# tiangexiang/OccNeRF

Measured on AMD Instinct MI355X. Metric: rays/sec at 512x512x128spp, random-init ckpt, higher is better.
Workload: dtype f32; 1 GPU; BASELINE configs[1]: free-view frame, 512x512 image, 128 samples/ray, non-rigid motion on, seeded random-init checkpoint; synthetic SMPL-like body and camera; 183784 rays hit the body bbox (ray_mask); H2D of the ray batch and the prior and D2H of [R,5] inside the step; the frame's rays sharded over the ranks; samples whose motion-weight sum is exactly 0 are dropped after the warp (bit-identical pi; rays_per_frame=183784, samples_per_ray=128, skip_empty_samples=True, dedup_repeated_samples=False, knn_center_cache=True, warp_bone_culling=True, world_size_formed=1

## Files before the change

### include/occnerf_hip.h

```cpp
#ifndef OCCNERF_HIP_H
#define OCCNERF_HIP_H

#include <stdint.h>

#ifdef __cplusplus
extern "C" {
#endif

#define OCCNERF_ABI_VERSION 5

int occnerf_abi_version(void);
const char *occnerf_last_error(void);

int occnerf_experiment_knob(const char *name, int value);


int occnerf_grid_encode_forward(const float *inputs, const float *embeddings,
                                const int32_t *offsets, float *outputs, uint32_t B, uint32_t D,
                                uint32_t C, uint32_t L, float S, uint32_t H, float *dy_dx,
                                uint32_t gridtype, int align_corners, uint32_t interp,
                                void *stream);

int occnerf_grid_encode_backward(const float *grad, const float *inputs, const float *embeddings,
                                 const int32_t *offsets, float *grad_embeddings, uint32_t B,
                                 uint32_t D, uint32_t C, uint32_t L, float S, uint32_t H,
                                 const float *dy_dx, float *grad_inputs, uint32_t gridtype,
                                 int align_corners, uint32_t interp, void *stream);

int occnerf_grid_encode_forward_h(const float *inputs, const float *embeddings, const int32_t *offsets,
                                  const int32_t *h_offsets, float *outputs, uint32_t B, uint32_t D, uint32_t C, uint32_t L,
                                  float S, uint32_t H, float *dy_dx, uint32_t gridtype, int align_corners,
                                  uint32_t interp, void *stream);

int occnerf_grid_grad_runs(const float *grad_rows, const float *inputs, int64_t B, uint32_t D, uint32_t L, uint32_t C,
                           float *grad, void *stream);

int occnerf_grid_encode_backward_h(const float *grad, const float *inputs, const float *embeddings,
                                   const int32_t *offsets, const int32_t *h_offsets, float *grad_embeddings,
                                   uint32_t B, uint32_t D, uint32_t C, uint32_t L, float S, uint32_t H,
                                   const float *dy_dx, float *grad_inputs, uint32_t gridtype, int align_corners,
                                   uint32_t interp, void *scratch, int64_t scratch_bytes, void *stream);

int occnerf_grid_encode_forward_f16(const float *inputs, const void *embeddings, const int32_t *offsets, void *outputs,
                                    uint32_t B, uint32_t D, uint32_t C, uint32_t L, float S, uint32_t H, void *dy_dx,
                                    uint32_t gridtype, int align_corners, uint32_t interp, void *stream);
int occnerf_grid_encode_backward_f16(const void *grad, const float *inputs, const void *embeddings, const int32_t *offsets,
                                     void *grad_embeddings, uint32_t B, uint32_t D, uint32_t C, uint32_t L, float S,
                                     uint32_t H, const void *dy_dx, void *grad_inputs, uint32_t gridtype, int align_corners,
                                     uint32_t interp, void *stream);

int occnerf_grid_encode_forward_f64(const float *inputs, const double *embeddings, const int32_t *offsets, double *outputs,
                                    uint32_t B, uint32_t D, uint32_t C, uint32_t L, float S, uint32_t H, double *dy_dx,
                                    uint32_t gridtype, int align_corners, uint32_t interp, void *stream);
int occnerf_grid_encode_backward_f64(const double *grad, const float *inputs, const double *embeddings, const int32_t *offsets,
                                     double *grad_embeddings, uint32_t B, uint32_t D, uint32_t C, uint32_t L, float S,
                                     uint32_t H, const double *dy_dx, double *grad_inputs, uint32_t gridtype, int align_corners,
                                     uint32_t interp, void *stream);

int occnerf_grad_total_variation(const float *inputs, const float *embeddings, float *grad,
                                 const int32_t *offsets, float weight, uint32_t B, uint32_t D,
                                 uint32_t C, uint32_t L, float S, uint32_t H, uint32_t gridtype,
                                 int align_corners, void *stream);


int occnerf_sample_warp(const float *rays, int64_t n, int32_t S, const float *t_vals,
                        const float *t_rand, const float *Rs, const float *Ts, const float *vol,
                        int32_t nb, int32_t G, const float *h_bbox_min, const float *h_bbox_scale,
                        float *z_vals, float *pts, float *x_skel, float *mask, void *stream);
int occnerf_bone_boxes(const float *vol, int32_t nb, int32_t G, int32_t *boxes, void *stream);
int occnerf_sample_warp_culled(const float *rays, int64_t n, int32_t S, const float *t_vals,
                               const float *Rs, const float *Ts, const float *vol, int32_t nb, int32_t G,
                               const int32_t *boxes, const float *h_bbox_min, const float *h_bbox_scale,
                               float *z_vals, float *x_skel, float *mask, void *stream);

int64_t occnerf_ray_order_temp_bytes(int64_t R);
int occnerf_ray_order(const float *dirs, int64_t R, int64_t stride, int64_t *order, void *temp, int64_t temp_bytes,
                      void *stream);

int occnerf_gen_rays(const double *h_Kinv, const double *h_R, const double *h_T, int32_t f32_camera,
                     int32_t H, int32_t W, const double *h_bbox_min, const double *h_bbox_max, float *rays8,
                     uint8_t *mask, void *stream);

int64_t occnerf_nonrigid_packed_floats(void);
int occnerf_nonrigid_pack(const float *const *h_W, const float *const *h_b, float *packed,
                          void *stream);
int occnerf_nonrigid(const float *xyz_in, int64_t N, const float *cond, const float *h_hann,
                     const float *W0, const float *b0, float *packed, float *xyz_out,
                     void *stream);
int occnerf_nonrigid_rows(float *xyz, int64_t N_max, const int32_t *rows, const int32_t *n_dev,
                          const float *cond, const float *h_hann, const float *W0, const float *b0,
                          float *packed, void *stream);
int occnerf_nonrigid_direct(const float *xyz_in, int64_t N, const float *cond, const float *h_hann,
                            const float *W0, const float *b0, float *packed, float *xyz_out,
                            void *stream);

int64_t occnerf_nonrigid_packed_bf16_bytes(void);
int occnerf_nonrigid_pack_bf16(const float *const *h_W, void *packed_bf16, void *stream);
int occnerf_nonrigid_bf16x3(const float *xyz_in, int64_t N, const float *cond, const float *h_hann,
                            const float *W0, const float *b0, float *packed, const void *packed_bf16,
                            float *xyz_out, void *stream);
int occnerf_nonrigid_bf16x3_rows(float *xyz, int64_t N_max, const int32_t *rows, const int32_t *n_dev,
                                 const float *cond, const float *h_hann, const float *W0, const float *b0,
                                 float *packed, const void *packed_bf16, void *stream);

int occnerf_msknn(const float *xyz, int64_t N, const float *points, const int32_t *index_map,
                  const int32_t *h_scale_begin, const int32_t *h_seed_from_coarser,
                  int32_t nscale, int32_t *knn_idxs, void *stream);

int occnerf_msknn_clustered(const float *xyz, const float *mask, int64_t n_rays, int32_t samples_per_ray,
                            const float *points, const float *centers,
                            const int32_t *cluster_ranges, const float *cluster_radius, int32_t ncl,
                            const float *group_centers, const int32_t *group_ranges, const float *group_radius, int32_t ngrp,
                            const int32_t *h_coarse_rows, const int32_t *h_seed_from_coarser,
                            int32_t nscale, const int32_t *query_rows, const int32_t *n_query_dev, int32_t *ray_start,
                            int32_t *knn_idxs, void *stream);
int occnerf_knn_center(const float *c, const float *points, const int32_t *index_map, const int32_t *h_scale_begin,
                       int32_t nscale, float *center_out, int32_t *idx_out, void *stream);
int occnerf_msknn_clustered_centered(const float *xyz, const float *mask, int64_t n_rays, int32_t samples_per_ray,
                                     const float *points, const float *centers,
                                     const int32_t *cluster_ranges, const float *cluster_radius, int32_t ncl,
                                     const float *group_centers, const int32_t *group_ranges, const float *group_radius, int32_t ngrp,
                                     const int32_t *h_coarse_rows, const int32_t *h_seed_from_coarser,
                                     int32_t nscale, const int32_t *query_rows, const int32_t *n_query_dev, int32_t *ray_start,
                                     const float *center, const int32_t *center_idx, int32_t *knn_idxs, void *stream);

int occnerf_knn_small(const float *q, int32_t nq, const float *s, int32_t ns, int32_t k,
                      int32_t *idx, void *stream);

int occnerf_unit_normals(const double *normals, int32_t P, double *unit, void *stream);

int occnerf_point_sdf(const float *point_cloud, const float *point_base, const double *normals,
                      const double *unit_normals, const int32_t *kidx, int32_t P,
                      double *knn_base, float *dist, void *stream);

int occnerf_point_sdf_backward(const float *point_cloud, const float *point_base, const double *normals,
                               const double *unit_normals, const int32_t *kidx, int32_t P, const double *d_knn_base,
                               const float *d_dist, float *d_point_dist, void *stream);
int32_t occnerf_point_table_stride(void);
int occnerf_point_table(const double *knn_base, const float *point_sdf, const float *learnable,
                        int32_t P, float bound, float two_bound, const float *embeddings,
                        const int32_t *offsets, const int32_t *h_offsets, uint32_t L, float S,
                        uint32_t H, float *table, void *stream);

int occnerf_point_pack(const float *point_base, const double *normals, const double *unit_normals,
                       const float *counter, const float *table, int32_t P, float *point_geo,
                       float *point_tail, void *stream);
int occnerf_sample_features(const float *xyz, int64_t N, const int32_t *knn_idxs, int32_t nscale,
                            const float *point_base, const double *normals,
                            const double *unit_normals, const float *counter,
                            const float *table, float bound, float two_bound,
                            const float *embeddings, const int32_t *offsets,
                            const int32_t *h_offsets, uint32_t L, float S, uint32_t H,
                            const int32_t *geo_idxs, const float *att_in, const int32_t *rows,
                            const int32_t *n_dev, const float *point_geo, const float *point_tail, int32_t P,
                            float *mlp_in, float *raw, float *enc_in, void *stream);
int occnerf_sample_features_centered(const float *xyz, int64_t N, const int32_t *knn_idxs, int32_t nscale,
                            const float *point_base, const double *normals,
                            const double *unit_normals, const float *counter,
                            const float *table, float bound, float two_bound,
                            const float *embeddings, const int32_t *offsets,
                            const int32_t *h_offsets, uint32_t L, float S, uint32_t H,
                            const int32_t *geo_idxs, const float *att_in, const int32_t *rows,
                            const int32_t *n_dev, const float *point_geo, const float *point_tail, int32_t P,
                            const float *center, const float *center_agg,
                                     float *mlp_in, float *raw, float *enc_in, void *stream);

int occnerf_agg_forward(const float *feats, int32_t F, const int32_t *knn, const float *atts, int64_t N, int32_t K,
                        float *agg, void *stream);
int32_t occnerf_agg_backward_slices(int64_t N);
int64_t occnerf_agg_backward_scratch_bytes(int64_t N, int32_t F);
int occnerf_agg_backward(const float *grad_agg, int32_t F, const int32_t *knn, const float *atts, int64_t N,
                         int32_t K, int32_t P, float *partial, void *scratch, int64_t scratch_bytes, void *stream);

int64_t occnerf_live_rows_temp_bytes(int64_t N);
int occnerf_live_rows(const float *mask, int64_t N, int32_t *rows, int32_t *count, void *temp,
                      int64_t temp_bytes, void *stream);
int occnerf_scatter_raw(const float *raw_c, const int32_t *rows, const int32_t *n_dev, int64_t N_max,
                        float *raw_full, void *stream);

int64_t occnerf_repeat_heads_temp_bytes(int64_t N_max);
int occnerf_repeat_heads(const void *keys, int64_t stride_dwords, int32_t key_dwords, const int32_t *rows,
                         const int32_t *n_dev, int64_t N_max, int32_t *scan, int32_t *heads, int32_t *head_count,
                         float *head_mask, void *temp, int64_t temp_bytes, void *stream);
int64_t occnerf_unique_heads_temp_bytes(int64_t cap);
int occnerf_unique_heads(const void *keys, int64_t stride_dwords, int32_t key_dwords, const int32_t *heads,
                         const int32_t *n_dev, int64_t cap, int32_t *heads_out, int32_t *count_out, int32_t *scan,
                         const int32_t *n_scan_dev, int64_t scan_cap, void *temp, int64_t temp_bytes, void *stream);
int occnerf_scatter_raw_heads(const float *raw_h, const float *raw_c, const int32_t *rows, const int32_t *n_dev,
                              const int32_t *scanA, const int32_t *scanB, int64_t N_max, float *raw_full, void *stream);
int occnerf_canonical_mlp_rows(const float *mlp_in, const int32_t *in_rows, int64_t N_max, const int32_t *n_dev,
                               const float *packed, float *raw, void *stream);

int64_t occnerf_canonical_mlp_packed_floats(void);
int occnerf_canonical_mlp_pack(const float *const *h_W, const float *const *h_b, float *packed,
                               void *stream);

int occnerf_canonical_mlp(const float *mlp_in, int64_t N, const float *packed, float *raw,
                          void *stream);
int occnerf_canonical_mlp_direct(const float *mlp_in, int64_t N, const float *packed, float *raw,
                                 void *stream);
int occnerf_canonical_mlp_counted(const float *mlp_in, int64_t N_max, const int32_t *n_dev,
                                  const float *packed, float *raw, void *stream);

int64_t occnerf_canonical_mlp_packed_bf16_bytes(void);
int occnerf_canonical_mlp_pack_bf16(const float *const *h_W, void *packed_bf16, void *stream);
int occnerf_canonical_mlp_bf16x3(const float *mlp_in, int64_t N, const float *packed,
                                 const void *packed_bf16, float *raw, int32_t variant,
                                 void *stream);
int occnerf_canonical_mlp_bf16x3_rows(const float *mlp_in, const int32_t *in_rows, int64_t N_max,
                                      const int32_t *n_dev, const float *packed, const void *packed_bf16,
                                      float *raw, int32_t variant, void *stream);

int occnerf_canonical_mlp_pack_f16(const float *const *h_W, void *packed_f16, void *stream);
int occnerf_canonical_mlp_f16x3(const float *mlp_in, const int32_t *in_rows, int64_t N_max, const int32_t *n_dev,
                                const float *packed, const void *packed_f16, float *raw, uint32_t *domain_flag,
                                void *stream);
int occnerf_nonrigid_pack_f16(const float *const *h_W, void *packed_f16, void *stream);
int occnerf_nonrigid_f16x3(const float *xyz_in, int64_t N_max, const int32_t *rows, const int32_t *n_dev,
                           const float *cond, const float *h_hann, const float *W0, const float *b0, float *packed,
                           const void *packed_f16, float *xyz_out, uint32_t *domain_flag, void *stream);

int occnerf_composite(const float *raw, const float *mask, const float *z_vals, const float *rays,
                      const float *h_bgcolor, int64_t n, int32_t S, float *rgb, float *acc,
                      float *depth, float *weights, int32_t *term, const int64_t *out_rows, void *stream);


int occnerf_linear_pack(const float *W, const float *b, int32_t out_dim, int32_t in_dim, const int32_t *row_map,
                        int32_t n_pad, const int32_t *col_map, int32_t k_pad, int32_t bf16, void *Wp, void *Wt,
                        float *bias_p, void *stream);
int occnerf_linear_forward(const void *x0, int64_t ld0, int32_t k0, const void *x1, int64_t ld1, int32_t k1,
                           const void *W, const float *bias, int32_t relu, const void *mask, int64_t ldm, void *y,
                           int64_t ldy, int32_t out_f32, int32_t n_store, float *aux, int32_t aux_col,
                           int64_t aux_stride, int64_t M, int32_t n_pad, int32_t bf16, void *stream);
int32_t occnerf_linear_wgrad_slices(int64_t M);
int occnerf_linear_wgrad(const void *dz, int64_t lddz, int32_t n_pad, const void *x, int64_t ldx, int32_t k_pad,
                         int64_t M, int32_t bf16, float *part, float *dbpart, void *stream);
int occnerf_linear_wgrad_reduce(const float *part, const float *dbpart, int32_t G, int32_t n_pad, int32_t k_pad,
                                const int32_t *row_map, const int32_t *col_map, float *dW, int32_t in_dim, float *db,
                                int32_t accumulate, void *stream);

int64_t occnerf_trunks_packed_bytes(void);
int occnerf_trunks_pack_bf16(const float *const *h_W, void *packed, void *stream);
int occnerf_trunks_forward_bf16(const float *agg, const float *var, const float *enc, int64_t M, const float *packed_f32,
                                const void *packed_bf16, void *X0, void *const *h_A, void *GEO, void *const *h_B, float *raw4,
                                void *stream);

int occnerf_composite_backward(const float *raw, const float *mask, const float *z_vals, const float *rays,
                               const float *h_bgcolor, int64_t n, int32_t S, const float *g_rgb, const float *g_acc,
                               const float *g_depth, float *d_raw, float *d_mask, void *stream);

int32_t occnerf_warp_backward_slices(int64_t n_samples);
int occnerf_warp_backward(const float *rays, int64_t n, int32_t S, const float *z_vals, const float *g_mask,
                          const float *Rs, const float *Ts, const float *vol, int32_t nb, int32_t G,
                          const float *h_bbox_min, const float *h_bbox_scale, float *d_vol_part, float *d_rt_part,
                          void *stream);

int occnerf_agg_weights(const float *counter, const int32_t *knn, int64_t N, int32_t K, float *atts, float *var,
                        void *stream);

int occnerf_pose_motion_bases_backward(const float *const *h_W, const float *const *h_b, const float *posevec,
                                       const float *dst_Rs, const float *dst_Ts, const float *cnl_gtfms,
                                       const float *dRs, const float *dTs, float *const *h_dW, float *const *h_db,
                                       void *stream);

int occnerf_pose_motion_bases(const float *const *h_W, const float *const *h_b, const float *posevec, int32_t refine,
                              const float *dst_Rs, const float *dst_Ts, const float *cnl_gtfms, float *Rs, float *Ts,
                              void *stream);
int occnerf_prior_softmax(const float *decoded, const float *prior, int32_t C, int64_t V, float *vol, void *stream);
int occnerf_pack_rays(const float *rays, const float *near, const float *far, const int64_t *order, int64_t R, float *rays8,
                      void *stream);

int occnerf_assemble_image(const float *rgb, const float *alpha, const int64_t *ray_index, int64_t R, int32_t height,
                           int32_t width, const float *h_bgcolor01, uint8_t *out_rgb, uint8_t *out_alpha, void *stream);

int occnerf_convt3d_col2im(const float *cols, const float *bias, int32_t Cout, int32_t D, int32_t H, int32_t W,
                           float *out, void *stream);
int occnerf_convt3d_im2col(const float *gy, int32_t Cout, int32_t D, int32_t H, int32_t W, float *dcols, void *stream);

int32_t occnerf_adam_table_row_bytes(void);
int occnerf_adam_step(const void *table, int32_t n_tensors, const int32_t *chunks, int32_t n_chunks,
                      int32_t chunk_elems, double beta1, double beta2, double eps, double max_grad_norm, float *scratch,
                      void *stream);

int64_t occnerf_lpips_packed_floats(void);
int64_t occnerf_lpips_workspace_floats(int32_t N, int32_t H, int32_t W);
int occnerf_lpips_pack(const float *const *h_conv_w, const float *const *h_conv_b, const float *const *h_lin,
                       const float *shift, const float *scale, float *packed, void *stream);
int occnerf_lpips_forward(const float *packed, const float *in0, const float *in1, int32_t N, int32_t H, int32_t W,
                          int32_t in_nhwc, float *work, float *val, float *res, void *stream);
int occnerf_lpips_backward(const float *packed, float *work, int32_t N, int32_t H, int32_t W, int32_t in_nhwc,
                           const float *gres, float *d_in0, float *d_in1, void *stream);

int occnerf_patch_assemble(const float *rgb, const int32_t *row_of_pix, int64_t R, int32_t n_patches, int32_t size,
                           const float *h_bgcolor01, float *img, void *stream);
int occnerf_patch_assemble_backward(const float *d_img, const int32_t *pix_of_row, int64_t R, float *d_rgb, void *stream);

int32_t occnerf_patch_batch_max_patches(void);
int occnerf_patch_batch(const uint8_t *image, const uint8_t *alpha, const float *rays8, const uint8_t *box_mask, int32_t H,
                        int32_t W, int32_t n_patches, int32_t size, const double *h_u, double subject_ratio,
                        const float *h_bgcolor, int32_t *row_counts, float *rays, float *near, float *far, float *target_rgbs,
                        float *target_patches, uint8_t *patch_masks, int32_t *patch_div_indices, int32_t *xy_min,
                        int32_t *pix_of_row, int32_t *row_of_pix, int32_t *n_rows, void *stream);

#define OCCNERF_FRAME_METRICS_RECORD 14
int64_t occnerf_frame_metrics_workspace_bytes(int32_t N, int32_t H, int32_t W);
int occnerf_frame_metrics(const uint8_t *pred, const uint8_t *truth, const float *alpha, const uint8_t *body,
                          const float *gt_vis_alpha, const float *gt_alpha, int32_t N, int32_t H, int32_t W,
                          double data_range, double *record, double *ssim_map, void *workspace, void *stream);

#ifdef __cplusplus
}
#endif
#endif
```

### occnerf_amd/_lib.py

```python
import ctypes as C
import os

_HERE = os.path.dirname(os.path.abspath(__file__))
LIB_PATH = os.environ.get('OCCNERF_HIP_LIB') or os.path.join(_HERE, 'liboccnerf_hip.so')

ABI_VERSION = 5

_vp, _i32, _i64, _u32, _f32 = C.c_void_p, C.c_int32, C.c_int64, C.c_uint32, C.c_float

SIGNATURES = {
    'occnerf_abi_version': (C.c_int, []),
    'occnerf_last_error': (C.c_char_p, []),
    'occnerf_experiment_knob': (C.c_int, [C.c_char_p, C.c_int]),
    'occnerf_grid_encode_forward': (C.c_int, [_vp, _vp, _vp, _vp, _u32, _u32, _u32, _u32, _f32, _u32,
                                               _vp, _u32, C.c_int, _u32, _vp]),
    'occnerf_grid_encode_backward': (C.c_int, [_vp, _vp, _vp, _vp, _vp, _u32, _u32, _u32, _u32, _f32,
                                                _u32, _vp, _vp, _u32, C.c_int, _u32, _vp]),
    'occnerf_grid_grad_runs': (C.c_int, [_vp, _vp, _i64, _u32, _u32, _u32, _vp, _vp]),
    'occnerf_grid_encode_forward_h': (C.c_int, [_vp, _vp, _vp, _vp, _vp, _u32, _u32, _u32, _u32, _f32, _u32,
                                                 _vp, _u32, C.c_int, _u32, _vp]),
    'occnerf_grid_encode_backward_h': (C.c_int, [_vp, _vp, _vp, _vp, _vp, _vp, _u32, _u32, _u32, _u32, _f32,
                                                  _u32, _vp, _vp, _u32, C.c_int, _u32, _vp, _i64, _vp]),
    'occnerf_grid_encode_forward_f16': (C.c_int, [_vp, _vp, _vp, _vp, _u32, _u32, _u32, _u32, _f32, _u32,
                                                   _vp, _u32, C.c_int, _u32, _vp]),
    'occnerf_grid_encode_backward_f16': (C.c_int, [_vp, _vp, _vp, _vp, _vp, _u32, _u32, _u32, _u32, _f32,
                                                    _u32, _vp, _vp, _u32, C.c_int, _u32, _vp]),
    'occnerf_grid_encode_forward_f64': (C.c_int, [_vp, _vp, _vp, _vp, _u32, _u32, _u32, _u32, _f32, _u32,
                                                   _vp, _u32, C.c_int, _u32, _vp]),
    'occnerf_grid_encode_backward_f64': (C.c_int, [_vp, _vp, _vp, _vp, _vp, _u32, _u32, _u32, _u32, _f32,
                                                    _u32, _vp, _vp, _u32, C.c_int, _u32, _vp]),
    'occnerf_trunks_packed_bytes': (_i64, []),
    'occnerf_trunks_pack_bf16': (C.c_int, [_vp, _vp, _vp]),
    'occnerf_trunks_forward_bf16': (C.c_int, [_vp, _vp, _vp, _i64, _vp, _vp, _vp, _vp, _vp, _vp, _vp, _vp]),
    'occnerf_grad_total_variation': (C.c_int, [_vp, _vp, _vp, _vp, _f32, _u32, _u32, _u32, _u32, _f32,
                                                _u32, _u32, C.c_int, _vp]),
    'occnerf_sample_warp': (C.c_int, [_vp, _i64, _i32, _vp, _vp, _vp, _vp, _vp, _i32, _i32, _vp, _vp,
                                       _vp, _vp, _vp, _vp, _vp]),
    'occnerf_bone_boxes': (C.c_int, [_vp, _i32, _i32, _vp, _vp]),
    'occnerf_sample_warp_culled': (C.c_int, [_vp, _i64, _i32, _vp, _vp, _vp, _vp, _i32, _i32, _vp, _vp, _vp, _vp, _vp, _vp, _vp]),
    'occnerf_nonrigid_packed_floats': (_i64, []),
    'occnerf_nonrigid_pack': (C.c_int, [_vp, _vp, _vp, _vp]),
    'occnerf_nonrigid': (C.c_int, [_vp, _i64, _vp, _vp, _vp, _vp, _vp, _vp, _vp]),
    'occnerf_nonrigid_direct': (C.c_int, [_vp, _i64, _vp, _vp, _vp, _vp, _vp, _vp, _vp]),
    'occnerf_nonrigid_packed_bf16_bytes': (_i64, []),
    'occnerf_nonrigid_pack_bf16': (C.c_int, [_vp, _vp, _vp]),
    'occnerf_nonrigid_bf16x3': (C.c_int, [_vp, _i64, _vp, _vp, _vp, _vp, _vp, _vp, _vp, _vp]),
    'occnerf_nonrigid_bf16x3_rows': (C.c_int, [_vp, _i64, _vp, _vp, _vp, _vp, _vp, _vp, _vp, _vp, _vp]),
    'occnerf_msknn': (C.c_int, [_vp, _i64, _vp, _vp, _vp, _vp, _i32, _vp, _vp]),
    'occnerf_msknn_clustered': (C.c_int, [_vp, _vp, _i64, _i32, _vp, _vp, _vp, _vp, _i32, _vp, _vp, _vp, _i32, _vp, _vp, _i32,
                                           _vp, _vp, _vp, _vp, _vp]),
    'occnerf_msknn_clustered_centered': (C.c_int, [_vp, _vp, _i64, _i32, _vp, _vp, _vp, _vp, _i32, _vp, _vp, _vp, _i32, _vp, _vp, _i32,
                                           _vp, _vp, _vp, _vp, _vp, _vp, _vp]),
    'occnerf_knn_center': (C.c_int, [_vp, _vp, _vp, _vp, _i32, _vp, _vp, _vp]),
    'occnerf_knn_small': (C.c_int, [_vp, _i32, _vp, _i32, _i32, _vp, _vp]),
    'occnerf_unit_normals': (C.c_int, [_vp, _i32, _vp, _vp]),
    'occnerf_point_sdf': (C.c_int, [_vp, _vp, _vp, _vp, _vp, _i32, _vp, _vp, _vp]),
    'occnerf_ray_order_temp_bytes': (_i64, [_i64]),
    'occnerf_ray_order': (C.c_int, [_vp, _i64, _i64, _vp, _vp, _i64, _vp]),
    'occnerf_point_sdf_backward': (C.c_int, [_vp, _vp, _vp, _vp, _vp, _i32, _vp, _vp, _vp, _vp]),
    'occnerf_gen_rays': (C.c_int, [_vp, _vp, _vp, _i32, _i32, _i32, _vp, _vp, _vp, _vp, _vp]),
    'occnerf_agg_forward': (C.c_int, [_vp, _i32, _vp, _vp, _i64, _i32, _vp, _vp]),
    'occnerf_agg_backward_slices': (_i32, [_i64]),
    'occnerf_agg_backward_scratch_bytes': (_i64, [_i64, _i32]),
    'occnerf_agg_backward': (C.c_int, [_vp, _i32, _vp, _vp, _i64, _i32, _i32, _vp, _vp, _i64, _vp]),
    'occnerf_live_rows_temp_bytes': (_i64, [_i64]),
    'occnerf_live_rows': (C.c_int, [_vp, _i64, _vp, _vp, _vp, _i64, _vp]),
    'occnerf_scatter_raw': (C.c_int, [_vp, _vp, _vp, _i64, _vp, _vp]),
    'occnerf_repeat_heads_temp_bytes': (_i64, [_i64]),
    'occnerf_repeat_heads': (C.c_int, [_vp, _i64, _i32, _vp, _vp, _i64, _vp, _vp, _vp, _vp, _vp, _i64, _vp]),
    'occnerf_unique_heads_temp_bytes': (_i64, [_i64]),
    'occnerf_unique_heads': (C.c_int, [_vp, _i64, _i32, _vp, _vp, _i64, _vp, _vp, _vp, _vp, _i64, _vp, _i64, _vp]),
    'occnerf_scatter_raw_heads': (C.c_int, [_vp, _vp, _vp, _vp, _vp, _vp, _i64, _vp, _vp]),
    'occnerf_canonical_mlp_rows': (C.c_int, [_vp, _vp, _i64, _vp, _vp, _vp, _vp]),
    'occnerf_canonical_mlp_counted': (C.c_int, [_vp, _i64, _vp, _vp, _vp, _vp]),
    'occnerf_nonrigid_rows': (C.c_int, [_vp, _i64, _vp, _vp, _vp, _vp, _vp, _vp, _vp, _vp]),
    'occnerf_point_table_stride': (_i32, []),
    'occnerf_point_table': (C.c_int, [_vp, _vp, _vp, _i32, _f32, _f32, _vp, _vp, _vp, _u32, _f32, _u32, _vp,
                                       _vp]),
    'occnerf_point_pack': (C.c_int, [_vp, _vp, _vp, _vp, _vp, _i32, _vp, _vp, _vp]),
    'occnerf_sample_features': (C.c_int, [_vp, _i64, _vp, _i32, _vp, _vp, _vp, _vp, _vp, _f32, _f32, _vp,
                                           _vp, _vp, _u32, _f32, _u32, _vp, _vp, _vp, _vp, _vp, _vp, _i32, _vp, _vp,
                                           _vp, _vp]),
    'occnerf_sample_features_centered': (C.c_int, [_vp, _i64, _vp, _i32, _vp, _vp, _vp, _vp, _vp, _f32, _f32, _vp,
                                                    _vp, _vp, _u32, _f32, _u32, _vp, _vp, _vp, _vp, _vp, _vp, _i32, _vp, _vp,
                                                    _vp, _vp, _vp, _vp]),
    'occnerf_canonical_mlp_packed_floats': (_i64, []),
    'occnerf_canonical_mlp_pack': (C.c_int, [_vp, _vp, _vp, _vp]),
    'occnerf_canonical_mlp': (C.c_int, [_vp, _i64, _vp, _vp, _vp]),
    'occnerf_canonical_mlp_direct': (C.c_int, [_vp, _i64, _vp, _vp, _vp]),
    'occnerf_canonical_mlp_packed_bf16_bytes': (_i64, []),
    'occnerf_canonical_mlp_pack_bf16': (C.c_int, [_vp, _vp, _vp]),
    'occnerf_canonical_mlp_bf16x3': (C.c_int, [_vp, _i64, _vp, _vp, _vp, _i32, _vp]),
    'occnerf_canonical_mlp_pack_f16': (C.c_int, [_vp, _vp, _vp]),
    'occnerf_canonical_mlp_f16x3': (C.c_int, [_vp, _vp, _i64, _vp, _vp, _vp, _vp, _vp, _vp]),
    'occnerf_nonrigid_pack_f16': (C.c_int, [_vp, _vp, _vp]),
    'occnerf_nonrigid_f16x3': (C.c_int, [_vp, _i64, _vp, _vp, _vp, _vp, _vp, _vp, _vp, _vp, _vp, _vp, _vp]),
    'occnerf_canonical_mlp_bf16x3_rows': (C.c_int, [_vp, _vp, _i64, _vp, _vp, _vp, _vp, _i32, _vp]),
    'occnerf_composite': (C.c_int, [_vp, _vp, _vp, _vp, _vp, _i64, _i32, _vp, _vp, _vp, _vp, _vp, _vp, _vp]),
    'occnerf_linear_pack': (C.c_int, [_vp, _vp, _i32, _i32, _vp, _i32, _vp, _i32, _i32, _vp, _vp, _vp, _vp]),
    'occnerf_linear_forward': (C.c_int, [_vp, _i64, _i32, _vp, _i64, _i32, _vp, _vp, _i32, _vp, _i64, _vp, _i64, _i32,
                                          _i32, _vp, _i32, _i64, _i64, _i32, _i32, _vp]),
    'occnerf_linear_wgrad_slices': (_i32, [_i64]),
    'occnerf_linear_wgrad': (C.c_int, [_vp, _i64, _i32, _vp, _i64, _i32, _i64, _i32, _vp, _vp, _vp]),
    'occnerf_linear_wgrad_reduce': (C.c_int, [_vp, _vp, _i32, _i32, _i32, _vp, _vp, _vp, _i32, _vp, _i32, _vp]),
    'occnerf_composite_backward': (C.c_int, [_vp, _vp, _vp, _vp, _vp, _i64, _i32, _vp, _vp, _vp, _vp, _vp, _vp]),
    'occnerf_warp_backward_slices': (_i32, [_i64]),
    'occnerf_warp_backward': (C.c_int, [_vp, _i64, _i32, _vp, _vp, _vp, _vp, _vp, _i32, _i32, _vp, _vp, _vp, _vp, _vp]),
    'occnerf_agg_weights': (C.c_int, [_vp, _vp, _i64, _i32, _vp, _vp, _vp]),
    'occnerf_pose_motion_bases': (C.c_int, [_vp, _vp, _vp, _i32, _vp, _vp, _vp, _vp, _vp, _vp]),
    'occnerf_pose_motion_bases_backward': (C.c_int, [_vp, _vp, _vp, _vp, _vp, _vp, _vp, _vp, _vp, _vp, _vp]),
    'occnerf_prior_softmax': (C.c_int, [_vp, _vp, _i32, _i64, _vp, _vp]),
    'occnerf_pack_rays': (C.c_int, [_vp, _vp, _vp, _vp, _i64, _vp, _vp]),
    'occnerf_assemble_image': (C.c_int, [_vp, _vp, _vp, _i64, _i32, _i32, _vp, _vp, _vp, _vp]),
    'occnerf_convt3d_col2im': (C.c_int, [_vp, _vp, _i32, _i32, _i32, _i32, _vp, _vp]),
    'occnerf_convt3d_im2col': (C.c_int, [_vp, _i32, _i32, _i32, _i32, _vp, _vp]),
    'occnerf_adam_table_row_bytes': (_i32, []),
    'occnerf_adam_step': (C.c_int, [_vp, _i32, _vp, _i32, _i32] + [C.c_double] * 4 + [_vp, _vp]),
    'occnerf_lpips_packed_floats': (_i64, []),
    'occnerf_lpips_workspace_floats': (_i64, [_i32, _i32, _i32]),
    'occnerf_lpips_pack': (C.c_int, [_vp, _vp, _vp, _vp, _vp, _vp, _vp]),
    'occnerf_lpips_forward': (C.c_int, [_vp, _vp, _vp, _i32, _i32, _i32, _i32, _vp, _vp, _vp, _vp]),
    'occnerf_lpips_backward': (C.c_int, [_vp, _vp, _i32, _i32, _i32, _i32, _vp, _vp, _vp, _vp]),
    'occnerf_patch_assemble': (C.c_int, [_vp, _vp, _i64, _i32, _i32, _vp, _vp, _vp]),
    'occnerf_patch_assemble_backward': (C.c_int, [_vp, _vp, _i64, _vp, _vp]),
    'occnerf_patch_batch_max_patches': (_i32, []),
    'occnerf_patch_batch': (C.c_int, [_vp, _vp, _vp, _vp, _i32, _i32, _i32, _i32, _vp, C.c_double, _vp] + [_vp] * 12 + [_vp]),
    'occnerf_frame_metrics_workspace_bytes': (_i64, [_i32, _i32, _i32]),
    'occnerf_frame_metrics': (C.c_int, [_vp, _vp, _vp, _vp, _vp, _vp, _i32, _i32, _i32, C.c_double, _vp, _vp, _vp, _vp]),
}

_lib = None


def lib():
    global _lib
    if _lib is None:
        if not os.path.exists(LIB_PATH):
            raise ImportError(
                f'{LIB_PATH} not found: the gfx950 kernels are not built. Run '
                '`python -c "import __graft_entry__ as g; g.build()"` (or `make -C '
                'occnerf_amd/csrc`). There is no CPU fallback for this path.')
        import torch
        handle = C.CDLL(LIB_PATH)
        for name, (res, args) in SIGNATURES.items():
            fn = getattr(handle, name)
            fn.restype, fn.argtypes = res, args
        if handle.occnerf_abi_version() != ABI_VERSION:
            raise ImportError(f'liboccnerf_hip.so: ABI version {handle.occnerf_abi_version()}, this binding was written '
                              f'for {ABI_VERSION} (include/occnerf_hip.h OCCNERF_ABI_VERSION): rebuild the library')
        _lib = handle
    return _lib


def check(rc, what):
    if rc != 0:
        msg = lib().occnerf_last_error().decode(errors='replace')
        raise RuntimeError(f'{what} failed ({rc}): {msg}')
```

### occnerf_amd/config.py

```python
import argparse
import ast
import copy
import os

import yaml


class CfgNode(dict):
    def __getattr__(self, k):
        try:
            return self[k]
        except KeyError:
            raise AttributeError(k)

    def __setattr__(self, k, v):
        self[k] = v

    def get(self, k, default=None):
        return dict.get(self, k, default)

    @staticmethod
    def wrap(d):
        if isinstance(d, dict) and not isinstance(d, CfgNode):
            return CfgNode({k: CfgNode.wrap(v) for k, v in d.items()})
        return d

    def merge(self, other):
        for k, v in other.items():
            if isinstance(v, dict) and isinstance(self.get(k), dict):
                self[k].merge(v)
            else:
                self[k] = CfgNode.wrap(copy.deepcopy(v))
        return self

    def merge_from_file(self, path):
        with open(path) as f:
            return self.merge(yaml.safe_load(f) or {})

    def merge_from_list(self, opts):
        assert len(opts) % 2 == 0, 'opts must be KEY VALUE pairs'
        for key, val in zip(opts[0::2], opts[1::2]):
            node = self
            parts = key.split('.')
            for p in parts[:-1]:
                node = node[p]
            try:
                val = ast.literal_eval(val)
            except (ValueError, SyntaxError):
                pass
            node[parts[-1]] = val
        return self

    def clone(self):
        return CfgNode.wrap(copy.deepcopy(dict(self)))


_DEFAULTS = {
    'category': 'occnerf', 'task': 'zju_mocap', 'subject': 'p387', 'experiment': 'occnerf',
    'resume': False, 'eval_iter': 10000000, 'render_folder_name': '',
    'ignore_non_rigid_motions': False, 'render_skip': 1, 'render_frames': 100, 'num_workers': 4,
    'network_module': 'core.nets.occnerf.network',
    'embedder': {'module': 'core.nets.occnerf.embedders.fourier'},
    'non_rigid_embedder': {'module': 'core.nets.occnerf.embedders.hannw_fourier'},
    'canonical_mlp': {'module': 'core.nets.occnerf.canonical_mlps.occnerf_mlp', 'mlp_depth': 4,
                      'mlp_width': 256, 'multires': 10, 'i_embed': 0},
    'mweight_volume': {'module': 'core.nets.occnerf.mweight_vol_decoders.deconv_vol_decoder',
                       'embedding_size': 256, 'volume_size': 32, 'dst_voxel_size': 0.0625},
    'non_rigid_motion_mlp': {'module': 'core.nets.occnerf.non_rigid_motion_mlps.mlp_offset',
                             'condition_code_size': 69, 'mlp_width': 128, 'mlp_depth': 6,
                             'skips': [4], 'multires': 6, 'i_embed': 0, 'kick_in_iter': 100000,
                             'full_band_iter': 200000},
    'pose_decoder': {'module': 'core.nets.occnerf.pose_decoders.mlp_delta_body_pose',
                     'embedding_size': 69, 'mlp_width': 256, 'mlp_depth': 4,
                     'kick_in_iter': 2000000},
    'sex': 'neutral', 'total_bones': 24, 'bbox_offset': 0.3, 'load_net': 'latest',
    'N_samples': 128, 'perturb': 1.0, 'netchunk_per_gpu': 300000, 'chunk': 32768, 'n_gpus': 1,
    'bgcolor': [0.0, 0.0, 0.0], 'resize_img_scale': 0.5, 'show_alpha': False, 'show_truth': False,
    'patch': {'sample_subject_ratio': 0.8, 'N_patches': 6, 'size': 32},
    'freeview': {'frame_idx': 0}, 'tpose': {}, 'movement': {},
    'train': {'dataset_path': None, 'images_prescaled': False, 'seed': 0, 'prefetch': True},
    'occlude': False, 'occlusion': {'range': 405, 'mid': 451, 'width': 86},
    'eval': {'lpips': False, 'lpips_model_path': None, 'lpips_vgg16_path': None},
    'smpl_model': 'auto',
    'max_samples_per_pass': 1 << 28,
    'mlp_precision': 'fp32',
    'f16x3_domain_check': True,
    'train_fused_trunks': True,
    'skip_empty_samples': True,
    'device_rays': True,
    'ray_patch_order': True,
    'knn_culling': True,
    'knn_center_cache': True,
    'warp_bone_culling': True,
}

_cfg = None


def default_cfg():
    return CfgNode.wrap(copy.deepcopy(_DEFAULTS))


def get_cfg():
    global _cfg
    if _cfg is None:
        _cfg = default_cfg()
        _finish(_cfg)
    return _cfg


def set_cfg(cfg):
    global _cfg
    _cfg = cfg
    return cfg


def _finish(cfg):
    import torch
    cfg.logdir = os.path.join('experiments', cfg.category, cfg.task, cfg.subject, cfg.experiment)
    n = torch.cuda.device_count()
    cfg.n_gpus = n
    cfg.primary_gpus = [0] if n > 0 else ['cpu']
    cfg.secondary_gpus = ([g for g in range(n) if g != 0] or cfg.primary_gpus) if n > 1 \
        else cfg.primary_gpus


def make_cfg(argv=None):
    parser = argparse.ArgumentParser()
    parser.add_argument('--cfg', required=True, type=str)
    parser.add_argument('--eval', default='full', type=str)
    parser.add_argument('--type', default='skip', type=str)
    parser.add_argument('opts', default=None, nargs=argparse.REMAINDER)
    args = parser.parse_args(argv)
    cfg = default_cfg()
    here = os.path.dirname(os.path.dirname(os.path.abspath(__file__)))
    default_yaml = os.path.join(here, 'configs', 'default.yaml')
    if os.path.exists(default_yaml):
        cfg.merge_from_file(default_yaml)
    cfg.merge_from_file(args.cfg)
    cfg.merge_from_list(args.opts or [])
    _finish(cfg)
    set_cfg(cfg)
    return cfg, args
```

### occnerf_amd/csrc/features.hip

```cpp
#include "common.h"

#include <cstdlib>

namespace occ {

constexpr int kKnn = 10;
constexpr int kTableCols = 36;
constexpr int kTableStride = 64;

__device__ __forceinline__ double cos3_unit(const float (&a)[3], const double *__restrict__ un) {
    float na = norm3(a[0], a[1], a[2]);
    na = na < 1e-8f ? 1e-8f : na;
    const double t0 = __dmul_rn((double)__fdiv_rn(a[0], na), un[0]);
    const double t1 = __dmul_rn((double)__fdiv_rn(a[1], na), un[1]);
    const double t2 = __dmul_rn((double)__fdiv_rn(a[2], na), un[2]);
    return __dadd_rn(__dadd_rn(t0, t1), t2);
}

__global__ void unit_normals_kernel(const double *__restrict__ normals, int P,
                                    double *__restrict__ unit) {
    const int i = blockIdx.x * blockDim.x + threadIdx.x;
    if (i >= P) return;
    const double b0 = normals[i * 3], b1 = normals[i * 3 + 1], b2 = normals[i * 3 + 2];
    double nb = __dsqrt_rn(__dadd_rn(__dadd_rn(__dmul_rn(b0, b0), __dmul_rn(b1, b1)), __dmul_rn(b2, b2)));
// ... 68 lines not shown
        for (int k = 0; k < 3; k++) datt += d_knn_base[i * 3 + k] * (nbr[j][k] - num[k] / den);
        datt /= den;
        const double dc = c[j] < 0.0 ? -datt : (c[j] > 0.0 ? datt : 0.0);
        for (int k = 0; k < 3; k++) {
            const double u = dir[j][k] / nd[j];
            g += gd * u + dc * (unit[n * 3 + k] - c[j] * u) / nd[j];
        }
    }
    d_point_dist[i] = (float)g;
}

__global__ void point_table_kernel(const double *__restrict__ knn_base,
                                   const float *__restrict__ point_sdf,
                                   const float *__restrict__ learnable, int P, float bound,
                                   float two_bound, const float2 *__restrict__ embeddings,
                                   const int32_t *__restrict__ offsets, int L, GridLevels lv,
                                   GridModes4 gm, float *__restrict__ table) {
    const int i = blockIdx.x * blockDim.x + threadIdx.x;
    if (i >= P) return;
    float x[4];
#pragma unroll
    for (int c = 0; c < 3; c++)
        x[c] = (float)__ddiv_rn(__dadd_rn(knn_base[i * 3 + c], (double)bound), (double)two_bound);
    float s = __fdiv_rn(__fadd_rn(point_sdf[i], 0.2f), 0.8f);
    x[3] = s < 0.0f ? 0.0f : (s > 1.0f ? 1.0f : s);
    bool oob = false;
#pragma unroll
    for (int d = 0; d < 4; d++) oob |= (x[d] < 0.f || x[d] > 1.f);
    float *row = table + (size_t)i * kTableStride;
    for (int l = 0; l < L; l++) {
        float2 v = make_float2(0.f, 0.f);
        if (!oob) {
            const uint32_t o0 = (uint32_t)offsets[l];
            v = encode_level_d4c2(x, embeddings + o0, (uint32_t)offsets[l + 1] - o0, lv.scale[l],
                                  lv.resolution[l], gm.mode[l]);
        }
        row[l * 2] = v.x;
        row[l * 2 + 1] = v.y;
    }
    for (int l = L; l < 16; l++) row[l * 2] = row[l * 2 + 1] = 0.f;
#pragma unroll
    for (int c = 0; c < 3; c++) row[32 + c] = learnable[i * 3 + c];
    row[35] = 0.0f;
}

static GridModes4 modes_from_host_offsets(uint32_t L, const GridLevels &lv, const int32_t *h_offsets) {
    uint32_t sizes[kMaxLevels] = {0};
    if (h_offsets)
        for (uint32_t l = 0; l < L; l++) sizes[l] = (uint32_t)(h_offsets[l + 1] - h_offsets[l]);
    GridModes4 gm = make_grid_modes_d4(h_offsets ? L : 0, lv, sizes);
    return gm;
}

struct FeatParams {
    float bound, two_bound;
    int nscale, L;
    int P;
};

struct LevelRec4 {
    uint32_t entry0, size;
    float scale;
    uint32_t res_mode;
};
struct LevelRecs {
    LevelRec4 r[kMaxLevels];
};
struct LevelRec8 {
    uint32_t entry0, mask;
    float scale;
    uint32_t dense;
    uint32_t mul1, mul2, mul3, pad;
};
struct LevelRecs8 {
    LevelRec8 r[kMaxLevels];
};
__device__ __forceinline__ void level_taps_select(const float (&x)[4], const float2 *grid, const LevelRec8 lr,
                                                  LevelTaps4 &tp) {
    const uint32_t mul[4] = {1u, lr.mul1, lr.mul2, lr.mul3};
    uint32_t t[4][2];
#pragma unroll
    for (int d = 0; d < 4; d++) {
        float pos = __fmaf_rn(x[d], lr.scale, 0.5f);
        const float fl = floorf(pos);
        const uint32_t pg = (uint32_t)fl;
        pos -= fl;
        tp.fr[d] = pos;
        t[d][0] = pg * mul[d];
        t[d][1] = t[d][0] + mul[d];
    }
    uint32_t a01[4], x01[4], a23[4], x23[4];
#pragma unroll
    for (int i = 0; i < 4; i++) {
        a01[i] = t[0][i & 1] + t[1][i >> 1];
        x01[i] = t[0][i & 1] ^ t[1][i >> 1];
        a23[i] = t[2][i & 1] + t[3][i >> 1];
        x23[i] = t[2][i & 1] ^ t[3][i >> 1];
    }
#pragma unroll
    for (int idx = 0; idx < 16; idx++) {
        const uint32_t ia = a01[idx & 3] + a23[idx >> 2];
        const uint32_t ix = (x01[idx & 3] ^ x23[idx >> 2]) & lr.mask;
        const uint32_t index = lr.dense ? ia : ix;
#ifdef OCC_FEAT_EXP_RESIDENT_HASH
        tp.v[idx] = ld32(grid, (lr.entry0 + (index & 63u)) * 8u);
#else
        tp.v[idx] = ld32(grid, (lr.entry0 + index) * 8u);
#endif
    }
}

__global__ __launch_bounds__(256) void sample_features_kernel(
    const float *__restrict__ xyz, int64_t N, const int32_t *__restrict__ knn_idxs,
    const float *__restrict__ point_base, const double *__restrict__ normals,
    const double *__restrict__ unit, const float *__restrict__ counter,
    const float4 *__restrict__ table, const float2 *__restrict__ embeddings,
    const int32_t *__restrict__ offsets, GridLevels lv, GridModes4 gm, FeatParams prm,
    const int32_t *__restrict__ geo_idxs, const float *__restrict__ att_in,
    float *__restrict__ mlp_in, float *__restrict__ raw, float *__restrict__ enc_in_out) {
    const int nk = prm.nscale * kKnn;
    for (int64_t i = (int64_t)blockIdx.x * blockDim.x + threadIdx.x; i < N;
         i += (int64_t)gridDim.x * blockDim.x) {
        const int32_t *id = knn_idxs + i * nk;
        const float p[3] = {xyz[i * 3], xyz[i * 3 + 1], xyz[i * 3 + 2]};

        int neg = 0;
        float dsum = 0.0f;
        double num[3] = {0.0, 0.0, 0.0}, den = 0.0;
#pragma unroll
        for (int j = 0; j < kKnn; j++) {
            const int n = geo_idxs ? geo_idxs[i * kKnn + j] : id[j];
            float dir[3], nbr[3];
#pragma unroll
            for (int c = 0; c < 3; c++) {
                nbr[c] = point_base[n * 3 + c];
                dir[c] = __fsub_rn(p[c], nbr[c]);
            }
            double dot = 0.0;
#pragma unroll
            for (int c = 0; c < 3; c++) dot = __dadd_rn(dot, __dmul_rn((double)dir[c], normals[(size_t)n * 3 + c]));
            neg += dot < 0.0;
            dsum = __fadd_rn(dsum, norm3(dir[0], dir[1], dir[2]));
            if (j < 3) {
                const double att = fabs(cos3_unit(dir, unit + (size_t)n * 3));
#pragma unroll
                for (int c = 0; c < 3; c++) {
                    const float pn = __fdiv_rn(__fadd_rn(nbr[c], prm.bound), prm.two_bound);
                    num[c] = __dadd_rn(num[c], __dmul_rn(att, (double)pn));
                }
                den = __dadd_rn(den, att);
            }
        }
        float dist = __fdiv_rn(dsum, (float)kKnn);
        if (2 * neg > kKnn) dist = -dist;
        float nd = __fdiv_rn(__fadd_rn(dist, 0.2f), 0.5f);
        nd = nd < 0.0f ? 0.0f : (nd > 1.0f ? 1.0f : nd);
        float x[4];
#pragma unroll
        for (int c = 0; c < 3; c++) x[c] = (float)__ddiv_rn(num[c], den);
        x[3] = nd;
        if (enc_in_out) {
#pragma unroll
            for (int c = 0; c < 4; c++) enc_in_out[i * 4 + c] = x[c];
        }
        raw[i * 5 + 4] = dist;

        float *out = mlp_in + i * 68;

        bool oob = false;
#pragma unroll
        for (int d = 0; d < 4; d++) oob |= (x[d] < 0.f || x[d] > 1.f);
        for (int l = 0; l < prm.L; l++) {
            float2 v = make_float2(0.f, 0.f);
            if (!oob) {
                const uint32_t o0 = (uint32_t)offsets[l];
                v = encode_level_d4c2(x, embeddings + o0, (uint32_t)offsets[l + 1] - o0,
                                      lv.scale[l], lv.resolution[l], gm.mode[l]);
            }
            *reinterpret_cast<float2 *>(out + 36 + l * 2) = v;
        }

        float att[4 * kKnn];
        float amin = INFINITY;
#pragma unroll
        for (int j = 0; j < 4 * kKnn; j++) {
            att[j] = j < nk ? (att_in ? att_in[i * nk + j] : counter[id[j]]) : INFINITY;
            amin = fminf(amin, att[j]);
        }
        float amax = -INFINITY;
#pragma unroll
        for (int j = 0; j < 4 * kKnn; j++) {
            if (j < nk) {
                att[j] = __fadd_rn(att[j], __fsub_rn(1.0f, amin));
                amax = fmaxf(amax, att[j]);
            }
        }
        float mean = 0.0f;
#pragma unroll
        for (int j = 0; j < 4 * kKnn; j++) {
            if (j < nk) {
                att[j] = __fdiv_rn(att[j], amax);
                mean = __fadd_rn(mean, att[j]);
            }
        }
        mean = __fdiv_rn(mean, (float)nk);
        float var = 0.0f, smax = -INFINITY;
#pragma unroll
        for (int j = 0; j < 4 * kKnn; j++) {
            if (j < nk) {
                const float dlt = __fsub_rn(att[j], mean);
                var = __fadd_rn(var, __fmul_rn(dlt, dlt));
                smax = fmaxf(smax, att[j]);
            }
        }
        var = __fdiv_rn(var, (float)(nk - 1));
        float ssum = 0.0f;
#pragma unroll
        for (int j = 0; j < 4 * kKnn; j++) {
            if (j < nk) {
                att[j] = expf(__fsub_rn(att[j], smax));
                ssum = __fadd_rn(ssum, att[j]);
            }
        }
        float agg[kTableCols];
#pragma unroll
        for (int f = 0; f < kTableCols; f++) agg[f] = 0.0f;
#pragma unroll
        for (int j = 0; j < 4 * kKnn; j++) {
            if (j < nk) {
                const float a = __fdiv_rn(att[j], ssum);
                const float4 *row = table + (size_t)id[j] * (kTableStride / 4);
#pragma unroll
                for (int v = 0; v < kTableCols / 4; v++) {
                    const float4 t = row[v];
                    agg[v * 4 + 0] = __fadd_rn(agg[v * 4 + 0], __fmul_rn(a, t.x));
                    agg[v * 4 + 1] = __fadd_rn(agg[v * 4 + 1], __fmul_rn(a, t.y));
                    agg[v * 4 + 2] = __fadd_rn(agg[v * 4 + 2], __fmul_rn(a, t.z));
                    agg[v * 4 + 3] = __fadd_rn(agg[v * 4 + 3], __fmul_rn(a, t.w));
                }
            }
        }
        agg[35] = var;
#pragma unroll
        for (int v = 0; v < kTableCols / 4; v++)
            *reinterpret_cast<float4 *>(out + v * 4) =
                make_float4(agg[v * 4], agg[v * 4 + 1], agg[v * 4 + 2], agg[v * 4 + 3]);
    }
}


__global__ void point_pack_kernel(const float *__restrict__ point_base, const double *__restrict__ normals,
                                  const double *__restrict__ unit, const float *__restrict__ counter,
                                  const float *__restrict__ table, int P, float *__restrict__ geo,
                                  float4 *__restrict__ tailc) {
    const int i = blockIdx.x * blockDim.x + threadIdx.x;
    if (i >= P) return;
    float *r = geo + (size_t)i * 16;
    r[0] = point_base[i * 3], r[1] = point_base[i * 3 + 1], r[2] = point_base[i * 3 + 2], r[3] = 0.0f;
    double *d = reinterpret_cast<double *>(r + 4);
    d[0] = normals[i * 3], d[1] = normals[i * 3 + 1], d[2] = normals[i * 3 + 2];
    d[3] = unit[i * 3], d[4] = unit[i * 3 + 1], d[5] = unit[i * 3 + 2];
    const float *t = table + (size_t)i * kTableStride + 32;
    tailc[i] = make_float4(t[0], t[1], t[2], counter[i]);
}

__device__ __forceinline__ float grp_sum8(float v) {
    v += __shfl_xor(v, 1, 8);
    v += __shfl_xor(v, 2, 8);
    v += __shfl_xor(v, 4, 8);
    return v;
}
__device__ __forceinline__ float grp_min8(float v) {
    v = fminf(v, __shfl_xor(v, 1, 8));
    v = fminf(v, __shfl_xor(v, 2, 8));
    return fminf(v, __shfl_xor(v, 4, 8));
}
__device__ __forceinline__ float grp_max8(float v) {
    v = fmaxf(v, __shfl_xor(v, 1, 8));
    v = fmaxf(v, __shfl_xor(v, 2, 8));
    return fmaxf(v, __shfl_xor(v, 4, 8));
}

template <int Q>
__device__ __forceinline__ float quad_bcast(float v) {
    return __builtin_bit_cast(float, __builtin_amdgcn_mov_dpp(__builtin_bit_cast(int, v), Q * 0x55, 0xf, 0xf, true));
}
template <int Q>
__device__ __forceinline__ double quad_bcast_f64(float lo, float hi) {
    return __hiloint2double(__builtin_amdgcn_mov_dpp(__builtin_bit_cast(int, hi), Q * 0x55, 0xf, 0xf, true),
                            __builtin_amdgcn_mov_dpp(__builtin_bit_cast(int, lo), Q * 0x55, 0xf, 0xf, true));
}

constexpr int kLdsTailPoints = 9216;

template <bool GENERIC ,
          bool LDS_TAIL >
__global__ __launch_bounds__(LDS_TAIL ? 768 : 256, 3) void sample_features8_kernel(
    const float *__restrict__ xyz, int64_t N_max, const int32_t *__restrict__ knn_idxs,
    const float4 *__restrict__ geo , const float4 *__restrict__ tailc ,
    const float4 *__restrict__ table, const float2 *__restrict__ embeddings,
    LevelRecs levels, LevelRecs8 levels8, FeatParams prm, const int32_t *__restrict__ rows ,
    const int32_t *__restrict__ n_dev , float *__restrict__ mlp_in, float *__restrict__ raw, float *__restrict__ enc_in_out,
    const float *__restrict__ center ,
    const float *__restrict__ center_agg ) {
    constexpr int NK = 4 * kKnn;
    float ccx = 0.f, ccy = 0.f, ccz = 0.f, cr2 = 0.f;
    if (center) ccx = center[0], ccy = center[1], ccz = center[2], cr2 = center[3];
    __shared__ float4 s_tail[LDS_TAIL ? kLdsTailPoints : 1];
    __shared__ float4 s_out[LDS_TAIL ? 768 : 256];
    static_assert(sizeof(float4) * (size_t)kLdsTailPoints + sizeof(float4) * 768 <= 160 * 1024,
                  "sample_features8_kernel<LDS_TAIL>: (tail, count) image + per-lane encoding slots exceed gfx950's 160 KiB of LDS");
    if constexpr (LDS_TAIL) {
        for (int i = threadIdx.x; i < prm.P; i += blockDim.x) s_tail[i] = tailc[i];
        __syncthreads();
    }
    const int g = threadIdx.x & 7;
    const int lane64 = threadIdx.x & 63;
    const int tr = ((lane64 & 7) << 3) | (lane64 >> 3);
    const int64_t N = n_dev ? (int64_t)*n_dev : N_max;
    if (N <= 0) return;
    const int64_t group0 = ((int64_t)blockIdx.x * blockDim.x + threadIdx.x) >> 3;
    const int64_t ngroups = ((int64_t)gridDim.x * blockDim.x) >> 3;
    const int64_t iters = (N + ngroups - 1) / ngroups;

    struct StageA {
        float p[3];
        int idg, id89;
        int id5[5];
    };
    auto out_row = [&](int64_t it) {
        const int64_t i_raw = group0 + it * ngroups;
        return i_raw < N ? i_raw : N - 1;
    };
    auto load_a = [&](int64_t i, StageA &a) {
        const int32_t *id = knn_idxs + i * NK;
        struct __attribute__((packed, aligned(4))) F3 { float v[3]; };
        struct __attribute__((packed, aligned(4))) I4 { int v[4]; };
        const F3 pq = *reinterpret_cast<const F3 *>(xyz + i * 3);
        a.p[0] = pq.v[0], a.p[1] = pq.v[1], a.p[2] = pq.v[2];
        a.idg = id[g];
        a.id89 = id[8 + (g >> 2)];
        const I4 q = *reinterpret_cast<const I4 *>(id + g * 5);
        a.id5[0] = q.v[0], a.id5[1] = q.v[1], a.id5[2] = q.v[2], a.id5[3] = q.v[3];
        a.id5[4] = id[g * 5 + 4];
    };
    StageA cur, nxt;
    int32_t i1;
    {
        const int64_t o0 = out_row(0), o1 = out_row(1);
        load_a(rows ? (int64_t)rows[o0] : o0, cur);
        i1 = rows ? rows[o1] : (int32_t)o1;
    }
    for (int64_t it = 0; it < iters; it++) {
        const bool live = group0 + it * ngroups < N;
        const int64_t o = out_row(it);
        const int64_t o2 = out_row(it + 2);
        float *out = mlp_in + o * 68;

        bool cached_agg = false;
        if (cr2 > 0.0f) {
            const float dx = cur.p[0] - ccx, dy = cur.p[1] - ccy, dz = cur.p[2] - ccz;
            const bool inside = __builtin_fmaf(dz, dz, __builtin_fmaf(dy, dy, dx * dx)) < cr2;
            cached_agg = __builtin_amdgcn_ballot_w64(live && !inside) == 0;
        }
        float4 tl[5];
#pragma unroll
        for (int k = 0; k < 5; k++) tl[k] = make_float4(0.f, 0.f, 0.f, 0.f);
        if (!cached_agg) {
#pragma unroll
            for (int k = 0; k < 5; k++) tl[k] = LDS_TAIL ? s_tail[cur.id5[k]] : ld32(tailc, (uint32_t)cur.id5[k] * 16u);
        }

        float nrm[5];
        int negf[5];
        double t_att[2] = {0.0, 0.0}, t_num[2][3] = {{0.0, 0.0, 0.0}, {0.0, 0.0, 0.0}};
        {
            float4 pc[5];
#pragma unroll
            for (int k = 0; k < 5; k++) {
                const int nid = k < 4 ? __shfl(cur.idg, 2 * k + (g >> 2), 8) : cur.id89;
                pc[k] = ld32(geo, (uint32_t)nid * 64u + (uint32_t)(g & 3) * 16u);
            }
#pragma unroll
            for (int k = 0; k < 5; k++) {
                const float nbr[3] = {quad_bcast<0>(pc[k].x), quad_bcast<0>(pc[k].y), quad_bcast<0>(pc[k].z)};
                const double nx = quad_bcast_f64<1>(pc[k].x, pc[k].y), ny = quad_bcast_f64<1>(pc[k].z, pc[k].w);
                const double nz = quad_bcast_f64<2>(pc[k].x, pc[k].y);
                float dir[3];
#pragma unroll
                for (int c = 0; c < 3; c++) dir[c] = __fsub_rn(cur.p[c], nbr[c]);
                double dot = __dadd_rn(0.0, __dmul_rn((double)dir[0], nx));
                dot = __dadd_rn(dot, __dmul_rn((double)dir[1], ny));
                dot = __dadd_rn(dot, __dmul_rn((double)dir[2], nz));
                negf[k] = dot < 0.0;
                nrm[k] = norm3(dir[0], dir[1], dir[2]);
                if (k < 2) {
                    const double un[3] = {quad_bcast_f64<2>(pc[k].z, pc[k].w), quad_bcast_f64<3>(pc[k].x, pc[k].y),
                                          quad_bcast_f64<3>(pc[k].z, pc[k].w)};
                    t_att[k] = fabs(cos3_unit(dir, un));
#pragma unroll
                    for (int c = 0; c < 3; c++) {
                        const float pn = __fdiv_rn(__fadd_rn(nbr[c], prm.bound), prm.two_bound);
                        t_num[k][c] = __dmul_rn(t_att[k], (double)pn);
                    }
                }
            }
        }
        float dsum = 0.0f;
        int neg = 0;
#pragma unroll
        for (int j = 0; j < kKnn; j++) {
            dsum = __fadd_rn(dsum, __shfl(nrm[j >> 1], 4 * (j & 1), 8));
            neg += __shfl(negf[j >> 1], 4 * (j & 1), 8);
        }
        double num[3] = {0.0, 0.0, 0.0}, den = 0.0;
#pragma unroll
        for (int j = 0; j < 3; j++) {
#pragma unroll
            for (int c = 0; c < 3; c++) num[c] = __dadd_rn(num[c], __shfl(t_num[j >> 1][c], 4 * (j & 1), 8));
            den = __dadd_rn(den, __shfl(t_att[j >> 1], 4 * (j & 1), 8));
        }
        float dist = __fdiv_rn(dsum, (float)kKnn);
        if (2 * neg > kKnn) dist = -dist;
        float nd = __fdiv_rn(__fadd_rn(dist, 0.2f), 0.5f);
        nd = nd < 0.0f ? 0.0f : (nd > 1.0f ? 1.0f : nd);
        float x[4];
#pragma unroll
        for (int c = 0; c < 3; c++) x[c] = (float)__ddiv_rn(num[c], den);
        x[3] = nd;
        if (live && g == 0) {
            raw[o * 5 + 4] = dist;
            if (enc_in_out) *reinterpret_cast<float4 *>(enc_in_out + o * 4) = make_float4(x[0], x[1], x[2], x[3]);
        }

        float a5[5] = {0.f, 0.f, 0.f, 0.f, 0.f};
        float var = 0.0f;
        float tail[3] = {0.f, 0.f, 0.f};
        if (!cached_agg) {
            float lmin = INFINITY;
#pragma unroll
            for (int k = 0; k < 5; k++) {
                a5[k] = tl[k].w;
                lmin = fminf(lmin, a5[k]);
            }
            const float amin = grp_min8(lmin);
            float lmax = -INFINITY;
#pragma unroll
            for (int k = 0; k < 5; k++) {
                a5[k] = __fadd_rn(a5[k], __fsub_rn(1.0f, amin));
                lmax = fmaxf(lmax, a5[k]);
            }
            const float amax = grp_max8(lmax);
            float lsum = 0.0f;
#pragma unroll
            for (int k = 0; k < 5; k++) {
                a5[k] = __fdiv_rn(a5[k], amax);
                lsum += a5[k];
            }
            const float mean = __fdiv_rn(grp_sum8(lsum), (float)NK);
            float lvar = 0.0f, lsm = -INFINITY;
#pragma unroll
            for (int k = 0; k < 5; k++) {
                const float dl = a5[k] - mean;
                lvar += dl * dl;
                lsm = fmaxf(lsm, a5[k]);
            }
            var = __fdiv_rn(grp_sum8(lvar), (float)(NK - 1));
            const float smax = grp_max8(lsm);
            float le = 0.0f;
#pragma unroll
            for (int k = 0; k < 5; k++) {
                a5[k] = expf(__fsub_rn(a5[k], smax));
                le += a5[k];
            }
            const float ssum = grp_sum8(le);
#pragma unroll
            for (int k = 0; k < 5; k++) a5[k] = __fdiv_rn(a5[k], ssum);

#pragma unroll
            for (int k = 0; k < 5; k++) {
                tail[0] += a5[k] * tl[k].x;
                tail[1] += a5[k] * tl[k].y;
                tail[2] += a5[k] * tl[k].z;
            }
        }

        bool cached_enc = false;
        if (cached_agg) {
            const bool eq = __float_as_uint(x[0]) == __float_as_uint(center_agg[36]) && __float_as_uint(x[1]) == __float_as_uint(center_agg[37]) &&
                            __float_as_uint(x[2]) == __float_as_uint(center_agg[38]) && __float_as_uint(x[3]) == __float_as_uint(center_agg[39]);
            cached_enc = __builtin_amdgcn_ballot_w64(live && !eq) == 0;
        }
        float2 ev[2];
        int32_t i2;
        if (!cached_enc) {
            LevelTaps4 tp[2];
            bool oob = false;
            float xt[4];
#pragma unroll
            for (int d = 0; d < 4; d++) xt[d] = __shfl(x[d], tr);
#pragma unroll
            for (int d = 0; d < 4; d++) oob |= (xt[d] < 0.f || xt[d] > 1.f);
            __builtin_amdgcn_sched_barrier(0);
            if (oob) {
#pragma unroll
                for (int d = 0; d < 4; d++) xt[d] = 0.5f;
            }
#pragma unroll
            for (int a = 0; a < 2; a++) {
                if constexpr (GENERIC) {
                    const LevelRec4 lr = levels.r[2 * (lane64 >> 3) + a];
                    encode_level_d4c2_taps(xt, embeddings, lr.size, lr.scale, lr.res_mode & 0xFFFFFFu, lr.res_mode >> 24,
                                           lr.entry0, tp[a]);
                } else {
                    level_taps_select(xt, embeddings, levels8.r[2 * (lane64 >> 3) + a], tp[a]);
                }
            }
            load_a(i1, nxt);
            i2 = rows ? rows[o2] : (int32_t)o2;
            __builtin_amdgcn_sched_barrier(0);
            float2 evt[2];
#pragma unroll
            for (int a = 0; a < 2; a++) {
                evt[a] = encode_level_d4c2_reduce(tp[a]);
                if (oob) evt[a] = make_float2(0.f, 0.f);
            }
#pragma unroll
            for (int a = 0; a < 2; a++) ev[a] = make_float2(__shfl(evt[a].x, tr), __shfl(evt[a].y, tr));
        } else {
            load_a(i1, nxt);
            i2 = rows ? rows[o2] : (int32_t)o2;
            const float4 ce = *reinterpret_cast<const float4 *>(center_agg + 40 + 4 * g);
            ev[0] = make_float2(ce.x, ce.y), ev[1] = make_float2(ce.z, ce.w);
        }
        s_out[threadIdx.x] = make_float4(ev[0].x, ev[0].y, ev[1].x, ev[1].y);

        float agg[4] = {0.f, 0.f, 0.f, 0.f};
        if (!cached_agg) {
            const uint32_t piece = (uint32_t)g * 16u;
            auto issue_chunk = [&](int c, float4 (&t)[10]) {
#pragma unroll
                for (int h = 0; h < 2; h++) {
#pragma unroll
                    for (int k = 0; k < 5; k++)
#ifdef OCC_FEAT_EXP_RESIDENT_ROWS
                        t[h * 5 + k] = ld32(table, (uint32_t)(__shfl(cur.id5[k], 2 * c + h, 8) & 15) * (uint32_t)(kTableStride * 4) + piece);
#else
                        t[h * 5 + k] = ld32(table, (uint32_t)__shfl(cur.id5[k], 2 * c + h, 8) * (uint32_t)(kTableStride * 4) + piece);
#endif
                }
            };
            float4 b0[10], b1[10], b2[10];
            issue_chunk(0, b0);
            issue_chunk(1, b1);
    #pragma unroll 1
            for (int c = 0; c < 4; c++) {
                const int cn = c + 2 < 4 ? c + 2 : 3;
                issue_chunk(cn, b2);
#pragma unroll
                for (int h = 0; h < 2; h++) {
#pragma unroll
                    for (int k = 0; k < 5; k++) {
                        const float w = __shfl(a5[k], 2 * c + h, 8);
                        const float4 t = b0[h * 5 + k];
                        agg[0] = __fadd_rn(agg[0], __fmul_rn(w, t.x));
                        agg[1] = __fadd_rn(agg[1], __fmul_rn(w, t.y));
                        agg[2] = __fadd_rn(agg[2], __fmul_rn(w, t.z));
                        agg[3] = __fadd_rn(agg[3], __fmul_rn(w, t.w));
                    }
                }
#pragma unroll
                for (int k = 0; k < 10; k++) b0[k] = b1[k], b1[k] = b2[k];
            }
#pragma unroll
            for (int c = 0; c < 3; c++) tail[c] = grp_sum8(tail[c]);
        } else {
            const float4 ca = *reinterpret_cast<const float4 *>(center_agg + 4 * g);
            agg[0] = ca.x, agg[1] = ca.y, agg[2] = ca.z, agg[3] = ca.w;
            tail[0] = center_agg[32], tail[1] = center_agg[33], tail[2] = center_agg[34], var = center_agg[35];
        }
        if (live) {
            *reinterpret_cast<float4 *>(out + 4 * g) = make_float4(agg[0], agg[1], agg[2], agg[3]);
            if (g == 0) *reinterpret_cast<float4 *>(out + 32) = make_float4(tail[0], tail[1], tail[2], var);
            *reinterpret_cast<float4 *>(out + 36 + 4 * g) = s_out[threadIdx.x];
        }
        cur = nxt;
        i1 = i2;
    }
}


}

OCC_API int occnerf_unit_normals(const double *normals, int32_t P, double *unit, void *stream) {
    using namespace occ;
    OCC_REQUIRE(normals && unit, "unit_normals: null argument");
    if (P <= 0) return 0;
    hipLaunchKernelGGL(unit_normals_kernel, dim3((P + 255) / 256), dim3(256), 0, as_stream(stream), normals, P, unit);
    return check_launch("unit_normals");
}

OCC_API int occnerf_point_sdf(const float *point_cloud, const float *point_base,
                              const double *normals, const double *unit_normals,
                              const int32_t *kidx, int32_t P, double *knn_base, float *dist,
                              void *stream) {
    using namespace occ;
    OCC_REQUIRE(point_cloud && point_base && normals && unit_normals && kidx && knn_base && dist,
                "point_sdf: null argument");
    if (P <= 0) return 0;
    hipLaunchKernelGGL(point_sdf_kernel, dim3((P + 255) / 256), dim3(256), 0, as_stream(stream), point_cloud,
                       point_base, normals, unit_normals, kidx, P, knn_base, dist);
    return check_launch("point_sdf");
}

OCC_API int occnerf_point_sdf_backward(const float *point_cloud, const float *point_base, const double *normals,
                                       const double *unit_normals, const int32_t *kidx, int32_t P, const double *d_knn_base,
                                       const float *d_dist, float *d_point_dist, void *stream) {
    using namespace occ;
    OCC_REQUIRE(point_cloud && point_base && normals && unit_normals && kidx && d_knn_base && d_dist && d_point_dist,
                "point_sdf_backward: null argument");
    if (P <= 0) return 0;
    hipLaunchKernelGGL(point_sdf_backward_kernel, dim3((P + 255) / 256), dim3(256), 0, as_stream(stream), point_cloud, point_base,
                       normals, unit_normals, kidx, P, d_knn_base, d_dist, d_point_dist);
    return check_launch("point_sdf_backward");
}

OCC_API int32_t occnerf_point_table_stride(void) { return occ::kTableStride; }

OCC_API int occnerf_point_table(const double *knn_base, const float *point_sdf,
                                const float *learnable, int32_t P, float bound, float two_bound,
                                const float *embeddings, const int32_t *offsets,
                                const int32_t *h_offsets, uint32_t L, float S, uint32_t H, float *table,
                                void *stream) {
    using namespace occ;
    OCC_REQUIRE(knn_base && point_sdf && learnable && embeddings && offsets && table, "point_table: null argument");
    OCC_REQUIRE(L >= 1 && L <= 16, "point_table: L=%u unsupported", L);
    if (P <= 0) return 0;
    const GridLevels lv = make_grid_levels(L, S, H);
    const GridModes4 gm = modes_from_host_offsets(L, lv, h_offsets);
    hipLaunchKernelGGL(point_table_kernel, dim3((P + 255) / 256), dim3(256), 0, as_stream(stream), knn_base,
                       point_sdf, learnable, P, bound, two_bound, reinterpret_cast<const float2 *>(embeddings),
                       offsets, (int)L, lv, gm, table);
    return check_launch("point_table");
}

OCC_API int occnerf_point_pack(const float *point_base, const double *normals, const double *unit_normals,
                               const float *counter, const float *table, int32_t P, float *point_geo,
                               float *point_tail, void *stream) {
    using namespace occ;
    OCC_REQUIRE(point_base && normals && unit_normals && counter && table && point_geo && point_tail,
                "point_pack: null argument");
    if (P <= 0) return 0;
    hipLaunchKernelGGL(point_pack_kernel, dim3((P + 255) / 256), dim3(256), 0, as_stream(stream), point_base, normals,
                       unit_normals, counter, table, P, point_geo, reinterpret_cast<float4 *>(point_tail));
    return check_launch("point_pack");
}

OCC_API int occnerf_sample_features(const float *xyz, int64_t N, const int32_t *knn_idxs,
                                    int32_t nscale, const float *point_base, const double *normals,
                                    const double *unit_normals, const float *counter,
                                    const float *table, float bound, float two_bound,
                                    const float *embeddings, const int32_t *offsets,
                                    const int32_t *h_offsets, uint32_t L, float S, uint32_t H,
                                    const int32_t *geo_idxs,
                                    const float *att_in, const int32_t *rows, const int32_t *n_dev,
                                    const float *point_geo, const float *point_tail, int32_t P,
                                    float *mlp_in, float *raw, float *enc_in, void *stream) {
    return occnerf_sample_features_centered(xyz, N, knn_idxs, nscale, point_base, normals, unit_normals, counter, table, bound,
                                            two_bound, embeddings, offsets, h_offsets, L, S, H, geo_idxs, att_in, rows, n_dev,
                                            point_geo, point_tail, P, nullptr, nullptr, mlp_in, raw, enc_in, stream);
}

OCC_API int occnerf_sample_features_centered(const float *xyz, int64_t N, const int32_t *knn_idxs,
                                             int32_t nscale, const float *point_base, const double *normals,
                                             const double *unit_normals, const float *counter,
                                             const float *table, float bound, float two_bound,
                                             const float *embeddings, const int32_t *offsets,
                                             const int32_t *h_offsets, uint32_t L, float S, uint32_t H,
                                             const int32_t *geo_idxs,
                                             const float *att_in, const int32_t *rows, const int32_t *n_dev,
                                             const float *point_geo, const float *point_tail, int32_t P,
                                             const float *center, const float *center_agg,
                                             float *mlp_in, float *raw, float *enc_in, void *stream) {
    using namespace occ;
    OCC_REQUIRE(!center == !center_agg, "sample_features: center and center_agg come together");
    if (N <= 0) return 0;
    OCC_REQUIRE(xyz && knn_idxs && point_base && normals && unit_normals && (counter || att_in) && table &&
                    embeddings && offsets && mlp_in && raw, "sample_features: null argument");
    OCC_REQUIRE(nscale >= 1 && nscale <= 4, "sample_features: nscale=%d unsupported", nscale);
    OCC_REQUIRE(L == 16, "sample_features: built for the 16-level encoder of occnerf_mlp.py:45 (L=%u)", L);
    if (N <= 0) return 0;
    const GridLevels lv = make_grid_levels(L, S, H);
    const GridModes4 gm = modes_from_host_offsets(L, lv, h_offsets);
    FeatParams prm{bound, two_bound, nscale, (int)L, (int)P};
    OCC_REQUIRE(!n_dev || rows, "sample_features: a device-side count needs the row list");
    OCC_REQUIRE(!point_geo == !point_tail, "sample_features: point_geo and point_tail come together (occnerf_point_pack)");
    const bool lanes8 = nscale == 4 && !geo_idxs && !att_in && counter && h_offsets && point_geo;
    OCC_REQUIRE(!rows || lanes8,
                "sample_features: a row list is only supported on the renderer's path (4 scales, per-point inputs, "
                "packed point records)");
    if (lanes8) {
        LevelRecs levels;
        for (uint32_t l = 0; l < kMaxLevels; l++)
            levels.r[l] = LevelRec4{(uint32_t)h_offsets[l], (uint32_t)(h_offsets[l + 1] - h_offsets[l]), lv.scale[l],
                                    lv.resolution[l] | (gm.mode[l] << 24)};
        LevelRecs8 levels8;
        bool generic = false;
        for (uint32_t l = 0; l < kMaxLevels; l++) {
            const uint32_t size = (uint32_t)(h_offsets[l + 1] - h_offsets[l]), r1 = lv.resolution[l] + 1;
            const bool dense = gm.mode[l] == kGridDense;
            generic |= gm.mode[l] == kGridGeneric;
            levels8.r[l] = LevelRec8{(uint32_t)h_offsets[l], dense ? 0xFFFFFFFFu : size - 1, lv.scale[l], dense ? 1u : 0u,
                                     dense ? r1 : 2654435761u, dense ? r1 * r1 : 805459861u,
                                     dense ? r1 * r1 * r1 : 3674653429u, 0u};
        }
        OCC_REQUIRE(P > 0, "sample_features: P=%d rows of packed point records", P);
        const bool lds_tail = P <= kLdsTailPoints && N >= 96 * 64;
        const int threads = lds_tail ? 768 : 256;
        int64_t blocks8 = (N * 8 + threads - 1) / threads;
        const int64_t cap = lds_tail ? (int64_t)kNumCU : (int64_t)kNumCU * 32;
        if (blocks8 > cap) blocks8 = cap;
        auto kern = generic ? (lds_tail ? sample_features8_kernel<true, true> : sample_features8_kernel<true, false>)
                            : (lds_tail ? sample_features8_kernel<false, true> : sample_features8_kernel<false, false>);
        hipLaunchKernelGGL(kern, dim3((unsigned)blocks8), dim3(threads), 0, as_stream(stream), xyz,
                           N, knn_idxs, reinterpret_cast<const float4 *>(point_geo),
                           reinterpret_cast<const float4 *>(point_tail),
                           reinterpret_cast<const float4 *>(table), reinterpret_cast<const float2 *>(embeddings),
                           levels, levels8, prm, rows, n_dev, mlp_in, raw, enc_in, center, center_agg);
        return check_launch("sample_features");
    }
    OCC_REQUIRE(!center, "sample_features: the centre aggregate is only supported on the renderer's path");
    int64_t blocks = (N + 255) / 256;
    if (blocks > (int64_t)kNumCU * 16) blocks = (int64_t)kNumCU * 16;
    hipLaunchKernelGGL(sample_features_kernel, dim3((unsigned)blocks), dim3(256), 0, as_stream(stream), xyz, N,
                       knn_idxs, point_base, normals, unit_normals, counter,
                       reinterpret_cast<const float4 *>(table), reinterpret_cast<const float2 *>(embeddings),
                       offsets, lv, gm, prm, geo_idxs, att_in, mlp_in, raw, enc_in);
    return check_launch("sample_features");
}
```

### occnerf_amd/csrc/knn.hip

```cpp
#include "common.h"

#include <map>
#include <mutex>
#include <utility>

#include <cmath>
#include <vector>

namespace occ {

typedef float f32x2 __attribute__((ext_vector_type(2)));

constexpr int kK = 10;

struct KBest {
    float s[kK];
    int i[kK];
};

__device__ __forceinline__ void kbest_reset(KBest &b) {
#pragma unroll
    for (int p = 0; p < kK; p++) {
        b.s[p] = INFINITY;
        b.i[p] = 0;
// ... 22 lines not shown
        const float s = sqrtf(d2);
        if (s < b.s[kK - 1]) {
            kbest_insert(b, s, row);
            thr = fminf(thr, filter_bound(b.s[kK - 1]));
        }
    }
}

struct MsKnnScales {
    int begin[5];
    int end[5];
    int seed[4];
    int nscale;
};

constexpr int kQ = 4;

__global__ __launch_bounds__(256) void msknn_kernel(const float *__restrict__ xyz, int64_t N,
                                                    const float4 *__restrict__ points,
                                                    const int32_t *__restrict__ index_map,
                                                    MsKnnScales sc,
                                                    int32_t *__restrict__ knn_idxs) {
    const int64_t tile = (int64_t)blockDim.x * kQ;
    for (int64_t base = (int64_t)blockIdx.x * tile; base < N; base += (int64_t)gridDim.x * tile) {
        int64_t qi[kQ];
        f32x2 qx[2], qy[2], qz[2];
#pragma unroll
        for (int a = 0; a < kQ; a++) {
            qi[a] = base + threadIdx.x + (int64_t)a * blockDim.x;
            const int64_t src = qi[a] < N ? qi[a] : N - 1;
            qx[a >> 1][a & 1] = xyz[src * 3 + 0];
            qy[a >> 1][a & 1] = xyz[src * 3 + 1];
            qz[a >> 1][a & 1] = xyz[src * 3 + 2];
        }
        KBest best[kQ];
        float thr[kQ];
#pragma unroll
        for (int a = 0; a < kQ; a++) thr[a] = INFINITY;

        for (int l = sc.nscale - 1; l >= 0; l--) {
#pragma unroll
            for (int a = 0; a < kQ; a++) {
                const bool carry = (l < sc.nscale - 1) && sc.seed[l];
                thr[a] = carry ? filter_bound(best[a].s[kK - 1]) : INFINITY;
                kbest_reset(best[a]);
            }
            const int jb = sc.begin[l], je = sc.end[l];
            for (int j = jb; j < je; j += 4) {
                const float4 p0 = points[j], p1 = points[j + 1], p2 = points[j + 2],
                             p3 = points[j + 3];
#define OCC_PT(P, OFF)                                                                     \
    {                                                                                      \
        _Pragma("unroll") for (int h = 0; h < 2; h++) {                                    \
            const f32x2 dx = qx[h] - P.x, dy = qy[h] - P.y, dz = qz[h] - P.z;              \
            const f32x2 d2 = __builtin_elementwise_fma(                                    \
                dz, dz, __builtin_elementwise_fma(dy, dy, dx * dx));                       \
            consider(best[2 * h], thr[2 * h], d2[0], j + OFF - jb);                        \
            consider(best[2 * h + 1], thr[2 * h + 1], d2[1], j + OFF - jb);                \
        }                                                                                  \
    }
                OCC_PT(p0, 0)
                OCC_PT(p1, 1)
                OCC_PT(p2, 2)
                OCC_PT(p3, 3)
#undef OCC_PT
            }
#pragma unroll
            for (int a = 0; a < kQ; a++) {
                if (qi[a] < N) {
                    int32_t *out = knn_idxs + (qi[a] * sc.nscale + l) * kK;
#pragma unroll
                    for (int p = 0; p < kK; p++) out[p] = index_map[jb + best[a].i[p]];
                }
            }
        }
    }
}

struct KBest64 {
    double k[kK];
};

__device__ __forceinline__ double key64(float s, int row) { return __hiloint2double(__float_as_int(s), row); }
__device__ __forceinline__ float key_dist(double k) { return __int_as_float(__double2hiint(k)); }
__device__ __forceinline__ int key_row(double k) { return __double2loint(k); }

__device__ __forceinline__ void kbest64_reset(KBest64 &b) {
#pragma unroll
    for (int p = 0; p < kK; p++) b.k[p] = key64(INFINITY, 0x7fffffff);
}

__device__ __forceinline__ void kbest64_insert(KBest64 &b, double t) {
#pragma unroll
    for (int p = 0; p < kK; p++) {
        double hi;
        asm("v_max_f64 %0, %1, %2" : "=v"(hi) : "v"(b.k[p]), "v"(t));
        asm("v_min_f64 %0, %0, %1" : "+v"(b.k[p]) : "v"(t));
        t = hi;
    }
}

__device__ __forceinline__ void consider_lex(KBest64 &b, float &thr, float &sb, float d2, int row) {
    if (d2 < thr) {
        kbest64_insert(b, key64(sqrtf(d2), row));
        sb = fminf(sb, key_dist(b.k[kK - 1]));
        thr = filter_bound(sb);
    }
}

__global__ __launch_bounds__(256) void knn_center_kernel(const float *__restrict__ c, const float4 *__restrict__ points,
                                                         const int32_t *__restrict__ index_map, MsKnnScales sc,
                                                         float *__restrict__ center_out ,
                                                         int32_t *__restrict__ idx_out ) {
    __shared__ unsigned long long s_key[4][11];
    const int lane = threadIdx.x & 63, l = threadIdx.x >> 6;
    const float cx = c[0], cy = c[1], cz = c[2];
    if (l < sc.nscale) {
        const int jb = sc.begin[l], je = sc.end[l];
        unsigned long long best[11];
#pragma unroll
        for (int p = 0; p < 11; p++) best[p] = ~0ull;
        for (int j = jb + lane; j < je; j += 64) {
            const float4 P = points[j];
            const float dx = cx - P.x, dy = cy - P.y, dz = cz - P.z;
            const float d = sqrtf(__builtin_fmaf(dz, dz, __builtin_fmaf(dy, dy, dx * dx)));
            unsigned long long t = ((unsigned long long)__float_as_uint(d) << 32) | (unsigned)(j - jb);
            if (!(d < INFINITY)) t = ~0ull;
#pragma unroll
            for (int p = 0; p < 11; p++) {
                const unsigned long long lo = t < best[p] ? t : best[p];
                t = t < best[p] ? best[p] : t;
                best[p] = lo;
            }
        }
        for (int round = 0; round < 11; round++) {
            unsigned long long m = best[0];
#pragma unroll
            for (int o = 32; o > 0; o >>= 1) {
                const unsigned long long other = ((unsigned long long)__shfl_xor((unsigned)(m >> 32), o) << 32) | __shfl_xor((unsigned)m, o);
                m = other < m ? other : m;
            }
            if (best[0] == m && m != ~0ull) {
#pragma unroll
                for (int p = 0; p < 10; p++) best[p] = best[p + 1];
                best[10] = ~0ull;
            }
            if (lane == 0) s_key[l][round] = m;
        }
    }
    __syncthreads();
    if (threadIdx.x < sc.nscale * 10) {
        const int ls = threadIdx.x / 10, j = threadIdx.x % 10;
        idx_out[ls * 10 + j] = index_map[sc.begin[ls] + (int)(unsigned)s_key[ls][j]];
    }
    if (threadIdx.x == 0) {
        float g = INFINITY, dmax = 0.0f;
        for (int ls = 0; ls < sc.nscale; ls++) {
            if (s_key[ls][10] == ~0ull) g = 0.0f;
            for (int j = 0; j < 10; j++)
                g = fminf(g, __uint_as_float((unsigned)(s_key[ls][j + 1] >> 32)) - __uint_as_float((unsigned)(s_key[ls][j] >> 32)));
            if (s_key[ls][10] != ~0ull) dmax = fmaxf(dmax, __uint_as_float((unsigned)(s_key[ls][10] >> 32)));
        }
        const float r = 0.9f * (0.5f * g - 2e-6f * (dmax + 1.0f));
        center_out[0] = cx, center_out[1] = cy, center_out[2] = cz;
        center_out[3] = (r > 0.0f && r < INFINITY) ? r * r : 0.0f;
    }
}

struct ClusteredScales {
    int nscale, ncl, ngrp;
    int coarse_begin, coarse_end;
    int seed[4];
};

struct OneQuery {
    float x, y, z;
    bool live;
};

#define OCC_PT1(P)                                                                          \
    {                                                                                       \
        const float dx = q.x - P.x, dy = q.y - P.y, dz = q.z - P.z;                         \
        const float d2 = __builtin_fmaf(dz, dz, __builtin_fmaf(dy, dy, dx * dx));           \
        consider_lex(best, thr, sb, d2, __float_as_int(P.w));                               \
    }
#define OCC_SCAN1(JB, JE)                                                                   \
    {                                                                                       \
        const int je_ = (JE);                                                               \
        int j = (JB);                                                                       \
        float4 n0 = points[j], n1 = points[j + 1], n2 = points[j + 2], n3 = points[j + 3];  \
        for (; j < je_; j += 4) {                                                           \
            const float4 p0 = n0, p1 = n1, p2 = n2, p3 = n3;                                \
            const int jn = j + 4 < je_ ? j + 4 : j;                                         \
            n0 = points[jn], n1 = points[jn + 1], n2 = points[jn + 2], n3 = points[jn + 3]; \
            OCC_PT1(p0) OCC_PT1(p1) OCC_PT1(p2) OCC_PT1(p3)                                 \
        }                                                                                   \
    }
#define OCC_EMIT1(L)                                                                        \
    if (q.live) {                                                                           \
        struct __attribute__((packed, aligned(4))) I4 { int v[4]; };                        \
        struct __attribute__((packed, aligned(4))) I2 { int v[2]; };                        \
        int32_t *out = knn_idxs + (qi * sc.nscale + (L)) * kK;                              \
        int r_[kK];                                                                         \
        _Pragma("unroll") for (int p = 0; p < kK; p++) r_[p] = key_row(best.k[p]) & 0xFFFF; \
        *reinterpret_cast<I4 *>(out) = I4{{r_[0], r_[1], r_[2], r_[3]}};                    \
        *reinterpret_cast<I4 *>(out + 4) = I4{{r_[4], r_[5], r_[6], r_[7]}};                \
        *reinterpret_cast<I2 *>(out + 8) = I2{{r_[8], r_[9]}};                              \
    }

__device__ __forceinline__ void search_one_query(const OneQuery q, const int64_t qi, const int lane,
                                                 const float4 *__restrict__ points, const float4 *__restrict__ centers,
                                                 const int2 *__restrict__ ranges, const float *__restrict__ radius,
                                                 const float4 *__restrict__ gcenters, const int2 *__restrict__ granges,
                                                 const float *__restrict__ gradius, const ClusteredScales &sc,
                                                 int32_t *__restrict__ knn_idxs) {
    KBest64 best;
    float thr = q.live ? INFINITY : -1.0f, sb = INFINITY;
    kbest64_reset(best);
    OCC_SCAN1(sc.coarse_begin, sc.coarse_end)
    OCC_EMIT1(sc.nscale - 1)
    const unsigned long long lv = __builtin_amdgcn_ballot_w64(q.live);
    const int first = lv ? __builtin_ctzll(lv) : 0;
    const float rx = __shfl(q.x, first), ry = __shfl(q.y, first), rz = __shfl(q.z, first);
    for (int l = sc.nscale - 2; l >= 0; l--) {
        sb = sc.seed[l] ? key_dist(best.k[kK - 1]) : INFINITY;
        thr = q.live ? filter_bound(sb) : -1.0f;
        kbest64_reset(best);
        const int2 *rg = ranges + (size_t)l * sc.ncl;
        const float *rd = radius + (size_t)l * sc.ncl;
        int k_first;
        {
            float bd = INFINITY;
            int bk = 0;
            for (int k = lane; k < sc.ncl; k += kWave) {
                const float4 c = centers[k];
                const float dx = rx - c.x, dy = ry - c.y, dz = rz - c.z;
                const float d = dx * dx + dy * dy + dz * dz;
                const bool has = rg[k].x < rg[k].y;
                if (has && d < bd) {
                    bd = d;
                    bk = k;
                }
            }
#pragma unroll
            for (int o = 32; o > 0; o >>= 1) {
                const float od = __shfl_xor(bd, o);
                const int ok = __shfl_xor(bk, o);
                if (od < bd || (od == bd && ok < bk)) {
                    bd = od;
                    bk = ok;
                }
            }
            k_first = __builtin_amdgcn_readfirstlane(bk);
        }
        {
            const int2 range = rg[k_first];
            OCC_SCAN1(range.x, range.y)
        }
        auto in_reach = [&](const float4 c, const float r) -> bool {
            const float dx = q.x - c.x, dy = q.y - c.y, dz = q.z - c.z;
            const float d2 = __builtin_fmaf(dz, dz, __builtin_fmaf(dy, dy, dx * dx));
            const float lim = (sb + r) * 1.00001f;
            return __builtin_amdgcn_ballot_w64(q.live && !(d2 > lim * lim)) != 0;
        };
        const int ngrp = sc.ngrp > 0 ? sc.ngrp : 1;
        for (int gi = 0; gi < ngrp; gi++) {
            int k_lo = 0, k_hi = sc.ncl;
            if (sc.ngrp > 0) {
                const float gr = gradius[(size_t)l * sc.ngrp + gi];
                if (gr < 0.0f) continue;
                if (!in_reach(gcenters[gi], gr)) continue;
                const int2 gk = granges[gi];
                k_lo = gk.x, k_hi = gk.y;
            }
            for (int k = k_lo; k < k_hi; k++) {
                if (k == k_first) continue;
                const int2 range = rg[k];
                if (range.x >= range.y) continue;
                if (!in_reach(centers[k], rd[k])) continue;
                OCC_SCAN1(range.x, range.y)
            }
        }
        OCC_EMIT1(l)
    }
}
#undef OCC_PT1
#undef OCC_SCAN1
#undef OCC_EMIT1

constexpr float kSplitExtent2 = 0.04f;

template <bool SPLIT >
__global__ __launch_bounds__(256) void msknn_clustered_kernel(
    const float *__restrict__ xyz, const float *__restrict__ mask , int64_t n_rays, int S,
    const float4 *__restrict__ points, const float4 *__restrict__ centers,
    const int2 *__restrict__ ranges , const float *__restrict__ radius ,
    const float4 *__restrict__ gcenters , const int2 *__restrict__ granges ,
    const float *__restrict__ gradius ,
    ClusteredScales sc, int32_t *__restrict__ knn_idxs, unsigned *__restrict__ ticket,
    const int32_t *__restrict__ qrows ,
    const int32_t *__restrict__ ray_start ,
    const float *__restrict__ center ,
    const int32_t *__restrict__ center_idx ,
    const float split_extent2 ) {
    const int lane = threadIdx.x & 63;
    float ccx = 0.f, ccy = 0.f, ccz = 0.f, cr2 = 0.f;
    if (center) ccx = center[0], ccy = center[1], ccz = center[2], cr2 = center[3];
    const int tiles_per_chunk = (S + 3) / 4;
    const int64_t n_tiles = ((n_rays + 63) / 64) * tiles_per_chunk;
    for (;;) {
        unsigned t32 = 0;
        if (lane == 0) t32 = atomicAdd(ticket, 1u);
        const int64_t job = (int64_t)(unsigned)__builtin_amdgcn_readfirstlane((int)t32);
        const int64_t tile = SPLIT ? job >> 2 : job;
        const int part = SPLIT ? (int)(job & 3) : 0;
        if (tile >= n_tiles) break;
        const int64_t n_blocks = (n_rays + 63) / 64;
        const int64_t blk = qrows ? tile % n_blocks : tile / tiles_per_chunk;
        const int64_t ray = blk * 64 + lane;
        const int s0 = (int)(qrows ? tile / n_blocks : tile % tiles_per_chunk) * 4;
        int64_t qi[kQ];
        bool live[kQ];
        f32x2 qx[2], qy[2], qz[2];
        int32_t hs = 0, hn = 0;
        if (qrows) {
            const int64_t r = ray < n_rays ? ray : n_rays - 1;
            hs = ray_start[r];
            hn = ray < n_rays ? ray_start[r + 1] - hs : 0;
        }
#pragma unroll
        for (int a = 0; a < kQ; a++) {
            live[a] = ray < n_rays && (s0 + a) < S;
            const int64_t r = ray < n_rays ? ray : n_rays - 1;
            const int sm = (s0 + a) < S ? (s0 + a) : S - 1;
            qi[a] = r * S + sm;
            if (qrows) {
                live[a] = (s0 + a) < hn;
                qi[a] = live[a] ? (int64_t)qrows[hs + s0 + a] : r * S;
            }
            if (mask && mask[qi[a]] == 0.0f) live[a] = false;
            qx[a >> 1][a & 1] = xyz[qi[a] * 3 + 0];
            qy[a >> 1][a & 1] = xyz[qi[a] * 3 + 1];
            qz[a >> 1][a & 1] = xyz[qi[a] * 3 + 2];
        }
        if (cr2 > 0.0f) {
#pragma unroll
            for (int a = 0; a < kQ; a++) {
                const float dx = qx[a >> 1][a & 1] - ccx, dy = qy[a >> 1][a & 1] - ccy, dz = qz[a >> 1][a & 1] - ccz;
                const float d2 = __builtin_fmaf(dz, dz, __builtin_fmaf(dy, dy, dx * dx));
                if (live[a] && d2 < cr2) {
                    live[a] = false;
                    struct __attribute__((packed, aligned(4))) I4 { int v[4]; };
                    struct __attribute__((packed, aligned(4))) I2 { int v[2]; };
                    for (int l = 0; part == 0 && l < sc.nscale; l++) {
                        int32_t *out = knn_idxs + (qi[a] * sc.nscale + l) * kK;
                        const int32_t *ci = center_idx + l * kK;
                        *reinterpret_cast<I4 *>(out) = I4{{ci[0], ci[1], ci[2], ci[3]}};
                        *reinterpret_cast<I4 *>(out + 4) = I4{{ci[4], ci[5], ci[6], ci[7]}};
                        *reinterpret_cast<I2 *>(out + 8) = I2{{ci[8], ci[9]}};
                    }
                }
            }
        }
        if (__builtin_amdgcn_ballot_w64(live[0] || live[1] || live[2] || live[3]) == 0) continue;
        if constexpr (SPLIT) {
            float lo[3] = {INFINITY, INFINITY, INFINITY}, hi[3] = {-INFINITY, -INFINITY, -INFINITY};
#pragma unroll
            for (int a = 0; a < kQ; a++) {
                if (live[a]) {
                    const float v[3] = {qx[a >> 1][a & 1], qy[a >> 1][a & 1], qz[a >> 1][a & 1]};
#pragma unroll
                    for (int d = 0; d < 3; d++) lo[d] = fminf(lo[d], v[d]), hi[d] = fmaxf(hi[d], v[d]);
                }
            }
#pragma unroll
            for (int o = 32; o > 0; o >>= 1) {
#pragma unroll
                for (int d = 0; d < 3; d++) {
                    lo[d] = fminf(lo[d], __shfl_xor(lo[d], o));
                    hi[d] = fmaxf(hi[d], __shfl_xor(hi[d], o));
                }
            }
            const float ex = hi[0] - lo[0], ey = hi[1] - lo[1], ez = hi[2] - lo[2];
            const float ext2 = __int_as_float(__builtin_amdgcn_readfirstlane(__float_as_int(ex * ex + ey * ey + ez * ez)));
            const bool spread = ext2 > split_extent2;
            if (!spread && part != 0) continue;
            if (spread) {
                OneQuery q1{0.f, 0.f, 0.f, false};
                int64_t q1i = 0;
#pragma unroll
                for (int a = 0; a < kQ; a++) {
                    if (a == part) {
                        q1 = OneQuery{qx[a >> 1][a & 1], qy[a >> 1][a & 1], qz[a >> 1][a & 1], live[a]};
                        q1i = qi[a];
                    }
                }
                if (__builtin_amdgcn_ballot_w64(q1.live) != 0)
                    search_one_query(q1, q1i, lane, points, centers, ranges, radius, gcenters, granges, gradius, sc, knn_idxs);
                continue;
            }
        }
        KBest64 best[kQ];
        float thr[kQ], sb[kQ];

     \
#define OCC_PT4(P)                                                                          \
    {                                                                                       \
        const f32x2 dx0 = qx[0] - P.x, dy0 = qy[0] - P.y, dz0 = qz[0] - P.z;                \
        const f32x2 dx1 = qx[1] - P.x, dy1 = qy[1] - P.y, dz1 = qz[1] - P.z;                \
        const f32x2 da = __builtin_elementwise_fma(dz0, dz0, __builtin_elementwise_fma(dy0, dy0, dx0 * dx0)); \
        const f32x2 db = __builtin_elementwise_fma(dz1, dz1, __builtin_elementwise_fma(dy1, dy1, dx1 * dx1)); \
        if ((da[0] < thr[0]) | (da[1] < thr[1]) | (db[0] < thr[2]) | (db[1] < thr[3])) {    \
            const int row = __float_as_int(P.w);                                            \
            consider_lex(best[0], thr[0], sb[0], da[0], row);                               \
            consider_lex(best[1], thr[1], sb[1], da[1], row);                               \
            consider_lex(best[2], thr[2], sb[2], db[0], row);                               \
            consider_lex(best[3], thr[3], sb[3], db[1], row);                               \
        }                                                                                   \
    }
        \
#define OCC_SCAN(JB, JE)                                                                    \
    {                                                                                       \
        const int je_ = (JE);                                                               \
        int j = (JB);                                                                       \
        float4 n0 = points[j], n1 = points[j + 1], n2 = points[j + 2], n3 = points[j + 3];  \
        for (; j < je_; j += 4) {                                                           \
            const float4 p0 = n0, p1 = n1, p2 = n2, p3 = n3;                                \
            const int jn = j + 4 < je_ ? j + 4 : j;                                         \
            n0 = points[jn], n1 = points[jn + 1], n2 = points[jn + 2], n3 = points[jn + 3]; \
            OCC_PT4(p0) OCC_PT4(p1) OCC_PT4(p2) OCC_PT4(p3)                                 \
        }                                                                                   \
    }
       \
#define OCC_EMIT(L)                                                                         \
    _Pragma("unroll") for (int a = 0; a < kQ; a++) {                                        \
        if (live[a]) {                                                                      \
            struct __attribute__((packed, aligned(4))) I4 { int v[4]; };                    \
            struct __attribute__((packed, aligned(4))) I2 { int v[2]; };                    \
            int32_t *out = knn_idxs + (qi[a] * sc.nscale + (L)) * kK;                       \
            int r_[kK];                                                                     \
            _Pragma("unroll") for (int p = 0; p < kK; p++) r_[p] = key_row(best[a].k[p]) & 0xFFFF; \
            *reinterpret_cast<I4 *>(out) = I4{{r_[0], r_[1], r_[2], r_[3]}};                \
            *reinterpret_cast<I4 *>(out + 4) = I4{{r_[4], r_[5], r_[6], r_[7]}};            \
            *reinterpret_cast<I2 *>(out + 8) = I2{{r_[8], r_[9]}};                          \
        }                                                                                   \
    }

#pragma unroll
        for (int a = 0; a < kQ; a++) {
            thr[a] = live[a] ? INFINITY : -1.0f;
            sb[a] = INFINITY;
            kbest64_reset(best[a]);
        }
        OCC_SCAN(sc.coarse_begin, sc.coarse_end)
        OCC_EMIT(sc.nscale - 1)

        for (int l = sc.nscale - 2; l >= 0; l--) {
#pragma unroll
            for (int a = 0; a < kQ; a++) {
                sb[a] = sc.seed[l] ? key_dist(best[a].k[kK - 1]) : INFINITY;
                thr[a] = live[a] ? filter_bound(sb[a]) : -1.0f;
                kbest64_reset(best[a]);
            }
            const int2 *rg = ranges + (size_t)l * sc.ncl;
            const float *rd = radius + (size_t)l * sc.ncl;
            int k_first;
            {
                const float rx = __int_as_float(__builtin_amdgcn_readfirstlane(__float_as_int(qx[0][0])));
                const float ry = __int_as_float(__builtin_amdgcn_readfirstlane(__float_as_int(qy[0][0])));
                const float rz = __int_as_float(__builtin_amdgcn_readfirstlane(__float_as_int(qz[0][0])));
                float bd = INFINITY;
                int bk = 0;
                for (int k = lane; k < sc.ncl; k += kWave) {
                    const float4 c = centers[k];
                    const float dx = rx - c.x, dy = ry - c.y, dz = rz - c.z;
                    const float d = dx * dx + dy * dy + dz * dz;
                    const bool has = rg[k].x < rg[k].y;
                    if (has && d < bd) {
                        bd = d;
                        bk = k;
                    }
                }
#pragma unroll
                for (int o = 32; o > 0; o >>= 1) {
                    const float od = __shfl_xor(bd, o);
                    const int ok = __shfl_xor(bk, o);
                    if (od < bd || (od == bd && ok < bk)) {
                        bd = od;
                        bk = ok;
                    }
                }
                k_first = __builtin_amdgcn_readfirstlane(bk);
            }
            {
                const int2 range = rg[k_first];
                OCC_SCAN(range.x, range.y)
            }
            auto in_reach = [&](const float4 c, const float r) -> bool {
                bool want = false;
#pragma unroll
                for (int h = 0; h < 2; h++) {
                    const f32x2 dx = qx[h] - c.x, dy = qy[h] - c.y, dz = qz[h] - c.z;
                    const f32x2 d2 = __builtin_elementwise_fma(dz, dz, __builtin_elementwise_fma(dy, dy, dx * dx));
#pragma unroll
                    for (int e = 0; e < 2; e++) {
                        const float lim = (sb[2 * h + e] + r) * 1.00001f;
                        want |= live[2 * h + e] && !(d2[e] > lim * lim);
                    }
                }
                return __builtin_amdgcn_ballot_w64(want) != 0;
            };
            const int ngrp = sc.ngrp > 0 ? sc.ngrp : 1;
            for (int gi = 0; gi < ngrp; gi++) {
                int k_lo = 0, k_hi = sc.ncl;
                if (sc.ngrp > 0) {
                    const float gr = gradius[(size_t)l * sc.ngrp + gi];
                    if (gr < 0.0f) continue;
                    if (!in_reach(gcenters[gi], gr)) continue;
                    const int2 gk = granges[gi];
                    k_lo = gk.x, k_hi = gk.y;
                }
                for (int k = k_lo; k < k_hi; k++) {
                    if (k == k_first) continue;
                    const int2 range = rg[k];
                    if (range.x >= range.y) continue;
                    if (!in_reach(centers[k], rd[k])) continue;
                    OCC_SCAN(range.x, range.y)
                }
            }
            OCC_EMIT(l)
        }
#undef OCC_PT4
#undef OCC_SCAN
#undef OCC_EMIT
    }
}

template <int K, int LQ>
__global__ __launch_bounds__(256) void knn_small_kernel(const float *__restrict__ q, int nq,
                                                        const float *__restrict__ s, int ns,
                                                        int32_t *__restrict__ idx) {
    const int g = threadIdx.x & (LQ - 1);
    const int i_raw = (blockIdx.x * blockDim.x + threadIdx.x) / LQ;
    const int i = i_raw < nq ? i_raw : nq - 1;
    const float qx = q[i * 3], qy = q[i * 3 + 1], qz = q[i * 3 + 2];
    double best[K];
#pragma unroll
    for (int p = 0; p < K; p++) best[p] = key64(INFINITY, 0x7fffffff);
    for (int j0 = g; j0 < ns; j0 += 4 * LQ) {
        float sx[4], sy[4], sz[4];
#pragma unroll
        for (int u = 0; u < 4; u++) {
            const int j = j0 + u * LQ < ns ? j0 + u * LQ : ns - 1;
            sx[u] = s[j * 3];
            sy[u] = s[j * 3 + 1];
            sz[u] = s[j * 3 + 2];
        }
#pragma unroll
        for (int u = 0; u < 4; u++) {
            const int j = j0 + u * LQ;
            if (j >= ns) break;
            const float dx = qx - sx[u], dy = qy - sy[u], dz = qz - sz[u];
            double t = key64(sqrtf(__fmaf_rn(dz, dz, __fmaf_rn(dy, dy, __fmul_rn(dx, dx)))), j);
            if (t < best[K - 1]) {
#pragma unroll
                for (int p = 0; p < K; p++) {
                    const double lo = fmin(best[p], t);
                    t = fmax(best[p], t);
                    best[p] = lo;
                }
            }
        }
    }
#pragma unroll
    for (int o = 1; o < LQ; o <<= 1) {
        double other[K];
#pragma unroll
        for (int p = 0; p < K; p++) other[p] = __shfl_xor(best[p], o, LQ);
#pragma unroll
        for (int e = 0; e < K; e++) {
            double t = other[e];
#pragma unroll
            for (int p = 0; p < K; p++) {
                const double lo = fmin(best[p], t);
                t = fmax(best[p], t);
                best[p] = lo;
            }
        }
    }
    if (g == 0 && i_raw < nq) {
#pragma unroll
        for (int p = 0; p < K; p++) idx[i * K + p] = key_row(best[p]);
    }
}

}

OCC_API int occnerf_msknn(const float *xyz, int64_t N, const float *points,
                          const int32_t *index_map, const int32_t *h_scale_begin,
                          const int32_t *h_seed_from_coarser, int32_t nscale, int32_t *knn_idxs,
                          void *stream) {
    using namespace occ;
    if (N <= 0) return 0;
    OCC_REQUIRE(xyz && points && index_map && h_scale_begin && knn_idxs, "msknn: null argument");
    OCC_REQUIRE(nscale >= 1 && nscale <= 4, "msknn: nscale=%d unsupported (1..4)", nscale);
    if (N <= 0) return 0;
    MsKnnScales sc;
    sc.nscale = nscale;
    for (int l = 0; l < nscale; l++) {
        sc.begin[l] = h_scale_begin[l];
        sc.end[l] = h_scale_begin[l + 1];
        OCC_REQUIRE(sc.begin[l] % 4 == 0, "msknn: scale %d must start at a multiple of 4 rows "
                    "(pad each scale with +inf rows)", l);
        OCC_REQUIRE(sc.end[l] - sc.begin[l] >= kK, "msknn: scale %d has fewer than %d points", l, kK);
        sc.seed[l] = h_seed_from_coarser ? h_seed_from_coarser[l] : 0;
    }
    const int64_t tile = 256 * kQ;
    int64_t blocks = (N + tile - 1) / tile;
    if (blocks > (int64_t)kNumCU * 8) blocks = (int64_t)kNumCU * 8;
    hipLaunchKernelGGL(msknn_kernel, dim3((unsigned)blocks), dim3(256), 0, as_stream(stream), xyz, N,
                       reinterpret_cast<const float4 *>(points), index_map, sc, knn_idxs);
    return check_launch("msknn");
}

namespace occ {
__global__ void ray_list_ranges_kernel(const int32_t *__restrict__ qrows, const int32_t *__restrict__ n_dev, int64_t n_rays,
                                       int S, int32_t *__restrict__ ray_start) {
    const int64_t r = (int64_t)blockIdx.x * blockDim.x + threadIdx.x;
    if (r > n_rays) return;
    const int32_t n = *n_dev;
    const int64_t key = r * S;
    int32_t lo = 0, hi = n;
    while (lo < hi) {
        const int32_t mid = (lo + hi) >> 1;
        if ((int64_t)qrows[mid] < key) lo = mid + 1;
        else hi = mid;
    }
    ray_start[r] = lo;
}
}

OCC_API int occnerf_knn_center(const float *c, const float *points, const int32_t *index_map,
                               const int32_t *h_scale_begin, int32_t nscale, float *center_out, int32_t *idx_out, void *stream) {
    using namespace occ;
    OCC_REQUIRE(c && points && index_map && h_scale_begin && center_out && idx_out, "knn_center: null argument");
    OCC_REQUIRE(nscale >= 1 && nscale <= 4, "knn_center: nscale=%d unsupported (1..4)", nscale);
    MsKnnScales sc;
    sc.nscale = nscale;
    for (int l = 0; l < nscale; l++) {
        sc.begin[l] = h_scale_begin[l];
        sc.end[l] = h_scale_begin[l + 1];
        sc.seed[l] = 0;
        OCC_REQUIRE(sc.end[l] - sc.begin[l] >= kK, "knn_center: scale %d has fewer than %d points", l, kK);
    }
    hipLaunchKernelGGL(knn_center_kernel, dim3(1), dim3(256), 0, as_stream(stream), c, reinterpret_cast<const float4 *>(points),
                       index_map, sc, center_out, idx_out);
    return check_launch("knn_center");
}

OCC_API int occnerf_msknn_clustered(const float *xyz, const float *mask, int64_t n_rays, int32_t samples_per_ray,
                                    const float *points,
                                    const float *centers, const int32_t *cluster_ranges,
                                    const float *cluster_radius, int32_t ncl, const float *group_centers,
                                    const int32_t *group_ranges, const float *group_radius, int32_t ngrp,
                                    const int32_t *h_coarse_rows,
                                    const int32_t *h_seed_from_coarser, int32_t nscale,
                                    const int32_t *query_rows, const int32_t *n_query_dev, int32_t *ray_start,
                                    int32_t *knn_idxs, void *stream) {
    return occnerf_msknn_clustered_centered(xyz, mask, n_rays, samples_per_ray, points, centers, cluster_ranges, cluster_radius, ncl,
                                            group_centers, group_ranges, group_radius, ngrp, h_coarse_rows, h_seed_from_coarser,
                                            nscale, query_rows, n_query_dev, ray_start, nullptr, nullptr, knn_idxs, stream);
}

OCC_API int occnerf_msknn_clustered_centered(const float *xyz, const float *mask, int64_t n_rays, int32_t samples_per_ray,
                                             const float *points,
                                             const float *centers, const int32_t *cluster_ranges,
                                             const float *cluster_radius, int32_t ncl, const float *group_centers,
                                             const int32_t *group_ranges, const float *group_radius, int32_t ngrp,
                                             const int32_t *h_coarse_rows,
                                             const int32_t *h_seed_from_coarser, int32_t nscale,
                                             const int32_t *query_rows, const int32_t *n_query_dev, int32_t *ray_start,
                                             const float *center, const int32_t *center_idx,
                                             int32_t *knn_idxs, void *stream) {
    using namespace occ;
    OCC_REQUIRE(!center == !center_idx, "msknn_clustered: center and center_idx come together (occnerf_knn_center)");
    if (n_rays <= 0 || samples_per_ray <= 0) return 0;
    OCC_REQUIRE((!query_rows && !n_query_dev && !ray_start) || (query_rows && n_query_dev && ray_start),
                "msknn_clustered: query_rows, n_query_dev and the ray_start scratch come together");
    OCC_REQUIRE(!(query_rows && mask), "msknn_clustered: a query list replaces the mask");
    OCC_REQUIRE(xyz && points && centers && cluster_ranges && cluster_radius && h_coarse_rows && knn_idxs,
                "msknn_clustered: null argument");
    OCC_REQUIRE(nscale >= 2 && nscale <= 4, "msknn_clustered: nscale=%d unsupported (2..4)", nscale);
    OCC_REQUIRE(ncl >= 1, "msknn_clustered: ncl=%d", ncl);
    OCC_REQUIRE((ngrp == 0 && !group_centers && !group_ranges && !group_radius) ||
                    (ngrp > 0 && group_centers && group_ranges && group_radius),
                "msknn_clustered: group_centers, group_ranges, group_radius and ngrp come together");
    ClusteredScales sc;
    sc.nscale = nscale;
    sc.ncl = ncl;
    sc.ngrp = ngrp;
    sc.coarse_begin = h_coarse_rows[0];
    sc.coarse_end = h_coarse_rows[1];
    OCC_REQUIRE(sc.coarse_begin % 4 == 0 && (sc.coarse_end - sc.coarse_begin) % 4 == 0 &&
                    sc.coarse_end - sc.coarse_begin >= kK, "msknn_clustered: bad coarse row range");
    for (int l = 0; l < 4; l++) {
        sc.seed[l] = (l < nscale && h_seed_from_coarser) ? h_seed_from_coarser[l] : 0;
    }
    const int64_t tiles = ((n_rays + 63) / 64) * ((samples_per_ray + 3) / 4);
    OCC_REQUIRE(tiles < (1ll << 31), "msknn_clustered: too many tiles for one launch");
    const bool split = tiles <= (int64_t)kNumCU * 12 * 4;
    int64_t blocks = ((split ? 4 * tiles : tiles) + 3) / 4;
    if (blocks > (int64_t)kNumCU * 3) blocks = (int64_t)kNumCU * 3;
    constexpr int kTicketLines = 1024;
    static std::mutex mu;
    static std::map<int, unsigned *> pools;
    static std::map<std::pair<int, void *>, unsigned *> lines;
    int dev = 0;
    OCC_REQUIRE(hipGetDevice(&dev) == hipSuccess && dev >= 0, "msknn_clustered: device id");
    unsigned *ticket;
    {
        std::lock_guard<std::mutex> lock(mu);
        unsigned *&pool = pools[dev];
        if (!pool)
            OCC_REQUIRE(hipMalloc(&pool, kTicketLines * 64) == hipSuccess,
                        "msknn_clustered: hipMalloc of the ticket lines (the first call must not be inside a stream capture)");
        auto it = lines.find(std::make_pair(dev, stream));
        if (it == lines.end()) {
            int used = 0;
            for (auto &kv : lines) used += kv.first.first == dev;
            OCC_REQUIRE(used < kTicketLines, "msknn_clustered: more than %d streams on device %d", kTicketLines, dev);
            it = lines.emplace(std::make_pair(dev, stream), pool + 16 * used).first;
        }
        ticket = it->second;
    }
    OCC_REQUIRE(hipMemsetAsync(ticket, 0, sizeof(unsigned), as_stream(stream)) == hipSuccess, "msknn_clustered: memset");
    if (query_rows)
        hipLaunchKernelGGL(ray_list_ranges_kernel, dim3((unsigned)((n_rays + 256) / 256)), dim3(256), 0, as_stream(stream),
                           query_rows, n_query_dev, n_rays, samples_per_ray, ray_start);
    auto kern = split ? msknn_clustered_kernel<true> : msknn_clustered_kernel<false>;
    hipLaunchKernelGGL(kern, dim3((unsigned)blocks), dim3(256), 0, as_stream(stream), xyz, mask,
                       n_rays, samples_per_ray, reinterpret_cast<const float4 *>(points),
                       reinterpret_cast<const float4 *>(centers), reinterpret_cast<const int2 *>(cluster_ranges),
                       cluster_radius, reinterpret_cast<const float4 *>(group_centers),
                       reinterpret_cast<const int2 *>(group_ranges), group_radius, sc, knn_idxs, ticket, query_rows, ray_start,
                       center, center_idx, kSplitExtent2);
    return check_launch("msknn_clustered");
}

OCC_API int occnerf_knn_small(const float *q, int32_t nq, const float *s, int32_t ns, int32_t k,
                              int32_t *idx, void *stream) {
    using namespace occ;
    if (nq <= 0) return 0;
    OCC_REQUIRE(q && s && idx, "knn_small: null argument");
    OCC_REQUIRE(ns >= k, "knn_small: fewer support points (%d) than k (%d)", ns, k);
    if (nq <= 0) return 0;
    hipStream_t st = as_stream(stream);
    const bool wide = ns >= 1024 && nq <= (1 << 20);
    const dim3 block(64), grid(wide ? nq : (nq + 7) / 8);
#define OCC_KS(KK)                                                                                      \
    case KK:                                                                                            \
        if (wide) hipLaunchKernelGGL((knn_small_kernel<KK, 64>), grid, block, 0, st, q, nq, s, ns, idx); \
        else hipLaunchKernelGGL((knn_small_kernel<KK, 8>), grid, block, 0, st, q, nq, s, ns, idx);       \
        break;
    switch (k) {
        OCC_KS(1)
        OCC_KS(3)
        OCC_KS(10)
        OCC_KS(16)
        default: set_error("knn_small: k=%d not built (1, 3, 10, 16)", k); return 1;
    }
#undef OCC_KS
    return check_launch("knn_small");
}
```

### occnerf_amd/network.py

```python
import os

import numpy as np
import torch
import torch.nn as nn

from . import geometry, ops
from .canonical_mlp import CanonicalMLP
from .config import get_cfg
from .rayorder import ray_patch_order
from .modules import (BodyPoseRefiner, MotionBasisComputer, MotionWeightVolumeDecoder,
                      NonRigidMotionMLP, hann_window_weights)


class _Replica(nn.Module):

    def __init__(self, module):
        super().__init__()
        self.module = module

    def forward(self, *a, **k):
        return self.module(*a, **k)


def _load_smpl(cfg):
    choice = cfg.get('smpl_model', 'auto')
    model_dir = './third_parties/smpl/models' if choice in ('auto', 'synthetic') else choice
    pkl = os.path.join(model_dir, 'basicModel_neutral_lbs_10_207_0_v1.0.0.pkl')
    if choice != 'synthetic' and os.path.exists(pkl):
        from third_parties.smpl.smpl_numpy import SMPL
        return SMPL(sex='neutral', model_dir=model_dir)
    from .synth import SyntheticSMPL
    return SyntheticSMPL()


class Network(nn.Module):
    def __init__(self, avg_betas=None):
        super().__init__()
        cfg = get_cfg()
        self.cfg = cfg
        self.motion_basis_computer = MotionBasisComputer(total_bones=cfg.total_bones)
        self.mweight_vol_decoder = MotionWeightVolumeDecoder(
            embedding_size=cfg.mweight_volume.embedding_size,
            volume_size=cfg.mweight_volume.volume_size, total_bones=cfg.total_bones)
        nr = cfg.non_rigid_motion_mlp
        self.non_rigid_mlp = _Replica(NonRigidMotionMLP(
            pos_embed_size=nr.multires * 6, condition_code_size=nr.condition_code_size,
            mlp_width=nr.mlp_width, mlp_depth=nr.mlp_depth, skips=nr.skips))
        self.pose_decoder = BodyPoseRefiner(
            embedding_size=cfg.pose_decoder.embedding_size, mlp_width=cfg.pose_decoder.mlp_width,
            mlp_depth=cfg.pose_decoder.mlp_depth, total_bones=cfg.total_bones)
        self._ctx = None
        self._ray_orders = {}
        self._wconst = None
        self._packed = None

    def generate_neural_points(self, avg_betas):
        cfg = self.cfg
        self.smpl = _load_smpl(cfg)
        betas = np.zeros(10) if avg_betas is None else np.asarray(avg_betas)
        verts, joints = self.smpl(np.zeros(72,), betas)
        try:
            import trimesh
            normals = np.asarray(trimesh.Trimesh(vertices=verts, faces=self.smpl.faces, process=False,
                                                 maintain_order=True).vertex_normals)
        except ImportError:
            normals = geometry.vertex_normals(verts, self.smpl.faces)
        min_xyz = np.min(joints, axis=0) - cfg.bbox_offset
        max_xyz = np.max(joints, axis=0) + cfg.bbox_offset
        self.bound = np.max(np.abs(list(min_xyz) + list(max_xyz)))
        self.detailed_bound = torch.tensor(np.array([list(min_xyz), list(max_xyz)]))

        self.point_base = nn.Parameter(torch.tensor(verts).float(), requires_grad=False)
        self.point_dist = nn.Parameter(torch.zeros(verts.shape[0], 1).float(), requires_grad=True)
        self.point_dist.data.uniform_(-1e-4, 1e-4)
        self.point_counter = nn.Parameter(torch.ones(verts.shape[0]), requires_grad=False)
        self.point_norms = torch.tensor(normals)

        self.fps_index, ratio = [], 1.0
        for _ in range(3):
            ratio /= 4
            self.fps_index.append(torch.from_numpy(geometry.farthest_point_sampling(verts, ratio)))

        self.cnl_mlp = _Replica(CanonicalMLP(
            mlp_depth=cfg.canonical_mlp.mlp_depth, mlp_width=cfg.canonical_mlp.mlp_width,
            input_ch=63, skips=[], bound=self.bound, detailed_bound=self.detailed_bound))
        self._ctx = self._packed = self._wconst = None

    def deploy_mlps_to_secondary_gpus(self):
        return self

    @property
    def point_cloud(self):
        return self.point_base + self.point_dist

    def _f16x3_flag_word(self):
        w = self.__dict__.get('_f16x3_word')
        if w is None or w.device != self.point_base.device:
            w = self.__dict__['_f16x3_word'] = torch.zeros(1, device=self.point_base.device, dtype=torch.int32)
        return w

    def _f16x3_enqueue_check(self, flag, what):
        self._frames_rendered = getattr(self, '_frames_rendered', 0) + 1
        host = torch.empty(1, dtype=torch.int32, pin_memory=True)
        host.copy_(flag, non_blocking=True)
        flag.zero_()
        done = torch.cuda.Event()
        done.record(torch.cuda.current_stream(flag.device))
        self.__dict__.setdefault('_f16x3_pending', []).append((done, host, f'{what} {self._frames_rendered}'))

    def check_f16x3_domain(self, wait=True):
        pending = self.__dict__.get('_f16x3_pending')
        while pending:
            done, host, frame_no = pending[0]
            if not wait and not done.query():
                return
            done.synchronize()
            pending.pop(0)
            if int(host[0]) != 0:
                pending.clear()
                raise RuntimeError(f"occnerf_amd: {frame_no} of this Network left the domain of the f16x3 kernels (a hidden activation "
                                   'reached 4 094): its results are not fp32-grade -- use mlp_precision=\'fp32\' / '
                                   "train_nonrigid_f16x3=False (a render with cfg.f16x3_domain_check=True falls back by itself, at the "
                                   'price of one wait per frame)')

    def invalidate_cache(self):
        self._ctx = self._packed = self._wconst = None
        self._ray_orders = {}
        self.__dict__.pop('_per_step_graph', None)

    def load_state_dict(self, *a, **k):
        out = super().load_state_dict(*a, **k)
        self.invalidate_cache()
        return out

    def _apply(self, fn, *a, **k):
        out = super()._apply(fn, *a, **k)
        self.invalidate_cache()
        return out

    def _context(self):
        dev = self.point_base.device
        if self._ctx is not None and self._ctx['device'] == dev:
            return self._ctx
        base = self.point_base.detach()
        P = base.shape[0]
        sets = [torch.arange(P)] + [f.long() for f in self.fps_index]
        rows, imap, begin = [], [], [0]
        for idx in sets:
            pts = base[idx.to(dev)]
            pad = (-pts.shape[0]) % 4
            rows.append(torch.cat([pts, torch.full((pad, 3), float('inf'), device=dev)]))
            imap.append(torch.cat([idx, torch.zeros(pad, dtype=idx.dtype)]))
            begin.append(begin[-1] + pts.shape[0] + pad)
        pts4 = torch.cat(rows)
        pts4 = torch.cat([pts4, torch.zeros(pts4.shape[0], 1, device=dev)], dim=1).contiguous()
        as_sets = [set(s.tolist()) for s in sets]
        seed = [int(l + 1 < len(sets) and as_sets[l + 1] <= as_sets[l]) for l in range(len(sets))]
        normals = self.point_norms.to(dev).double().contiguous()
        cl = geometry.build_knn_clusters(base.cpu().numpy(), [s.numpy() for s in sets])
        clusters = {k: (torch.from_numpy(np.ascontiguousarray(v)).to(dev) if k in
                        ('points', 'index_map', 'centers', 'ranges', 'radius', 'group_centers', 'group_ranges', 'group_radius') else v)
                    for k, v in cl.items()}
        self._ctx = {
            'clusters': clusters,
            'device': dev, 'points': pts4, 'index_map': torch.cat(imap).int().to(dev),
            'scale_begin': begin, 'seed': seed, 'normals': normals,
            'unit': ops.unit_normals(normals),
            'bound32': float(np.float32(self.bound)),
            'two_bound32': float(np.float32(2 * np.float64(self.bound))),
        }
        return self._ctx

    def _packed_weights(self):
        cm, nr = self.cnl_mlp.module, self.non_rigid_mlp.module
        nr_lin = [m for m in nr.block_mlps if isinstance(m, nn.Linear)]
        cw, cb = cm.linear_params()
        prec = str(self.cfg.get('mlp_precision', 'fp32'))
        if prec not in ('fp32', 'bf16x3', 'f16x3'):
            raise RuntimeError(f"cfg.mlp_precision must be 'fp32', 'f16x3' or 'bf16x3', got {prec!r}")
        pack_c = {'bf16x3': ops.canonical_mlp_pack_bf16, 'f16x3': ops.canonical_mlp_pack_f16}.get(prec)
        pack_n = {'bf16x3': ops.nonrigid_pack_bf16, 'f16x3': ops.nonrigid_pack_f16}.get(prec)
        srcs = cw + cb + [m.weight for m in nr_lin] + [m.bias for m in nr_lin]
        key = (prec, str(self.cfg.get('f16x3_domain_check', True))) + tuple((t.data_ptr(), t._version) for t in srcs)
        if self._packed is not None and self._packed['key'] == key:
            return self._packed
        self._packed = {
            'key': key,
            'cnl': ops.canonical_mlp_pack(cw, cb),
            'cnl_bf16': pack_c(cw) if pack_c else None,
            'nr': ops.nonrigid_pack([m.weight.detach() for m in nr_lin],
                                    [m.bias.detach() for m in nr_lin]),
            'nr_bf16': pack_n([m.weight.detach() for m in nr_lin]) if pack_n else None,
            'nr_w0': nr_lin[0].weight.detach(), 'nr_b0': nr_lin[0].bias.detach(),
            'domain_flag': torch.zeros(1, device=cw[0].device, dtype=torch.int32)
            if (prec == 'f16x3' and self.cfg.get('f16x3_domain_check', True)) else None,
        }
        return self._packed

    def _weight_constants(self):
        dec_mod = self.mweight_vol_decoder
        enc = self.cnl_mlp.module.encoder
        srcs = list(dec_mod.parameters()) + [self.point_dist, self.point_base, enc.embeddings]
        key = tuple((t.data_ptr(), t._version) for t in srcs)
        if self._wconst is not None and self._wconst['key'] == key:
            return self._wconst
        with torch.no_grad():
            dec = dec_mod.decoder.forward_gemm(dec_mod.const_embedding[None])[0].contiguous()
            table = self._point_stage(self._context())
        self._wconst = {'key': key, 'dec': dec, 'table': table}
        return self._wconst

    def _point_pack(self, wc):
        srcs = [self.point_counter, self.point_base]
        key = (wc['table'].data_ptr(),) + tuple((t.data_ptr(), t._version) for t in srcs)
        if wc.get('pack_key') != key:
            ctx = self._context()
            wc['pack'] = ops.point_pack(self.point_base.detach(), ctx['normals'], ctx['unit'],
                                        self.point_counter.detach(), wc['table'])
            wc['pack_key'] = key
        return wc['pack']

    def _point_stage(self, ctx):
        enc = self.cnl_mlp.module.encoder
        pc = self.point_cloud.detach().float().contiguous()
        base = self.point_base.detach()
        kidx = ops.knn_small(pc, base, 3)
        knn_base, sdf = ops.point_sdf(pc, base, ctx['normals'], ctx['unit'], kidx)
        table = ops.point_table(knn_base, sdf, pc, ctx['bound32'], ctx['two_bound32'],
                                enc.embeddings.detach(), enc.offsets, enc.log2_per_level_scale,
                                enc.base_resolution)
        return table

    def _stage_features(self, rays8, z, xyz, mask, pk, cond, hann, table, pack, center=None):
        cfg, ctx = self.cfg, self._context()
        S = int(cfg.N_samples)
        enc = self.cnl_mlp.module.encoder
        rows, count = ops.live_rows(mask)
        self.last_live_count = count
        dedup = bool(cfg.get('dedup_repeated_samples', True))
        scan_a = scan_b = mrows = mcount = None
        frows, fcount, kmask = rows, count, mask
        if not cfg.ignore_non_rigid_motions:
            if pk['nr_bf16'] is not None:
                ops.nonrigid_bf16x3_rows(xyz, rows, count, cond, hann, pk['nr_w0'], pk['nr_b0'], pk['nr'], pk['nr_bf16'],
                                         domain_flag=pk['domain_flag'])
            else:
                ops.nonrigid_rows(xyz, rows, count, cond, hann, pk['nr_w0'], pk['nr_b0'], pk['nr'])
        if dedup:
            scan_a, frows, fcount, kmask = ops.repeat_heads(xyz, 3, count, rows=rows,
                                                            want_mask=not cfg.get('knn_query_list', True))
            if cfg.get('dedup_global_positions', False):
                frows, fcount = ops.unique_heads(xyz, 3, frows, fcount, scan=scan_a, scan_count=count)
        self.last_head_counts = (fcount, None)
        if cfg.get('knn_query_list', True):
            knn = ops.msknn_clustered(xyz, rays8.shape[0], S, ctx['clusters'], ctx['seed'], rows=frows, count=fcount, center=center)
        else:
            knn = ops.msknn_clustered(xyz, rays8.shape[0], S, ctx['clusters'], ctx['seed'], mask=kmask, center=center)
        if center is not None and len(center) > 3 and center[3] != self._center_stamp(table):
            raise RuntimeError('stale kNN centre: its cached feature row was computed from another table / counter / embedding '
                               'version than this frame\'s (ops.sample_features freshness contract)')
        mlp_in, raw_c, _ = ops.sample_features(
            xyz, knn, self.point_base.detach(), ctx['normals'], ctx['unit'],
            self.point_counter.detach(), table, ctx['bound32'], ctx['two_bound32'],
            enc.embeddings.detach(), enc.offsets, enc.log2_per_level_scale, enc.base_resolution,
            rows=frows, count=fcount, pack=pack, center=None if center is None else center[0],
            center_agg=None if center is None else center[2])
        del knn
        if dedup:
            scan_b, mrows, mcount, _ = ops.repeat_heads(mlp_in, 68, fcount)
            if cfg.get('dedup_global', True):
                mrows, mcount = ops.unique_heads(mlp_in, 68, mrows, mcount, scan=scan_b, scan_count=fcount)
            self.last_head_counts = (fcount, mcount)
        return {'dedup': dedup, 'rays8': rays8, 'z': z, 'mask': mask, 'rows': rows, 'count': count, 'mlp_in': mlp_in,
                'raw_c': raw_c, 'scan_a': scan_a, 'scan_b': scan_b, 'mrows': mrows, 'mcount': mcount, 'cnl': pk['cnl'],
                'cnl_bf16': pk['cnl_bf16'], 'domain_flag': pk['domain_flag'], 'N': xyz.shape[0]}

    @staticmethod
    def _stage_mlp_composite(st, bgcolor, out, out_rows):
        dev, N = st['mlp_in'].device, st['N']

        def mlp(raw_out, count, in_rows=None):
            if st['cnl_bf16'] is not None:
                ops.canonical_mlp_bf16x3(st['mlp_in'], st['cnl'], st['cnl_bf16'], raw_out, count=count, in_rows=in_rows,
                                         domain_flag=st['domain_flag'])
            else:
                ops.canonical_mlp(st['mlp_in'], st['cnl'], raw_out, count=count, in_rows=in_rows)
        if st['dedup']:
            raw_h = torch.empty(st['mlp_in'].shape[0], 5, device=dev)
            mlp(raw_h, st['mcount'], st['mrows'])
            raw = ops.scatter_raw_heads(raw_h, st['raw_c'], st['rows'], st['count'], st['scan_a'], st['scan_b'],
                                        torch.zeros(N, 5, device=dev))
        else:
            mlp(st['raw_c'], st['count'])
            raw = ops.scatter_raw(st['raw_c'], st['rows'], st['count'], torch.zeros(N, 5, device=dev))
        st['mlp_in'] = None
        return ops.composite(raw, st['mask'], st['z'], st['rays8'], bgcolor, out=out, out_rows=out_rows)[:3]

    def _nonrigid_f16_pack(self):
        pk = self._packed_weights()
        if pk.get('nr_f16_train') is None:
            nr_lin = [m for m in self.non_rigid_mlp.module.block_mlps if isinstance(m, nn.Linear)]
            pk['nr_f16_train'] = pk['nr_bf16'] if (pk['nr_bf16'] is not None and pk['nr_bf16'].dtype == torch.float16) else \
                ops.nonrigid_pack_f16([m.weight.detach() for m in nr_lin])
        return pk['nr_f16_train']

    def _knn_center_lists(self, cond, hann):
        ctx, pk = self._context(), self._packed_weights()
        c = torch.zeros(64, 3, device=self.point_base.device)
        if not self.cfg.ignore_non_rigid_motions:
            c = ops.nonrigid(c, cond, hann, pk['nr_w0'], pk['nr_b0'], pk['nr'], direct=True)
        return ops.knn_center(c[0].contiguous(), ctx['points'], ctx['index_map'], ctx['scale_begin'])

    def _knn_center(self, cond, hann, table, pack):
        ctx, pk = self._context(), self._packed_weights()
        c = torch.zeros(64, 3, device=self.point_base.device)
        if not self.cfg.ignore_non_rigid_motions:
            c = ops.nonrigid(c, cond, hann, pk['nr_w0'], pk['nr_b0'], pk['nr'], direct=True)
        center, idx = ops.knn_center(c[0].contiguous(), ctx['points'], ctx['index_map'], ctx['scale_begin'])
        enc = self.cnl_mlp.module.encoder
        row, _, enc_in = ops.sample_features(
            c[:8].contiguous(), idx[None].expand(8, -1, -1).contiguous(), self.point_base.detach(), ctx['normals'], ctx['unit'],
            self.point_counter.detach(), table, ctx['bound32'], ctx['two_bound32'], enc.embeddings.detach(), enc.offsets,
            enc.log2_per_level_scale, enc.base_resolution, pack=pack, want_enc_in=True)
        return center, idx, ops.center_row(row[0], enc_in[0]), self._center_stamp(table)

    def _center_stamp(self, table):
        return (table.data_ptr(), table._version, self.point_counter._version, self.cnl_mlp.module.encoder.embeddings._version)

    def _render_rays(self, rays8, Rs, Ts, vol, bbox_min, bbox_scale, bgcolor, cond, hann,
                     table, t_rand=None, out=None, out_rows=None, pack=None, boxes=None, center=None):
        cfg, ctx = self.cfg, self._context()
        S = int(cfg.N_samples)
        enc = self.cnl_mlp.module.encoder
        t_vals = torch.linspace(0., 1., steps=S, device=rays8.device)
        z, xyz, mask, _ = ops.sample_warp(rays8, S, t_vals, Rs, Ts, vol, bbox_min, bbox_scale,
                                          t_rand=t_rand, boxes=boxes)
        pk = self._packed_weights()
        N = xyz.shape[0]
        if cfg.get('skip_empty_samples', True) and cfg.get('knn_culling', True):
            st = self._stage_features(rays8, z, xyz, mask, pk, cond, hann, table, pack, center)
            return self._stage_mlp_composite(st, bgcolor, out, out_rows)

        if not cfg.ignore_non_rigid_motions:
            if pk['nr_bf16'] is not None:
                ops.nonrigid_bf16x3(xyz, cond, hann, pk['nr_w0'], pk['nr_b0'], pk['nr'], pk['nr_bf16'], out=xyz, domain_flag=pk['domain_flag'])
            else:
                ops.nonrigid(xyz, cond, hann, pk['nr_w0'], pk['nr_b0'], pk['nr'], out=xyz)
        if cfg.get('knn_culling', True):
            knn = ops.msknn_clustered(xyz, rays8.shape[0], S, ctx['clusters'], ctx['seed'], center=center)
        else:
            knn = ops.msknn(xyz, ctx['points'], ctx['index_map'], ctx['scale_begin'], ctx['seed'])
        mlp_in, raw, _ = ops.sample_features(
            xyz, knn, self.point_base.detach(), ctx['normals'], ctx['unit'],
            self.point_counter.detach(), table, ctx['bound32'], ctx['two_bound32'],
            enc.embeddings.detach(), enc.offsets, enc.log2_per_level_scale, enc.base_resolution, pack=pack)
        del knn
        if pk['cnl_bf16'] is not None:
            ops.canonical_mlp_bf16x3(mlp_in, pk['cnl'], pk['cnl_bf16'], raw, domain_flag=pk['domain_flag'])
        else:
            ops.canonical_mlp(mlp_in, pk['cnl'], raw)
        del mlp_in
        return ops.composite(raw, mask, z, rays8, bgcolor, out=out, out_rows=out_rows)[:3]

    @staticmethod
    def _ray_patch_order(rays_d):
        return ray_patch_order(rays_d)

    @staticmethod
    def _host3(v):
        return ops.host_float3(v)

    @torch.no_grad()
    def live_samples_per_ray(self, rays, dst_Rs, dst_Ts, cnl_gtfms, motion_weights_priors, dst_posevec=None,
                             near=None, far=None, iter_val=1e7, **kwargs):
        cfg, dev = self.cfg, self.point_base.device
        f32 = lambda t: t.detach().float().contiguous().to(dev)
        wc = self._weight_constants()
        refine = iter_val >= cfg.pose_decoder.get('kick_in_iter', 0)
        Rs, Ts = ops.pose_motion_bases(self.pose_decoder, f32(dst_posevec).reshape(-1), refine, f32(dst_Rs), f32(dst_Ts),
                                       f32(cnl_gtfms))
        vol = ops.prior_softmax(wc['dec'], f32(motion_weights_priors))
        rays8 = ops.pack_rays(f32(rays).reshape(2, -1, 3), f32(near).reshape(-1), f32(far).reshape(-1), None)
        S = int(cfg.N_samples)
        t_vals = torch.linspace(0., 1., steps=S, device=dev)
        boxes = ops.bone_boxes(vol, Rs.shape[0]) if cfg.get('warp_bone_culling', True) else None
        _, _, mask, _ = ops.sample_warp(rays8, S, t_vals, Rs, Ts, vol, self._host3(kwargs['cnl_bbox_min_xyz']),
                                        self._host3(kwargs['cnl_bbox_scale_xyz']), boxes=boxes)
        return (mask.view(-1, S) != 0).sum(dim=1)

    @torch.no_grad()
    def render_preamble(self, data, iter_val=1e7):
        f32 = lambda t: t.detach().float().contiguous().to(self.point_base.device)
        wc = self._weight_constants()
        refine = iter_val >= self.cfg.pose_decoder.get('kick_in_iter', 0)
        Rs, Ts = ops.pose_motion_bases(self.pose_decoder, f32(data['dst_posevec']).reshape(-1), refine, f32(data['dst_Rs']),
                                       f32(data['dst_Ts']), f32(data['cnl_gtfms']))
        return Rs, Ts, ops.prior_softmax(wc['dec'], f32(data['motion_weights_priors']))

    def forward(self, rays, dst_Rs, dst_Ts, cnl_gtfms, motion_weights_priors, dst_posevec=None,
                near=None, far=None, iter_val=1e7, **kwargs):
        cfg = self.cfg
        dev = self.point_base.device
        if dev.type != 'cuda':
            raise RuntimeError('occnerf_amd.Network renders on a GPU only; move the module with '
                               '.cuda() first (the reference has no CPU path either)')
        dst_Rs, dst_Ts = dst_Rs[None], dst_Ts[None]
        dst_posevec, cnl_gtfms = dst_posevec[None], cnl_gtfms[None]
        motion_weights_priors = motion_weights_priors[None]
        want_grad = torch.is_grad_enabled()
        fused = not want_grad and not self.training
        R = int(near.numel())
        shape = list(rays[1].shape[:-1])
        if R == 0:
            z = torch.zeros(0, device=dev)
            return {'rgb': z.reshape(shape + [3]), 'alpha': z.reshape(shape), 'depth': z.reshape(shape),
                    'comp_loss': torch.zeros(0 if self.training else 1, device=dev)}

        nr = cfg.non_rigid_motion_mlp
        hann = hann_window_weights(nr.multires, iter_val, nr.kick_in_iter, nr.full_band_iter)
        refine = iter_val >= cfg.pose_decoder.get('kick_in_iter', 0)
        bbox_min = self._host3(kwargs['cnl_bbox_min_xyz'])
        bbox_scale = self._host3(kwargs['cnl_bbox_scale_xyz'])
        bgcolor = self._host3(kwargs['bgcolor'])
        S = int(cfg.N_samples)
        rays_o, rays_d = rays

        def morton_order(dirs):
            if not cfg.get('ray_patch_order', True):
                return None
            key = kwargs.get('ray_order_key')
            hit = self._ray_orders.get(key) if key is not None else None
            if hit is not None and hit.numel() == R and hit.device == dirs.device:
                return hit
            order = self._ray_patch_order(dirs)
            if key is not None:
                if len(self._ray_orders) >= 8:
                    self._ray_orders.clear()
                self._ray_orders[key] = order
            return order

        if fused:
            self.check_f16x3_domain(wait=False)
            with torch.no_grad():
                wc = self._weight_constants()
                pack = self._point_pack(wc)
                f32 = lambda t: t.detach().float().contiguous()
                cond = f32(dst_posevec).reshape(-1) if iter_val >= nr.kick_in_iter else \
                    torch.zeros(dst_posevec.numel(), device=dev)
                center = None
                if cfg.get('knn_center_cache', True) and cfg.get('knn_culling', True):
                    center = self._knn_center(cond, hann.tolist(), wc['table'], pack)
                Rs, Ts = ops.pose_motion_bases(self.pose_decoder, f32(dst_posevec).reshape(-1), refine, f32(dst_Rs[0]),
                                               f32(dst_Ts[0]), f32(cnl_gtfms[0]))
                vol = ops.prior_softmax(wc['dec'], f32(motion_weights_priors[0]))
                boxes = ops.bone_boxes(vol, Rs.shape[0]) if cfg.get('warp_bone_culling', True) else None
                rays_f = f32(torch.stack([rays_o.reshape(-1, 3), rays_d.reshape(-1, 3)]) if not torch.is_tensor(rays) else
                             rays.reshape(2, -1, 3))
                order = morton_order(rays_f[1])
                rays8 = ops.pack_rays(rays_f, f32(near).reshape(-1), f32(far).reshape(-1), order)
                out = (torch.empty(R, 3, device=dev), torch.empty(R, device=dev), torch.empty(R, device=dev))
                cap = int(cfg.get('max_samples_per_pass', 1 << 28))
                if R * S > (1 << 26):
                    free = (torch.cuda.mem_get_info(dev)[0] + torch.cuda.memory_reserved(dev)
                            - torch.cuda.memory_allocated(dev))
                    cap = min(cap, max(1 << 22, int(free // 2 // 470)))
                rays_per_pass = max(1, cap // S)

                def passes():
                    for i in range(0, R, rays_per_pass):
                        n = min(rays_per_pass, R - i)
                        if order is not None:
                            self._render_rays(rays8[i:i + n], Rs, Ts, vol, bbox_min, bbox_scale, bgcolor, cond, hann.tolist(),
                                              wc['table'], out=out, out_rows=order[i:i + n], pack=pack, boxes=boxes, center=center)
                        else:
                            self._render_rays(rays8[i:i + n], Rs, Ts, vol, bbox_min, bbox_scale, bgcolor, cond, hann.tolist(),
                                              wc['table'], out=tuple(t[i:i + n] for t in out), pack=pack, boxes=boxes, center=center)
                passes()
                mode = cfg.get('f16x3_domain_check', True)
                flag = self._packed_weights().get('domain_flag') if (R > 0 and mode) else None
                if flag is not None and mode == 'deferred':
                    self._f16x3_enqueue_check(flag, 'frame')
                elif flag is not None and int(flag.item()) != 0:
                    flag.zero_()
                    self.f16x3_fallback_frames = getattr(self, 'f16x3_fallback_frames', 0) + 1
                    if self.f16x3_fallback_frames == 1:
                        import warnings
                        warnings.warn("occnerf_amd: a hidden activation left the domain of cfg.mlp_precision='f16x3' (>= 4 094); "
                                      'this frame -- and every later one that does -- is rendered again with the fp32 kernels')
                    prec0 = cfg.mlp_precision
                    cfg.mlp_precision = 'fp32'
                    try:
                        passes()
                    finally:
                        cfg.mlp_precision = prec0
                rgb, acc, depth = out
                comp_loss = torch.zeros(1, device=dev)
        else:
            from . import train_path
            self.check_f16x3_domain(wait=False)
            with torch.set_grad_enabled(want_grad):
                with torch.autocast('cuda', enabled=False):
                    dst_Rs, dst_Ts, cnl_gtfms = dst_Rs.float(), dst_Ts.float(), cnl_gtfms.float()
                    dst_posevec = dst_posevec.float()
                    cond = dst_posevec if iter_val >= nr.kick_in_iter else torch.zeros_like(dst_posevec)
                    static = None
                    if want_grad and cfg.get('train_graph', True):
                        from . import train_graph
                        static = train_graph.get(self)(refine, dst_posevec, dst_Rs, dst_Ts, cnl_gtfms, motion_weights_priors)
                    if static is not None:
                        Rs, Ts, vol, knn_base, point_sdf = static
                    else:
                        Rs, Ts = train_path.motion_bases(self, refine, dst_posevec, dst_Rs, dst_Ts, cnl_gtfms)
                        vol = self.mweight_vol_decoder(motion_weights_priors=motion_weights_priors.float())[0]
                        knn_base, point_sdf = train_path.point_sdf_block(self)
                rays8 = torch.cat([rays_o.reshape(-1, 3).float(), rays_d.reshape(-1, 3).float(),
                                   near.reshape(-1, 1).float(), far.reshape(-1, 1).float()], -1)
                order = morton_order(rays8[:, 3:6])
                rays8 = (rays8[order] if order is not None else rays8).contiguous()
                t_rand = kwargs.get('t_rand')
                if t_rand is not None and order is not None:
                    t_rand = t_rand[order]
                outs = []
                for i in range(0, rays8.shape[0], int(cfg.chunk)):
                    outs.append(train_path.render_rays_autograd(
                        self, rays8[i:i + cfg.chunk], Rs, Ts, vol, bbox_min, bbox_scale, bgcolor, cond.float(),
                        hann.tolist(), None if t_rand is None else t_rand[i:i + cfg.chunk], point_block=(knn_base, point_sdf)))
                rgb, acc, depth, comp_loss = (torch.cat(t, 0) if len(outs) > 1 else outs[0][j]
                                              for j, t in enumerate(zip(*outs)))
                if order is not None:
                    inv = torch.empty_like(order)
                    inv[order] = torch.arange(order.numel(), device=order.device)
                    rgb, acc, depth = rgb[inv], acc[inv], depth[inv]
                    if comp_loss.shape[0] == order.numel():
                        comp_loss = comp_loss[inv]
        return {'rgb': rgb.reshape(shape + [3]), 'alpha': acc.reshape(shape),
                'depth': depth.reshape(shape),
                'comp_loss': comp_loss.reshape(-1)}
```

### occnerf_amd/ops.py

```python
import ctypes as C

import numpy as np
import torch

from . import _lib

_f32p = C.POINTER(C.c_float)


def _chk(t, dtype, name):
    if not torch.is_tensor(t):
        raise RuntimeError(f'{name} must be a tensor')
    if not t.is_cuda:
        raise RuntimeError(f'{name} must be a CUDA(HIP) tensor; there is no CPU path')
    if not t.is_contiguous():
        raise RuntimeError(f'{name} must be a contiguous tensor')
    if t.dtype != dtype:
        raise RuntimeError(f'{name} must be {dtype}, got {t.dtype}')
    return t.data_ptr()


def _guard_dev(dev):
    if torch.device(dev).type != 'cuda':
        raise RuntimeError(f'tensors are on {dev}: this path runs on a GPU only, there is no CPU path')
# ... 108 lines not shown
        args = [_chk(grad, dt, 'grad'), _chk(inputs, torch.float32, 'inputs'), _chk(embeddings, dt, 'embeddings'),
                _chk(offsets, torch.int32, 'offsets')]
        if fp32:
            args.append(_host_offsets(offsets))
        args += [_chk(grad_embeddings, dt, 'grad_embeddings'), int(B), int(D), int(Cc), int(L), float(S), int(H),
                 _opt(dy_dx, dt, 'dy_dx'), _opt(grad_inputs, dt, 'grad_inputs'), int(gridtype), int(bool(align_corners)),
                 int(interp)]
        if fp32:
            args += [None if scratch is None else scratch.data_ptr(), 0 if scratch is None else scratch.numel() * 8]
        rc = getattr(_lib.lib(), 'occnerf_grid_encode_backward' + _ENCODER_ENTRY[dt])(*args, _stream(inputs))
    _lib.check(rc, 'grid_encode_backward')


def grad_total_variation(inputs, embeddings, grad, offsets, weight, B, D, Cc, L, S, H, gridtype=0,
                         align_corners=False):
    rc = _lib.lib().occnerf_grad_total_variation(None, None, None, None, float(weight), int(B), int(D),
                                                 int(Cc), int(L), float(S), int(H), int(gridtype),
                                                 int(bool(align_corners)), None)
    _lib.check(rc, 'grad_total_variation')


def _host_f64(vals, n):
    a = np.ascontiguousarray(np.asarray(vals, dtype=np.float64).ravel())
    assert a.size == n, (a.size, n)
    return a, a.ctypes.data_as(C.c_void_p)


def gen_rays(K, E, H, W, bbox_min, bbox_max, device, out=None):
    dev = torch.device(device)
    if dev.type != 'cuda':
        raise RuntimeError(f'gen_rays: needs a GPU device, got {dev}')
    f32 = int(np.asarray(K).dtype == np.float32 and np.asarray(E).dtype == np.float32)
    E = np.asarray(E, dtype=np.float64)
    k0, pk = _host_f64(np.linalg.inv(np.asarray(K)).astype(np.float64), 9)
    r0, pr = _host_f64(E[:3, :3], 9)
    t0, pt = _host_f64(E[:3, 3], 3)
    l0, pl = _host_f64(bbox_min, 3)
    h0, ph = _host_f64(bbox_max, 3)
    if out is None:
        rays8 = torch.empty(H * W, 8, device=dev, dtype=torch.float32)
        mask = torch.empty(H * W, device=dev, dtype=torch.uint8)
    else:
        rays8, mask = out
        _chk(rays8, torch.float32, 'rays8'), _chk(mask, torch.uint8, 'mask')
        if rays8.numel() != H * W * 8 or mask.numel() != H * W or rays8.device != mask.device:
            raise RuntimeError(f'gen_rays: out must be rays8[{H * W},8] and mask[{H * W}] on one device')
    with _guard_dev(rays8.device):
        rc = _lib.lib().occnerf_gen_rays(pk, pr, pt, f32, int(H), int(W), pl, ph, rays8.data_ptr(),
                                         mask.data_ptr(), _stream(rays8))
    _lib.check(rc, 'gen_rays')
    return rays8, mask


def bone_boxes(vol, nb):
    boxes = torch.empty(nb, 6, device=vol.device, dtype=torch.int32)
    with _guard(vol):
        rc = _lib.lib().occnerf_bone_boxes(_chk(vol, torch.float32, 'vol'), int(nb), int(vol.shape[-1]), boxes.data_ptr(), _stream(vol))
    _lib.check(rc, 'bone_boxes')
    return boxes


def sample_warp(rays8, S, t_vals, Rs, Ts, vol, bbox_min, bbox_scale, t_rand=None, want_pts=False, boxes=None):
    n = rays8.shape[0]
    dev = rays8.device
    if boxes is not None and t_rand is None and not want_pts:
        z = torch.empty(n, S, device=dev, dtype=torch.float32)
        xs = torch.empty(n * S, 3, device=dev, dtype=torch.float32)
        mk = torch.empty(n * S, device=dev, dtype=torch.float32)
        _kmin, pmin = _host_f32(bbox_min, 3)
        _ksc, psc = _host_f32(bbox_scale, 3)
        with _guard_dev(dev):
            rc = _lib.lib().occnerf_sample_warp_culled(
                _chk(rays8, torch.float32, 'rays'), n, int(S), _chk(t_vals, torch.float32, 't_vals'),
                _chk(Rs, torch.float32, 'Rs'), _chk(Ts, torch.float32, 'Ts'), _chk(vol, torch.float32, 'vol'), int(Rs.shape[0]),
                int(vol.shape[-1]), _chk(boxes, torch.int32, 'boxes'), pmin, psc, z.data_ptr(), xs.data_ptr(), mk.data_ptr(),
                _stream(rays8))
        _lib.check(rc, 'sample_warp_culled')
        return z, xs, mk, None
    z = torch.empty(n, S, device=dev, dtype=torch.float32)
    xs = torch.empty(n * S, 3, device=dev, dtype=torch.float32)
    mk = torch.empty(n * S, device=dev, dtype=torch.float32)
    pts = torch.empty(n * S, 3, device=dev, dtype=torch.float32) if want_pts else None
    _kmin, pmin = _host_f32(bbox_min, 3)
    _ksc, psc = _host_f32(bbox_scale, 3)
    with _guard_dev(dev):
        rc = _lib.lib().occnerf_sample_warp(
            _chk(rays8, torch.float32, 'rays'), n, int(S), _chk(t_vals, torch.float32, 't_vals'),
            _opt(t_rand, torch.float32, 't_rand'), _chk(Rs, torch.float32, 'Rs'),
            _chk(Ts, torch.float32, 'Ts'), _chk(vol, torch.float32, 'vol'), int(Rs.shape[0]),
            int(vol.shape[-1]), pmin, psc, z.data_ptr(), None if pts is None else pts.data_ptr(),
            xs.data_ptr(), mk.data_ptr(), _stream(rays8))
    _lib.check(rc, 'sample_warp')
    return z, xs, mk, pts


def nonrigid_pack(weights, biases):
    dev = weights[0].device
    n = _lib.lib().occnerf_nonrigid_packed_floats()
    packed = torch.zeros(n, device=dev, dtype=torch.float32)
    with _guard_dev(dev):
        rc = _lib.lib().occnerf_nonrigid_pack(_ptr_table(weights, 'W'), _ptr_table(biases, 'b'),
                                              packed.data_ptr(), _stream(packed))
    _lib.check(rc, 'nonrigid_pack')
    return packed


def nonrigid(xyz, cond, hann, W0, b0, packed, out=None, direct=False):
    out = torch.empty_like(xyz) if out is None else out
    _kh, ph = _host_f32(hann, 6)
    fn = _lib.lib().occnerf_nonrigid_direct if direct else _lib.lib().occnerf_nonrigid
    with _guard(xyz):
        rc = fn(
            _chk(xyz, torch.float32, 'xyz'), xyz.shape[0], _chk(cond, torch.float32, 'cond'), ph,
            _chk(W0, torch.float32, 'W0'), _chk(b0, torch.float32, 'b0'),
            _chk(packed, torch.float32, 'packed'), _chk(out, torch.float32, 'xyz_out'), _stream(xyz))
    _lib.check(rc, 'nonrigid')
    return out


def nonrigid_rows(xyz, rows, count, cond, hann, W0, b0, packed):
    _kh, ph = _host_f32(hann, 6)
    with _guard(xyz):
        rc = _lib.lib().occnerf_nonrigid_rows(
            _chk(xyz, torch.float32, 'xyz'), rows.shape[0], _chk(rows, torch.int32, 'rows'),
            _chk(count, torch.int32, 'count'), _chk(cond, torch.float32, 'cond'), ph,
            _chk(W0, torch.float32, 'W0'), _chk(b0, torch.float32, 'b0'), _chk(packed, torch.float32, 'packed'),
            _stream(xyz))
    _lib.check(rc, 'nonrigid_rows')
    return xyz


def live_rows(mask):
    N = mask.shape[0]
    dev = mask.device
    nbytes = int(_lib.lib().occnerf_live_rows_temp_bytes(N))
    if nbytes < 0:
        raise RuntimeError('live_rows: temp size query failed')
    temp = torch.empty(max(nbytes, 16), device=dev, dtype=torch.uint8)
    rows = torch.empty(N, device=dev, dtype=torch.int32)
    count = torch.empty(1, device=dev, dtype=torch.int32)
    with _guard(mask):
        rc = _lib.lib().occnerf_live_rows(_chk(mask, torch.float32, 'mask'), N, rows.data_ptr(), count.data_ptr(),
                                          temp.data_ptr(), nbytes, _stream(mask))
    _lib.check(rc, 'live_rows')
    return rows, count


def scatter_raw(raw_c, rows, count, raw_full):
    with _guard(raw_c):
        rc = _lib.lib().occnerf_scatter_raw(_chk(raw_c, torch.float32, 'raw_c'), _chk(rows, torch.int32, 'rows'),
                                            _chk(count, torch.int32, 'count'), rows.shape[0],
                                            _chk(raw_full, torch.float32, 'raw_full'), _stream(raw_c))
    _lib.check(rc, 'scatter_raw')
    return raw_full


def repeat_heads(keys, key_cols, count, rows=None, want_mask=False):
    dev = keys.device
    if keys.dim() != 2 or not keys.is_contiguous() or keys.element_size() != 4:
        raise RuntimeError('repeat_heads: keys must be a contiguous [M, C] tensor of 4-byte elements')
    cap = keys.shape[0] if rows is None else rows.shape[0]
    scan = torch.empty(cap, device=dev, dtype=torch.int32)
    heads = torch.empty(cap, device=dev, dtype=torch.int32)
    head_count = torch.empty(1, device=dev, dtype=torch.int32)
    head_mask = torch.zeros(keys.shape[0], device=dev, dtype=torch.float32) if want_mask else None
    if cap == 0:
        head_count.zero_()
        return scan, heads, head_count, head_mask
    nbytes = int(_lib.lib().occnerf_repeat_heads_temp_bytes(cap))
    if nbytes < 0:
        raise RuntimeError('repeat_heads: temp size query failed')
    temp = torch.empty(max(nbytes, 16), device=dev, dtype=torch.uint8)
    with _guard_dev(dev):
        rc = _lib.lib().occnerf_repeat_heads(
            keys.data_ptr(), keys.shape[1], int(key_cols), _opt(rows, torch.int32, 'rows'),
            _chk(count, torch.int32, 'count'), cap, scan.data_ptr(), heads.data_ptr(), head_count.data_ptr(),
            None if head_mask is None else head_mask.data_ptr(), temp.data_ptr(), nbytes, _stream(keys))
    _lib.check(rc, 'repeat_heads')
    return scan, heads, head_count, head_mask


def unique_heads(keys, key_cols, heads, count, scan=None, scan_count=None):
    dev = keys.device
    if keys.dim() != 2 or not keys.is_contiguous() or keys.element_size() != 4:
        raise RuntimeError('unique_heads: keys must be a contiguous [M, C] tensor of 4-byte elements')
    cap = keys.shape[0] if heads is None else heads.shape[0]
    heads_out = torch.empty(cap, device=dev, dtype=torch.int32)
    count_out = torch.empty(1, device=dev, dtype=torch.int32)
    if cap == 0:
        count_out.zero_()
        return heads_out, count_out
    nbytes = int(_lib.lib().occnerf_unique_heads_temp_bytes(cap))
    if nbytes <= 0:
        raise RuntimeError('unique_heads: temp size query failed')
    temp = torch.empty(nbytes, device=dev, dtype=torch.uint8)
    with _guard_dev(dev):
        rc = _lib.lib().occnerf_unique_heads(
            keys.data_ptr(), keys.shape[1], int(key_cols), _opt(heads, torch.int32, 'heads'),
            _chk(count, torch.int32, 'count'), cap, heads_out.data_ptr(), count_out.data_ptr(),
            _opt(scan, torch.int32, 'scan'), _opt(scan_count, torch.int32, 'scan_count'),
            0 if scan is None else scan.shape[0], temp.data_ptr(), nbytes, _stream(keys))
    _lib.check(rc, 'unique_heads')
    return heads_out, count_out


def scatter_raw_heads(raw_h, raw_c, rows, count, scan_a, scan_b, raw_full):
    with _guard(raw_c):
        rc = _lib.lib().occnerf_scatter_raw_heads(
            _chk(raw_h, torch.float32, 'raw_h'), _chk(raw_c, torch.float32, 'raw_c'), _chk(rows, torch.int32, 'rows'),
            _chk(count, torch.int32, 'count'), _opt(scan_a, torch.int32, 'scan_a'), _opt(scan_b, torch.int32, 'scan_b'),
            rows.shape[0], _chk(raw_full, torch.float32, 'raw_full'), _stream(raw_c))
    _lib.check(rc, 'scatter_raw_heads')
    return raw_full


def nonrigid_pack_bf16(weights):
    dev = weights[0].device
    n = _lib.lib().occnerf_nonrigid_packed_bf16_bytes()
    packed = torch.zeros(n // 2, device=dev, dtype=torch.bfloat16)
    with _guard_dev(dev):
        rc = _lib.lib().occnerf_nonrigid_pack_bf16(_ptr_table(weights[:6], 'W'), packed.data_ptr(), _stream(packed))
    _lib.check(rc, 'nonrigid_pack_bf16')
    return packed


def nonrigid_pack_f16(weights):
    dev = weights[0].device
    n = _lib.lib().occnerf_nonrigid_packed_bf16_bytes()
    packed = torch.zeros(n // 2, device=dev, dtype=torch.float16)
    with _guard_dev(dev):
        rc = _lib.lib().occnerf_nonrigid_pack_f16(_ptr_table(weights[:6], 'W'), packed.data_ptr(), _stream(packed))
    _lib.check(rc, 'nonrigid_pack_f16')
    return packed


def _nonrigid_f16x3(xyz, rows, count, cond, hann, W0, b0, packed, packed_f16, out, domain_flag=None):
    _kh, ph = _host_f32(hann, 6)
    n_max = xyz.shape[0] if rows is None else rows.shape[0]
    with _guard(xyz):
        rc = _lib.lib().occnerf_nonrigid_f16x3(
            _chk(xyz, torch.float32, 'xyz'), n_max, _opt(rows, torch.int32, 'rows'), _opt(count, torch.int32, 'count'),
            _chk(cond, torch.float32, 'cond'), ph, _chk(W0, torch.float32, 'W0'), _chk(b0, torch.float32, 'b0'),
            _chk(packed, torch.float32, 'packed'), _chk(packed_f16, torch.float16, 'packed_f16'),
            _chk(out, torch.float32, 'xyz_out'), _opt(domain_flag, torch.int32, 'domain_flag'), _stream(xyz))
    _lib.check(rc, 'nonrigid_f16x3')
    return out


def nonrigid_bf16x3(xyz, cond, hann, W0, b0, packed, packed_bf16, out=None, domain_flag=None):
    out = torch.empty_like(xyz) if out is None else out
    if packed_bf16.dtype == torch.float16:
        return _nonrigid_f16x3(xyz, None, None, cond, hann, W0, b0, packed, packed_bf16, out, domain_flag)
    _kh, ph = _host_f32(hann, 6)
    with _guard(xyz):
        rc = _lib.lib().occnerf_nonrigid_bf16x3(
            _chk(xyz, torch.float32, 'xyz'), xyz.shape[0], _chk(cond, torch.float32, 'cond'), ph,
            _chk(W0, torch.float32, 'W0'), _chk(b0, torch.float32, 'b0'), _chk(packed, torch.float32, 'packed'),
            _chk(packed_bf16, torch.bfloat16, 'packed_bf16'), _chk(out, torch.float32, 'xyz_out'), _stream(xyz))
    _lib.check(rc, 'nonrigid_bf16x3')
    return out


def nonrigid_bf16x3_rows(xyz, rows, count, cond, hann, W0, b0, packed, packed_bf16, domain_flag=None):
    if packed_bf16.dtype == torch.float16:
        return _nonrigid_f16x3(xyz, rows, count, cond, hann, W0, b0, packed, packed_bf16, xyz, domain_flag)
    _kh, ph = _host_f32(hann, 6)
    with _guard(xyz):
        rc = _lib.lib().occnerf_nonrigid_bf16x3_rows(
            _chk(xyz, torch.float32, 'xyz'), rows.shape[0], _chk(rows, torch.int32, 'rows'), _chk(count, torch.int32, 'count'),
            _chk(cond, torch.float32, 'cond'), ph, _chk(W0, torch.float32, 'W0'), _chk(b0, torch.float32, 'b0'),
            _chk(packed, torch.float32, 'packed'), _chk(packed_bf16, torch.bfloat16, 'packed_bf16'), _stream(xyz))
    _lib.check(rc, 'nonrigid_bf16x3_rows')
    return xyz


def msknn(xyz, points, index_map, scale_begin, seed_from_coarser):
    N = xyz.shape[0]
    nscale = len(scale_begin) - 1
    out = torch.empty(N, nscale, 10, device=xyz.device, dtype=torch.int32)
    _kb, pb = _host_i32(scale_begin)
    _ks, ps = _host_i32(seed_from_coarser)
    with _guard(xyz):
        rc = _lib.lib().occnerf_msknn(_chk(xyz, torch.float32, 'xyz'), N,
                                      _chk(points, torch.float32, 'points'),
                                      _chk(index_map, torch.int32, 'index_map'), pb, ps, nscale,
                                      out.data_ptr(), _stream(xyz))
    _lib.check(rc, 'msknn')
    return out


def knn_center(c, points, index_map, scale_begin):
    nscale = len(scale_begin) - 1
    center = torch.empty(4, device=c.device, dtype=torch.float32)
    idx = torch.empty(nscale, 10, device=c.device, dtype=torch.int32)
    _kb, pb = _host_i32(scale_begin)
    with _guard(c):
        rc = _lib.lib().occnerf_knn_center(_chk(c, torch.float32, 'c'), _chk(points, torch.float32, 'points'),
                                           _chk(index_map, torch.int32, 'index_map'), pb, nscale, center.data_ptr(), idx.data_ptr(),
                                           _stream(c))
    _lib.check(rc, 'knn_center')
    return center, idx


def msknn_clustered(xyz, n_rays, S, cl, seed_from_coarser, mask=None, rows=None, count=None, out=None, center=None):
    nscale = int(cl['ranges'].shape[0]) + 1
    if out is None:
        out = torch.empty(n_rays * S, nscale, 10, device=xyz.device, dtype=torch.int32)
    if (rows is None) != (count is None) or (rows is not None and mask is not None):
        raise RuntimeError('msknn_clustered: rows and count come together, instead of mask')
    ray_start = torch.empty(n_rays + 1, device=xyz.device, dtype=torch.int32) if rows is not None else None
    _kc, pc = _host_i32(cl['coarse_rows'])
    _ks, ps = _host_i32(seed_from_coarser)
    with _guard(xyz):
        rc = _lib.lib().occnerf_msknn_clustered_centered(
            _chk(xyz, torch.float32, 'xyz'), _opt(mask, torch.float32, 'mask'), int(n_rays), int(S),
            _chk(cl['points'], torch.float32, 'points'), _chk(cl['centers'], torch.float32, 'centers'), _chk(cl['ranges'], torch.int32, 'cluster_ranges'),
            _chk(cl['radius'], torch.float32, 'cluster_radius'), int(cl['ncl']),
            _opt(cl.get('group_centers'), torch.float32, 'group_centers'), _opt(cl.get('group_ranges'), torch.int32, 'group_ranges'),
            _opt(cl.get('group_radius'), torch.float32, 'group_radius'), int(cl.get('ngrp', 0)), pc, ps, nscale,
            _opt(rows, torch.int32, 'rows'), _opt(count, torch.int32, 'count'),
            None if ray_start is None else ray_start.data_ptr(),
            None if center is None else _chk(center[0], torch.float32, 'center'),
            None if center is None else _chk(center[1], torch.int32, 'center_idx'), out.data_ptr(), _stream(xyz))
    _lib.check(rc, 'msknn_clustered')
    return out


def knn_small(q, s, k):
    out = torch.empty(q.shape[0], k, device=q.device, dtype=torch.int32)
    with _guard(q):
        rc = _lib.lib().occnerf_knn_small(_chk(q, torch.float32, 'q'), q.shape[0],
                                          _chk(s, torch.float32, 's'), s.shape[0], int(k),
                                          out.data_ptr(), _stream(q))
    _lib.check(rc, 'knn_small')
    return out


def unit_normals(normals):
    out = torch.empty_like(normals)
    with _guard(normals):
        rc = _lib.lib().occnerf_unit_normals(_chk(normals, torch.float64, 'normals'), normals.shape[0],
                                             out.data_ptr(), _stream(normals))
    _lib.check(rc, 'unit_normals')
    return out


def point_sdf(point_cloud, point_base, normals, unit, kidx):
    P = point_cloud.shape[0]
    kb = torch.empty(P, 3, device=point_cloud.device, dtype=torch.float64)
    dist = torch.empty(P, device=point_cloud.device, dtype=torch.float32)
    with _guard(point_cloud):
        rc = _lib.lib().occnerf_point_sdf(
            _chk(point_cloud, torch.float32, 'point_cloud'), _chk(point_base, torch.float32, 'point_base'),
            _chk(normals, torch.float64, 'normals'), _chk(unit, torch.float64, 'unit_normals'),
            _chk(kidx, torch.int32, 'kidx'), P, kb.data_ptr(), dist.data_ptr(), _stream(point_cloud))
    _lib.check(rc, 'point_sdf')
    return kb, dist


def table_stride():
    return int(_lib.lib().occnerf_point_table_stride())


def point_table(knn_base, sdf, learnable, bound32, two_bound32, embeddings, offsets, S, H):
    P = knn_base.shape[0]
    table = torch.empty(P, table_stride(), device=knn_base.device, dtype=torch.float32)
    with _guard(knn_base):
        rc = _lib.lib().occnerf_point_table(
            _chk(knn_base, torch.float64, 'knn_base'), _chk(sdf, torch.float32, 'point_sdf'),
            _chk(learnable, torch.float32, 'learnable'), P, float(bound32), float(two_bound32),
            _chk(embeddings, torch.float32, 'embeddings'), _chk(offsets, torch.int32, 'offsets'),
            _host_offsets(offsets), int(offsets.shape[0] - 1), float(S), int(H), table.data_ptr(),
            _stream(knn_base))
    _lib.check(rc, 'point_table')
    return table


def point_pack(point_base, normals, unit, counter, table):
    P, dev = point_base.shape[0], point_base.device
    geo = torch.empty(P, 16, device=dev, dtype=torch.float32)
    tail = torch.empty(P, 4, device=dev, dtype=torch.float32)
    with _guard_dev(dev):
        rc = _lib.lib().occnerf_point_pack(
            _chk(point_base, torch.float32, 'point_base'), _chk(normals, torch.float64, 'normals'),
            _chk(unit, torch.float64, 'unit_normals'), _chk(counter, torch.float32, 'counter'),
            _chk(table, torch.float32, 'table'), P, geo.data_ptr(), tail.data_ptr(), _stream(point_base))
    _lib.check(rc, 'point_pack')
    return geo, tail


def center_row(mlp_in_row, enc_in_row):
    return torch.cat([mlp_in_row[:36], enc_in_row[:4], mlp_in_row[36:68]]).contiguous()


def sample_features(xyz, knn_idxs, point_base, normals, unit, counter, table, bound32, two_bound32,
                    embeddings, offsets, S, H, raw=None, want_enc_in=False, geo_idxs=None,
                    att_in=None, rows=None, count=None, pack=None, center=None, center_agg=None):
    N = xyz.shape[0] if rows is None else rows.shape[0]
    dev = xyz.device
    if (pack is None and N > 0 and knn_idxs.shape[1] == 4 and geo_idxs is None and att_in is None
            and counter is not None and table.dim() == 2 and table.shape[1] == table_stride()):
        pack = point_pack(point_base, normals, unit, counter, table)
    geo, tail = pack if pack is not None else (None, None)
    if table.dim() != 2 or table.shape[1] != table_stride():
        raise RuntimeError(f'sample_features: table must be [P,{table_stride()}] (ops.point_table), got {tuple(table.shape)}')
    mlp_in = torch.empty(N, 68, device=dev, dtype=torch.float32)
    raw = torch.empty(N, 5, device=dev, dtype=torch.float32) if raw is None else raw
    enc_in = torch.empty(N, 4, device=dev, dtype=torch.float32) if want_enc_in else None
    with _guard_dev(dev):
        rc = _lib.lib().occnerf_sample_features_centered(
            _chk(xyz, torch.float32, 'xyz'), N, _chk(knn_idxs, torch.int32, 'knn_idxs'),
            int(knn_idxs.shape[1]), _chk(point_base, torch.float32, 'point_base'),
            _chk(normals, torch.float64, 'normals'), _chk(unit, torch.float64, 'unit_normals'),
            _opt(counter, torch.float32, 'counter'), _chk(table, torch.float32, 'table'),
            float(bound32), float(two_bound32), _chk(embeddings, torch.float32, 'embeddings'),
            _chk(offsets, torch.int32, 'offsets'), _host_offsets(offsets), int(offsets.shape[0] - 1),
            float(S), int(H), _opt(geo_idxs, torch.int32, 'geo_idxs'), _opt(att_in, torch.float32, 'att_in'),
            _opt(rows, torch.int32, 'rows'), _opt(count, torch.int32, 'count'),
            _opt(geo, torch.float32, 'point_geo'), _opt(tail, torch.float32, 'point_tail'),
            0 if geo is None else int(geo.shape[0]),
            _opt(center, torch.float32, 'center'), _opt(center_agg, torch.float32, 'center_agg'),
            mlp_in.data_ptr(), _chk(raw, torch.float32, 'raw'),
            None if enc_in is None else enc_in.data_ptr(), _stream(xyz))
    _lib.check(rc, 'sample_features')
    return mlp_in, raw, enc_in


def canonical_mlp_pack(weights, biases):
    dev = weights[0].device
    n = _lib.lib().occnerf_canonical_mlp_packed_floats()
    packed = torch.zeros(n, device=dev, dtype=torch.float32)
    with _guard_dev(dev):
        rc = _lib.lib().occnerf_canonical_mlp_pack(_ptr_table(weights, 'W'), _ptr_table(biases, 'b'),
                                                   packed.data_ptr(), _stream(packed))
    _lib.check(rc, 'canonical_mlp_pack')
    return packed


def canonical_mlp(mlp_in, packed, raw, direct=False, count=None, in_rows=None):
    if in_rows is not None:
        with _guard(mlp_in):
            rc = _lib.lib().occnerf_canonical_mlp_rows(
                _chk(mlp_in, torch.float32, 'mlp_in'), _chk(in_rows, torch.int32, 'in_rows'), in_rows.shape[0],
                _chk(count, torch.int32, 'count'), _chk(packed, torch.float32, 'packed'),
                _chk(raw, torch.float32, 'raw'), _stream(mlp_in))
        _lib.check(rc, 'canonical_mlp_rows')
        return raw
    if count is not None:
        with _guard(mlp_in):
            rc = _lib.lib().occnerf_canonical_mlp_counted(
                _chk(mlp_in, torch.float32, 'mlp_in'), mlp_in.shape[0], _chk(count, torch.int32, 'count'),
                _chk(packed, torch.float32, 'packed'), _chk(raw, torch.float32, 'raw'), _stream(mlp_in))
        _lib.check(rc, 'canonical_mlp_counted')
        return raw
    fn = _lib.lib().occnerf_canonical_mlp_direct if direct else _lib.lib().occnerf_canonical_mlp
    with _guard(mlp_in):
        rc = fn(_chk(mlp_in, torch.float32, 'mlp_in'), mlp_in.shape[0], _chk(packed, torch.float32, 'packed'),
                _chk(raw, torch.float32, 'raw'), _stream(mlp_in))
    _lib.check(rc, 'canonical_mlp')
    return raw


def trunks_pack_bf16(weights, out=None):
    dev = weights[0].device
    if out is None:
        out = torch.zeros(_lib.lib().occnerf_trunks_packed_bytes() // 2, device=dev, dtype=torch.bfloat16)
    with _guard_dev(dev):
        rc = _lib.lib().occnerf_trunks_pack_bf16(_ptr_table(weights[:9], 'W'), out.data_ptr(), _stream(out))
    _lib.check(rc, 'trunks_pack_bf16')
    return out


def trunks_forward_bf16(agg, var, enc, packed_f32, packed_bf16):
    M, dev, bf = agg.shape[0], agg.device, torch.bfloat16
    X0 = torch.empty(M, 96, device=dev, dtype=bf)
    A = [torch.empty(M, 256, device=dev, dtype=bf) for _ in range(4)]
    GEO = torch.empty(M, 96, device=dev, dtype=bf)
    B = [torch.empty(M, 256, device=dev, dtype=bf) for _ in range(4)]
    raw4 = torch.empty(M, 4, device=dev, dtype=torch.float32)
    pa = (C.c_void_p * 4)(*[t.data_ptr() for t in A])
    pb = (C.c_void_p * 4)(*[t.data_ptr() for t in B])
    with _guard(agg):
        rc = _lib.lib().occnerf_trunks_forward_bf16(
            _chk(agg, torch.float32, 'agg'), _chk(var, torch.float32, 'var'), _chk(enc, torch.float32, 'enc'), M,
            _chk(packed_f32, torch.float32, 'packed_f32'), _chk(packed_bf16, torch.bfloat16, 'packed_bf16'), X0.data_ptr(), pa,
            GEO.data_ptr(), pb, raw4.data_ptr(), _stream(agg))
    _lib.check(rc, 'trunks_forward_bf16')
    return X0, A, GEO, B, raw4


def canonical_mlp_pack_bf16(weights):
    dev = weights[0].device
    n = _lib.lib().occnerf_canonical_mlp_packed_bf16_bytes()
    packed = torch.zeros(n // 2, device=dev, dtype=torch.bfloat16)
    with _guard_dev(dev):
        rc = _lib.lib().occnerf_canonical_mlp_pack_bf16(_ptr_table(weights, 'W'), packed.data_ptr(),
                                                        _stream(packed))
    _lib.check(rc, 'canonical_mlp_pack_bf16')
    return packed


def canonical_mlp_pack_f16(weights):
    dev = weights[0].device
    n = _lib.lib().occnerf_canonical_mlp_packed_bf16_bytes()
    packed = torch.zeros(n // 2, device=dev, dtype=torch.float16)
    with _guard_dev(dev):
        rc = _lib.lib().occnerf_canonical_mlp_pack_f16(_ptr_table(weights, 'W'), packed.data_ptr(), _stream(packed))
    _lib.check(rc, 'canonical_mlp_pack_f16')
    return packed


def canonical_mlp_bf16x3(mlp_in, packed, packed_bf16, raw, variant=0, count=None, in_rows=None, domain_flag=None):
    if packed_bf16.dtype == torch.float16:
        n_max = mlp_in.shape[0] if in_rows is None else in_rows.shape[0]
        with _guard(mlp_in):
            rc = _lib.lib().occnerf_canonical_mlp_f16x3(
                _chk(mlp_in, torch.float32, 'mlp_in'), _opt(in_rows, torch.int32, 'in_rows'), n_max,
                _opt(count, torch.int32, 'count'), _chk(packed, torch.float32, 'packed'),
                _chk(packed_bf16, torch.float16, 'packed_f16'), _chk(raw, torch.float32, 'raw'),
                _opt(domain_flag, torch.int32, 'domain_flag'), _stream(mlp_in))
        _lib.check(rc, 'canonical_mlp_f16x3')
        return raw
    with _guard(mlp_in):
        if count is None:
            assert in_rows is None
            rc = _lib.lib().occnerf_canonical_mlp_bf16x3(
                _chk(mlp_in, torch.float32, 'mlp_in'), mlp_in.shape[0], _chk(packed, torch.float32, 'packed'),
                _chk(packed_bf16, torch.bfloat16, 'packed_bf16'), _chk(raw, torch.float32, 'raw'),
                int(variant), _stream(mlp_in))
        else:
            n_max = mlp_in.shape[0] if in_rows is None else in_rows.shape[0]
            rc = _lib.lib().occnerf_canonical_mlp_bf16x3_rows(
                _chk(mlp_in, torch.float32, 'mlp_in'), _opt(in_rows, torch.int32, 'in_rows'), n_max,
                _chk(count, torch.int32, 'count'), _chk(packed, torch.float32, 'packed'),
                _chk(packed_bf16, torch.bfloat16, 'packed_bf16'), _chk(raw, torch.float32, 'raw'), int(variant),
                _stream(mlp_in))
    _lib.check(rc, 'canonical_mlp_bf16x3')
    return raw


def composite(raw, mask, z_vals, rays8, bgcolor, want_weights=False, want_term=False, out=None, out_rows=None):
    n, S = z_vals.shape
    dev = raw.device
    if out is None:
        if out_rows is not None:
            raise RuntimeError('composite: out_rows needs caller-allocated outputs')
        out = (torch.empty(n, 3, device=dev, dtype=torch.float32), torch.empty(n, device=dev, dtype=torch.float32),
               torch.empty(n, device=dev, dtype=torch.float32))
    rgb, acc, dep = out
    for t, nm in ((rgb, 'rgb'), (acc, 'acc'), (dep, 'depth')):
        _chk(t, torch.float32, nm)
    w = torch.empty(n, S, device=dev, dtype=torch.float32) if want_weights else None
    tp = torch.empty(n, device=dev, dtype=torch.int32) if want_term else None
    _kbg, pbg = _host_f32(bgcolor, 3)
    with _guard_dev(dev):
        rc = _lib.lib().occnerf_composite(
            _chk(raw, torch.float32, 'raw'), _chk(mask, torch.float32, 'mask'),
            _chk(z_vals, torch.float32, 'z_vals'), _chk(rays8, torch.float32, 'rays'), pbg, n, int(S),
            rgb.data_ptr(), acc.data_ptr(), dep.data_ptr(), None if w is None else w.data_ptr(),
            None if tp is None else tp.data_ptr(), _opt(out_rows, torch.int64, 'out_rows'), _stream(raw))
    _lib.check(rc, 'composite')
    return rgb, acc, dep, w, tp


def pose_motion_bases(pose_decoder, posevec, refine, dst_Rs, dst_Ts, cnl_gtfms):
    import torch.nn as nn
    dev = dst_Rs.device
    lin = [m for m in pose_decoder.block_mlps if isinstance(m, nn.Linear)]
    if len(lin) != 5 or lin[0].in_features != 69 or lin[0].out_features != 256 or lin[4].out_features != 69:
        raise RuntimeError('pose_motion_bases: the fused kernel is built for the 69 -> 256 x4 -> 69 refiner of occnerf.yaml')
    Rs = torch.empty(24, 3, 3, device=dev, dtype=torch.float32)
    Ts = torch.empty(24, 3, device=dev, dtype=torch.float32)
    with _guard_dev(dev):
        rc = _lib.lib().occnerf_pose_motion_bases(
            _ptr_table([m.weight.detach() for m in lin], 'W'), _ptr_table([m.bias.detach() for m in lin], 'b'),
            _chk(posevec, torch.float32, 'posevec'), int(bool(refine)), _chk(dst_Rs, torch.float32, 'dst_Rs'),
            _chk(dst_Ts, torch.float32, 'dst_Ts'), _chk(cnl_gtfms, torch.float32, 'cnl_gtfms'), Rs.data_ptr(),
            Ts.data_ptr(), _stream(dst_Rs))
    _lib.check(rc, 'pose_motion_bases')
    return Rs, Ts


def prior_softmax(decoded, prior):
    Cn = decoded.shape[0]
    V = decoded.numel() // Cn
    vol = torch.empty_like(decoded)
    with _guard(decoded):
        rc = _lib.lib().occnerf_prior_softmax(_chk(decoded, torch.float32, 'decoded'), _chk(prior, torch.float32, 'prior'),
                                              int(Cn), int(V), vol.data_ptr(), _stream(decoded))
    _lib.check(rc, 'prior_softmax')
    return vol


def ray_order(dirs):
    R = dirs.shape[0]
    order = torch.empty(R, device=dirs.device, dtype=torch.int64)
    if R == 0:
        return order
    if not dirs.is_cuda or dirs.dtype != torch.float32 or dirs.dim() != 2 or dirs.shape[1] != 3 or dirs.stride(1) != 1:
        raise RuntimeError('ray_order: dirs must be a float32 [R,3] GPU tensor with unit element stride')
    nbytes = int(_lib.lib().occnerf_ray_order_temp_bytes(R))
    if nbytes < 0:
        raise RuntimeError('ray_order: temp size query failed')
    temp = torch.empty(nbytes, device=dirs.device, dtype=torch.uint8)
    with _guard(dirs):
        rc = _lib.lib().occnerf_ray_order(dirs.data_ptr(), R, int(dirs.stride(0)), order.data_ptr(), temp.data_ptr(), nbytes,
                                          _stream(dirs))
    _lib.check(rc, 'ray_order')
    return order


def pack_rays(rays, near, far, order=None):
    R = rays.shape[1]
    rays8 = torch.empty(R, 8, device=rays.device, dtype=torch.float32)
    with _guard(rays):
        rc = _lib.lib().occnerf_pack_rays(_chk(rays, torch.float32, 'rays'), _chk(near, torch.float32, 'near'),
                                          _chk(far, torch.float32, 'far'), _opt(order, torch.int64, 'order'), R,
                                          rays8.data_ptr(), _stream(rays))
    _lib.check(rc, 'pack_rays')
    return rays8


def agg_forward(feats, knn, atts):
    N, K = knn.shape
    F = feats.shape[1]
    agg = torch.empty(N, F, device=feats.device, dtype=torch.float32)
    with _guard(feats):
        rc = _lib.lib().occnerf_agg_forward(_chk(feats, torch.float32, 'feats'), int(F), _chk(knn, torch.int32, 'knn'),
                                            _chk(atts, torch.float32, 'atts'), N, int(K), agg.data_ptr(), _stream(feats))
    _lib.check(rc, 'agg_forward')
    return agg


def agg_backward(grad_agg, knn, atts, P):
    N, K = knn.shape
    F = grad_agg.shape[1]
    W = int(_lib.lib().occnerf_agg_backward_slices(N))
    partial = torch.empty(W, P, F, device=grad_agg.device, dtype=torch.float32)
    nbytes = int(_lib.lib().occnerf_agg_backward_scratch_bytes(N, int(F)))
    scratch = torch.empty(max(nbytes, 16), device=grad_agg.device, dtype=torch.uint8)
    with _guard(grad_agg):
        rc = _lib.lib().occnerf_agg_backward(_chk(grad_agg, torch.float32, 'grad_agg'), int(F),
                                             _chk(knn, torch.int32, 'knn'), _chk(atts, torch.float32, 'atts'), N,
                                             int(K), int(P), partial.data_ptr(), scratch.data_ptr(), nbytes,
                                             _stream(grad_agg))
    _lib.check(rc, 'agg_backward')
    return partial.sum(0)


class _Aggregate(torch.autograd.Function):
    @staticmethod
    def forward(ctx, feats, knn, atts):
        feats = feats.contiguous()
        ctx.save_for_backward(knn, atts)
        ctx.P = feats.shape[0]
        return agg_forward(feats, knn, atts)

    @staticmethod
    def backward(ctx, grad_agg):
        knn, atts = ctx.saved_tensors
        return agg_backward(grad_agg.contiguous(), knn, atts, ctx.P), None, None


def aggregate(feats, knn, atts):
    return _Aggregate.apply(feats, knn.contiguous(), atts.contiguous())


def lpips_pack(conv_w, conv_b, lins, shift, scale):
    dev = conv_w[0].device
    packed = torch.empty(int(_lib.lib().occnerf_lpips_packed_floats()), device=dev, dtype=torch.float32)
    w = [t.detach().contiguous() for t in conv_w]
    b = [t.detach().contiguous() for t in conv_b]
    li = [t.detach().contiguous() for t in lins]
    sh, sc = shift.detach().contiguous(), scale.detach().contiguous()
    if len(w) != 13 or len(b) != 13 or len(li) != 5:
        raise RuntimeError('lpips_pack: needs 13 conv weights, 13 conv biases and 5 lin weights')
    with _guard_dev(dev):
        hw, hb, hl = _ptr_table(w, 'conv weight'), _ptr_table(b, 'conv bias'), _ptr_table(li, 'lin weight')
        rc = _lib.lib().occnerf_lpips_pack(hw, hb, hl, _chk(sh, torch.float32, 'shift'), _chk(sc, torch.float32, 'scale'),
                                           packed.data_ptr(), _stream(packed))
    _lib.check(rc, 'lpips_pack')
    return packed


def _lpips_layout(in0, in1):
    if in0.is_contiguous() and in1.is_contiguous():
        return in0, in1, 0
    p0, p1 = in0.permute(0, 2, 3, 1), in1.permute(0, 2, 3, 1)
    if p0.is_contiguous() and p1.is_contiguous():
        return in0, in1, 1
    return in0.contiguous(), in1.contiguous(), 0


def lpips_forward(packed, in0, in1, want_res=False):
    if in0.dim() != 4 or in0.shape != in1.shape or in0.shape[1] != 3:
        raise RuntimeError(f'lpips: in0 and in1 must both be [N,3,H,W], got {tuple(in0.shape)} and {tuple(in1.shape)}')
    N, _, H, W = in0.shape
    in0, in1, nhwc = _lpips_layout(in0, in1)
    with _guard(in0):
        nw = int(_lib.lib().occnerf_lpips_workspace_floats(N, H, W))
        if nw < 0:
            raise RuntimeError(f'lpips: H and W must be >= 16 so that relu5_3 is not empty (got {H} x {W}), N >= 1')
        work = torch.empty(nw, device=in0.device, dtype=torch.float32)
        val = torch.empty(N, device=in0.device, dtype=torch.float32)
        res = torch.empty(5, N, device=in0.device, dtype=torch.float32) if want_res else None
        a0 = _chk(in0.permute(0, 2, 3, 1) if nhwc else in0, torch.float32, 'in0')
        a1 = _chk(in1.permute(0, 2, 3, 1) if nhwc else in1, torch.float32, 'in1')
        rc = _lib.lib().occnerf_lpips_forward(_chk(packed, torch.float32, 'packed'), a0, a1, N, H, W, nhwc, work.data_ptr(),
                                              val.data_ptr(), None if res is None else res.data_ptr(), _stream(in0))
    _lib.check(rc, 'lpips_forward')
    return val, res, work, nhwc


def lpips_backward(packed, work, shape, nhwc, gres, need0, need1):
    N, _, H, W = shape

    def alloc():
        return torch.empty((N, H, W, 3) if nhwc else (N, 3, H, W), device=work.device, dtype=torch.float32)
    d0 = alloc() if need0 else None
    d1 = alloc() if need1 else None
    with _guard(work):
        rc = _lib.lib().occnerf_lpips_backward(_chk(packed, torch.float32, 'packed'), _chk(work, torch.float32, 'work'), N,
                                               H, W, nhwc, _chk(gres, torch.float32, 'gres'),
                                               None if d0 is None else d0.data_ptr(), None if d1 is None else d1.data_ptr(),
                                               _stream(work))
    _lib.check(rc, 'lpips_backward')
    fix = (lambda t: None if t is None else t.permute(0, 3, 1, 2)) if nhwc else (lambda t: t)
# ... 78 lines not shown
```

Before: 1.208 million rays/s.

## Share a single cached centre feature row across samples inside the kNN centre ball

Samples that fall inside the cached kNN centre radius no longer get their own kNN index rows written or their own 68-float feature row. The feature kernel instead reads the centre's neighbour indices directly and records, in a row_of map, that these samples use one shared row appended after the real rows. The canonical MLP is passed the row_of map so it can read that shared row. This cuts kNN output writes and mlp_in stores for centre samples, and it adds an indirection, an atomic counter and an extra prefetch stage in the feature kernel.

After: 1.219 million rays/s (median of 6 runs). No clear change (+0.9%).

```diff
diff --git a/include/occnerf_hip.h b/include/occnerf_hip.h
--- a/include/occnerf_hip.h
+++ b/include/occnerf_hip.h
@@ -123,6 +123,14 @@
                                      const int32_t *h_coarse_rows, const int32_t *h_seed_from_coarser,
                                      int32_t nscale, const int32_t *query_rows, const int32_t *n_query_dev, int32_t *ray_start,
                                      const float *center, const int32_t *center_idx, int32_t *knn_idxs, void *stream);
+int occnerf_msknn_clustered_shared(const float *xyz, const float *mask, int64_t n_rays, int32_t samples_per_ray,
+                                   const float *points, const float *centers,
+                                   const int32_t *cluster_ranges, const float *cluster_radius, int32_t ncl,
+                                   const float *group_centers, const int32_t *group_ranges, const float *group_radius, int32_t ngrp,
+                                   const int32_t *h_coarse_rows, const int32_t *h_seed_from_coarser,
+                                   int32_t nscale, const int32_t *query_rows, const int32_t *n_query_dev, int32_t *ray_start,
+                                   const float *center, const int32_t *center_idx, int32_t skip_center_rows, int32_t *knn_idxs,
+                                   void *stream);
 
 int occnerf_knn_small(const float *q, int32_t nq, const float *s, int32_t ns, int32_t k,
                       int32_t *idx, void *stream);
@@ -164,6 +172,17 @@
                             const int32_t *n_dev, const float *point_geo, const float *point_tail, int32_t P,
                             const float *center, const float *center_agg,
                                      float *mlp_in, float *raw, float *enc_in, void *stream);
+int occnerf_sample_features_shared(const float *xyz, int64_t N, const int32_t *knn_idxs, int32_t nscale,
+                                   const float *point_base, const double *normals,
+                                   const double *unit_normals, const float *counter,
+                                   const float *table, float bound, float two_bound,
+                                   const float *embeddings, const int32_t *offsets,
+                                   const int32_t *h_offsets, uint32_t L, float S, uint32_t H,
+                                   const int32_t *geo_idxs, const float *att_in, const int32_t *rows,
+                                   const int32_t *n_dev, const float *point_geo, const float *point_tail, int32_t P,
+                                   const float *center, const float *center_agg, const int32_t *center_idx,
+                                   int32_t *row_of, int32_t shared_row, int32_t *shared_count,
+                                   float *mlp_in, float *raw, float *enc_in, void *stream);
 
 int occnerf_agg_forward(const float *feats, int32_t F, const int32_t *knn, const float *atts, int64_t N, int32_t K,
                         float *agg, void *stream);
diff --git a/occnerf_amd/_lib.py b/occnerf_amd/_lib.py
--- a/occnerf_amd/_lib.py
+++ b/occnerf_amd/_lib.py
@@ -51,6 +51,8 @@
                                            _vp, _vp, _vp, _vp, _vp]),
     'occnerf_msknn_clustered_centered': (C.c_int, [_vp, _vp, _i64, _i32, _vp, _vp, _vp, _vp, _i32, _vp, _vp, _vp, _i32, _vp, _vp, _i32,
                                            _vp, _vp, _vp, _vp, _vp, _vp, _vp]),
+    'occnerf_msknn_clustered_shared': (C.c_int, [_vp, _vp, _i64, _i32, _vp, _vp, _vp, _vp, _i32, _vp, _vp, _vp, _i32, _vp, _vp, _i32,
+                                                  _vp, _vp, _vp, _vp, _vp, _i32, _vp, _vp]),
     'occnerf_knn_center': (C.c_int, [_vp, _vp, _vp, _vp, _i32, _vp, _vp, _vp]),
     'occnerf_knn_small': (C.c_int, [_vp, _i32, _vp, _i32, _i32, _vp, _vp]),
     'occnerf_unit_normals': (C.c_int, [_vp, _i32, _vp, _vp]),
@@ -84,6 +86,9 @@
     'occnerf_sample_features_centered': (C.c_int, [_vp, _i64, _vp, _i32, _vp, _vp, _vp, _vp, _vp, _f32, _f32, _vp,
                                                     _vp, _vp, _u32, _f32, _u32, _vp, _vp, _vp, _vp, _vp, _vp, _i32, _vp, _vp,
                                                     _vp, _vp, _vp, _vp]),
+    'occnerf_sample_features_shared': (C.c_int, [_vp, _i64, _vp, _i32, _vp, _vp, _vp, _vp, _vp, _f32, _f32, _vp,
+                                                  _vp, _vp, _u32, _f32, _u32, _vp, _vp, _vp, _vp, _vp, _vp, _i32, _vp, _vp,
+                                                  _vp, _vp, _i32, _vp, _vp, _vp, _vp, _vp]),
     'occnerf_canonical_mlp_packed_floats': (_i64, []),
     'occnerf_canonical_mlp_pack': (C.c_int, [_vp, _vp, _vp, _vp]),
     'occnerf_canonical_mlp': (C.c_int, [_vp, _i64, _vp, _vp, _vp]),
diff --git a/occnerf_amd/config.py b/occnerf_amd/config.py
--- a/occnerf_amd/config.py
+++ b/occnerf_amd/config.py
@@ -91,6 +91,7 @@
     'ray_patch_order': True,
     'knn_culling': True,
     'knn_center_cache': True,
+    'share_centre_rows': True,
     'warp_bone_culling': True,
 }
 
diff --git a/occnerf_amd/csrc/features.hip b/occnerf_amd/csrc/features.hip
--- a/occnerf_amd/csrc/features.hip
+++ b/occnerf_amd/csrc/features.hip
@@ -394,10 +394,16 @@
     LevelRecs levels, LevelRecs8 levels8, FeatParams prm, const int32_t *__restrict__ rows ,
     const int32_t *__restrict__ n_dev , float *__restrict__ mlp_in, float *__restrict__ raw, float *__restrict__ enc_in_out,
     const float *__restrict__ center ,
-    const float *__restrict__ center_agg ) {
+    const float *__restrict__ center_agg ,
+    const int32_t *__restrict__ center_idx ,
+    int32_t *__restrict__ row_of ,
+    const int32_t shared_row ,
+    int32_t *__restrict__ shared_count ) {
     constexpr int NK = 4 * kKnn;
     float ccx = 0.f, ccy = 0.f, ccz = 0.f, cr2 = 0.f;
     if (center) ccx = center[0], ccy = center[1], ccz = center[2], cr2 = center[3];
+    const bool ids_from_center = center_idx != nullptr && cr2 > 0.0f;
+    int n_shared = 0;
     __shared__ float4 s_tail[LDS_TAIL ? kLdsTailPoints : 1];
     __shared__ float4 s_out[LDS_TAIL ? 768 : 256];
     static_assert(sizeof(float4) * (size_t)kLdsTailPoints + sizeof(float4) * 768 <= 160 * 1024,
@@ -424,12 +430,16 @@
         const int64_t i_raw = group0 + it * ngroups;
         return i_raw < N ? i_raw : N - 1;
     };
-    auto load_a = [&](int64_t i, StageA &a) {
-        const int32_t *id = knn_idxs + i * NK;
+    auto load_p = [&](int64_t i, float (&p)[3]) {
         struct __attribute__((packed, aligned(4))) F3 { float v[3]; };
+        const F3 pq = *reinterpret_cast<const F3 *>(xyz + i * 3);
+        p[0] = pq.v[0], p[1] = pq.v[1], p[2] = pq.v[2];
+    };
+    auto load_ids = [&](int64_t i, StageA &a) {
+        const float dx = a.p[0] - ccx, dy = a.p[1] - ccy, dz = a.p[2] - ccz;
+        const float d2 = __builtin_fmaf(dz, dz, __builtin_fmaf(dy, dy, dx * dx));
+        const int32_t *id = (ids_from_center && d2 < cr2) ? center_idx : knn_idxs + i * NK;
         struct __attribute__((packed, aligned(4))) I4 { int v[4]; };
-        const F3 pq = *reinterpret_cast<const F3 *>(xyz + i * 3);
-        a.p[0] = pq.v[0], a.p[1] = pq.v[1], a.p[2] = pq.v[2];
         a.idg = id[g];
         a.id89 = id[8 + (g >> 2)];
         const I4 q = *reinterpret_cast<const I4 *>(id + g * 5);
@@ -437,16 +447,20 @@
         a.id5[4] = id[g * 5 + 4];
     };
     StageA cur, nxt;
-    int32_t i1;
+    int32_t i1, i2;
     {
-        const int64_t o0 = out_row(0), o1 = out_row(1);
-        load_a(rows ? (int64_t)rows[o0] : o0, cur);
+        const int64_t o0 = out_row(0), o1 = out_row(1), o2 = out_row(2);
+        const int64_t i0 = rows ? (int64_t)rows[o0] : o0;
+        load_p(i0, cur.p);
+        load_ids(i0, cur);
         i1 = rows ? rows[o1] : (int32_t)o1;
+        load_p(i1, nxt.p);
+        i2 = rows ? rows[o2] : (int32_t)o2;
     }
     for (int64_t it = 0; it < iters; it++) {
         const bool live = group0 + it * ngroups < N;
         const int64_t o = out_row(it);
-        const int64_t o2 = out_row(it + 2);
+        const int64_t o3 = out_row(it + 3);
         float *out = mlp_in + o * 68;
 
         bool cached_agg = false;
@@ -583,8 +597,10 @@
                             __float_as_uint(x[2]) == __float_as_uint(center_agg[38]) && __float_as_uint(x[3]) == __float_as_uint(center_agg[39]);
             cached_enc = __builtin_amdgcn_ballot_w64(live && !eq) == 0;
         }
-        float2 ev[2];
-        int32_t i2;
+        const bool share_row = row_of != nullptr && cached_enc;
+        float2 ev[2] = {make_float2(0.f, 0.f), make_float2(0.f, 0.f)};
+        float p2[3];
+        int32_t i3;
         if (!cached_enc) {
             LevelTaps4 tp[2];
             bool oob = false;
@@ -608,8 +624,9 @@
                     level_taps_select(xt, embeddings, levels8.r[2 * (lane64 >> 3) + a], tp[a]);
                 }
             }
-            load_a(i1, nxt);
-            i2 = rows ? rows[o2] : (int32_t)o2;
+            load_ids(i1, nxt);
+            load_p(i2, p2);
+            i3 = rows ? rows[o3] : (int32_t)o3;
             __builtin_amdgcn_sched_barrier(0);
             float2 evt[2];
 #pragma unroll
@@ -620,12 +637,15 @@
 #pragma unroll
             for (int a = 0; a < 2; a++) ev[a] = make_float2(__shfl(evt[a].x, tr), __shfl(evt[a].y, tr));
         } else {
-            load_a(i1, nxt);
-            i2 = rows ? rows[o2] : (int32_t)o2;
-            const float4 ce = *reinterpret_cast<const float4 *>(center_agg + 40 + 4 * g);
-            ev[0] = make_float2(ce.x, ce.y), ev[1] = make_float2(ce.z, ce.w);
-        }
-        s_out[threadIdx.x] = make_float4(ev[0].x, ev[0].y, ev[1].x, ev[1].y);
+            load_ids(i1, nxt);
+            load_p(i2, p2);
+            i3 = rows ? rows[o3] : (int32_t)o3;
+            if (!share_row) {
+                const float4 ce = *reinterpret_cast<const float4 *>(center_agg + 40 + 4 * g);
+                ev[0] = make_float2(ce.x, ce.y), ev[1] = make_float2(ce.z, ce.w);
+            }
+        }
+        if (!share_row) s_out[threadIdx.x] = make_float4(ev[0].x, ev[0].y, ev[1].x, ev[1].y);
 
         float agg[4] = {0.f, 0.f, 0.f, 0.f};
         if (!cached_agg) {
@@ -666,19 +686,27 @@
             }
 #pragma unroll
             for (int c = 0; c < 3; c++) tail[c] = grp_sum8(tail[c]);
-        } else {
+        } else if (!share_row) {
             const float4 ca = *reinterpret_cast<const float4 *>(center_agg + 4 * g);
             agg[0] = ca.x, agg[1] = ca.y, agg[2] = ca.z, agg[3] = ca.w;
             tail[0] = center_agg[32], tail[1] = center_agg[33], tail[2] = center_agg[34], var = center_agg[35];
         }
-        if (live) {
+        if (live && !share_row) {
             *reinterpret_cast<float4 *>(out + 4 * g) = make_float4(agg[0], agg[1], agg[2], agg[3]);
             if (g == 0) *reinterpret_cast<float4 *>(out + 32) = make_float4(tail[0], tail[1], tail[2], var);
             *reinterpret_cast<float4 *>(out + 36 + 4 * g) = s_out[threadIdx.x];
         }
+        if (row_of) {
+            if (live && g == 0) row_of[o] = share_row ? shared_row : (int32_t)o;
+            if (share_row) n_shared += __builtin_popcountll(__builtin_amdgcn_ballot_w64(live && g == 0));
+        }
         cur = nxt;
+#pragma unroll
+        for (int c = 0; c < 3; c++) nxt.p[c] = p2[c];
         i1 = i2;
-    }
+        i2 = i3;
+    }
+    if (shared_count && n_shared > 0 && lane64 == 0) atomicAdd(shared_count, n_shared);
 }
 
 
@@ -774,8 +802,30 @@
                                              const float *point_geo, const float *point_tail, int32_t P,
                                              const float *center, const float *center_agg,
                                              float *mlp_in, float *raw, float *enc_in, void *stream) {
+    return occnerf_sample_features_shared(xyz, N, knn_idxs, nscale, point_base, normals, unit_normals, counter, table, bound,
+                                          two_bound, embeddings, offsets, h_offsets, L, S, H, geo_idxs, att_in, rows, n_dev,
+                                          point_geo, point_tail, P, center, center_agg, nullptr, nullptr, 0, nullptr, mlp_in, raw,
+                                          enc_in, stream);
+}
+
+OCC_API int occnerf_sample_features_shared(const float *xyz, int64_t N, const int32_t *knn_idxs,
+                                           int32_t nscale, const float *point_base, const double *normals,
+                                           const double *unit_normals, const float *counter,
+                                           const float *table, float bound, float two_bound,
+                                           const float *embeddings, const int32_t *offsets,
+                                           const int32_t *h_offsets, uint32_t L, float S, uint32_t H,
+                                           const int32_t *geo_idxs,
+                                           const float *att_in, const int32_t *rows, const int32_t *n_dev,
+                                           const float *point_geo, const float *point_tail, int32_t P,
+                                           const float *center, const float *center_agg, const int32_t *center_idx,
+                                           int32_t *row_of, int32_t shared_row, int32_t *shared_count,
+                                           float *mlp_in, float *raw, float *enc_in, void *stream) {
     using namespace occ;
     OCC_REQUIRE(!center == !center_agg, "sample_features: center and center_agg come together");
+    OCC_REQUIRE(center || !center_idx, "sample_features: center_idx needs the centre");
+    OCC_REQUIRE(row_of || !shared_count, "sample_features: shared_count comes with row_of");
+    OCC_REQUIRE(!row_of || shared_row >= 0, "sample_features: shared_row=%d", shared_row);
+    OCC_REQUIRE(!row_of || N < (1ll << 31), "sample_features: row_of holds 32-bit rows");
     if (N <= 0) return 0;
     OCC_REQUIRE(xyz && knn_idxs && point_base && normals && unit_normals && (counter || att_in) && table &&
                     embeddings && offsets && mlp_in && raw, "sample_features: null argument");
@@ -818,7 +868,8 @@
                            N, knn_idxs, reinterpret_cast<const float4 *>(point_geo),
                            reinterpret_cast<const float4 *>(point_tail),
                            reinterpret_cast<const float4 *>(table), reinterpret_cast<const float2 *>(embeddings),
-                           levels, levels8, prm, rows, n_dev, mlp_in, raw, enc_in, center, center_agg);
+                           levels, levels8, prm, rows, n_dev, mlp_in, raw, enc_in, center, center_agg, center_idx, row_of,
+                           shared_row, shared_count);
         return check_launch("sample_features");
     }
     OCC_REQUIRE(!center, "sample_features: the centre aggregate is only supported on the renderer's path");
diff --git a/occnerf_amd/csrc/knn.hip b/occnerf_amd/csrc/knn.hip
--- a/occnerf_amd/csrc/knn.hip
+++ b/occnerf_amd/csrc/knn.hip
@@ -348,6 +348,7 @@
     const int32_t *__restrict__ ray_start ,
     const float *__restrict__ center ,
     const int32_t *__restrict__ center_idx ,
+    const bool skip_center_rows ,
     const float split_extent2 ) {
     const int lane = threadIdx.x & 63;
     float ccx = 0.f, ccy = 0.f, ccz = 0.f, cr2 = 0.f;
@@ -398,7 +399,7 @@
                     live[a] = false;
                     struct __attribute__((packed, aligned(4))) I4 { int v[4]; };
                     struct __attribute__((packed, aligned(4))) I2 { int v[2]; };
-                    for (int l = 0; part == 0 && l < sc.nscale; l++) {
+                    for (int l = 0; part == 0 && !skip_center_rows && l < sc.nscale; l++) {
                         int32_t *out = knn_idxs + (qi[a] * sc.nscale + l) * kK;
                         const int32_t *ci = center_idx + l * kK;
                         *reinterpret_cast<I4 *>(out) = I4{{ci[0], ci[1], ci[2], ci[3]}};
@@ -728,8 +729,24 @@
                                              const int32_t *query_rows, const int32_t *n_query_dev, int32_t *ray_start,
                                              const float *center, const int32_t *center_idx,
                                              int32_t *knn_idxs, void *stream) {
+    return occnerf_msknn_clustered_shared(xyz, mask, n_rays, samples_per_ray, points, centers, cluster_ranges, cluster_radius, ncl,
+                                          group_centers, group_ranges, group_radius, ngrp, h_coarse_rows, h_seed_from_coarser,
+                                          nscale, query_rows, n_query_dev, ray_start, center, center_idx, 0, knn_idxs, stream);
+}
+
+OCC_API int occnerf_msknn_clustered_shared(const float *xyz, const float *mask, int64_t n_rays, int32_t samples_per_ray,
+                                           const float *points,
+                                           const float *centers, const int32_t *cluster_ranges,
+                                           const float *cluster_radius, int32_t ncl, const float *group_centers,
+                                           const int32_t *group_ranges, const float *group_radius, int32_t ngrp,
+                                           const int32_t *h_coarse_rows,
+                                           const int32_t *h_seed_from_coarser, int32_t nscale,
+                                           const int32_t *query_rows, const int32_t *n_query_dev, int32_t *ray_start,
+                                           const float *center, const int32_t *center_idx, int32_t skip_center_rows,
+                                           int32_t *knn_idxs, void *stream) {
     using namespace occ;
     OCC_REQUIRE(!center == !center_idx, "msknn_clustered: center and center_idx come together (occnerf_knn_center)");
+    OCC_REQUIRE(!skip_center_rows || center, "msknn_clustered: skip_center_rows needs the centre");
     if (n_rays <= 0 || samples_per_ray <= 0) return 0;
     OCC_REQUIRE((!query_rows && !n_query_dev && !ray_start) || (query_rows && n_query_dev && ray_start),
                 "msknn_clustered: query_rows, n_query_dev and the ray_start scratch come together");
@@ -789,7 +806,7 @@
                        reinterpret_cast<const float4 *>(centers), reinterpret_cast<const int2 *>(cluster_ranges),
                        cluster_radius, reinterpret_cast<const float4 *>(group_centers),
                        reinterpret_cast<const int2 *>(group_ranges), group_radius, sc, knn_idxs, ticket, query_rows, ray_start,
-                       center, center_idx, kSplitExtent2);
+                       center, center_idx, skip_center_rows != 0, kSplitExtent2);
     return check_launch("msknn_clustered");
 }
 
diff --git a/occnerf_amd/network.py b/occnerf_amd/network.py
--- a/occnerf_amd/network.py
+++ b/occnerf_amd/network.py
@@ -252,19 +252,27 @@
             if cfg.get('dedup_global_positions', False):
                 frows, fcount = ops.unique_heads(xyz, 3, frows, fcount, scan=scan_a, scan_count=count)
         self.last_head_counts = (fcount, None)
+        share = center is not None and bool(cfg.get('share_centre_rows', True))
+        share_rows = share and not dedup and cfg.get('share_centre_rows', True) != 'lists'
         if cfg.get('knn_query_list', True):
-            knn = ops.msknn_clustered(xyz, rays8.shape[0], S, ctx['clusters'], ctx['seed'], rows=frows, count=fcount, center=center)
+            knn = ops.msknn_clustered(xyz, rays8.shape[0], S, ctx['clusters'], ctx['seed'], rows=frows, count=fcount, center=center,
+                                      skip_center_rows=share)
         else:
-            knn = ops.msknn_clustered(xyz, rays8.shape[0], S, ctx['clusters'], ctx['seed'], mask=kmask, center=center)
+            knn = ops.msknn_clustered(xyz, rays8.shape[0], S, ctx['clusters'], ctx['seed'], mask=kmask, center=center,
+                                      skip_center_rows=share)
         if center is not None and len(center) > 3 and center[3] != self._center_stamp(table):
             raise RuntimeError('stale kNN centre: its cached feature row was computed from another table / counter / embedding '
                                'version than this frame\'s (ops.sample_features freshness contract)')
-        mlp_in, raw_c, _ = ops.sample_features(
+        mlp_in, raw_c, _, *row_of = ops.sample_features(
             xyz, knn, self.point_base.detach(), ctx['normals'], ctx['unit'],
             self.point_counter.detach(), table, ctx['bound32'], ctx['two_bound32'],
             enc.embeddings.detach(), enc.offsets, enc.log2_per_level_scale, enc.base_resolution,
             rows=frows, count=fcount, pack=pack, center=None if center is None else center[0],
-            center_agg=None if center is None else center[2])
+            center_agg=None if center is None else center[2], center_idx=center[1] if share else None,
+            want_row_of=share_rows, shared_count=self.last_shared_rows if share_rows else None)
+        row_of = row_of[0] if share_rows else None
+        if share_rows:
+            mlp_in[-1] = center[4]
         del knn
         if dedup:
             scan_b, mrows, mcount, _ = ops.repeat_heads(mlp_in, 68, fcount)
@@ -272,7 +280,7 @@
                 mrows, mcount = ops.unique_heads(mlp_in, 68, mrows, mcount, scan=scan_b, scan_count=fcount)
             self.last_head_counts = (fcount, mcount)
         return {'dedup': dedup, 'rays8': rays8, 'z': z, 'mask': mask, 'rows': rows, 'count': count, 'mlp_in': mlp_in,
-                'raw_c': raw_c, 'scan_a': scan_a, 'scan_b': scan_b, 'mrows': mrows, 'mcount': mcount, 'cnl': pk['cnl'],
+                'row_of': row_of, 'raw_c': raw_c, 'scan_a': scan_a, 'scan_b': scan_b, 'mrows': mrows, 'mcount': mcount, 'cnl': pk['cnl'],
                 'cnl_bf16': pk['cnl_bf16'], 'domain_flag': pk['domain_flag'], 'N': xyz.shape[0]}
 
     @staticmethod
@@ -291,7 +299,7 @@
             raw = ops.scatter_raw_heads(raw_h, st['raw_c'], st['rows'], st['count'], st['scan_a'], st['scan_b'],
                                         torch.zeros(N, 5, device=dev))
         else:
-            mlp(st['raw_c'], st['count'])
+            mlp(st['raw_c'], st['count'], st['row_of'])
             raw = ops.scatter_raw(st['raw_c'], st['rows'], st['count'], torch.zeros(N, 5, device=dev))
         st['mlp_in'] = None
         return ops.composite(raw, st['mask'], st['z'], st['rays8'], bgcolor, out=out, out_rows=out_rows)[:3]
@@ -322,7 +330,8 @@
             c[:8].contiguous(), idx[None].expand(8, -1, -1).contiguous(), self.point_base.detach(), ctx['normals'], ctx['unit'],
             self.point_counter.detach(), table, ctx['bound32'], ctx['two_bound32'], enc.embeddings.detach(), enc.offsets,
             enc.log2_per_level_scale, enc.base_resolution, pack=pack, want_enc_in=True)
-        return center, idx, ops.center_row(row[0], enc_in[0]), self._center_stamp(table)
+        agg = ops.center_row(row[0], enc_in[0])
+        return center, idx, agg, self._center_stamp(table), ops.shared_row(agg)
 
     def _center_stamp(self, table):
         return (table.data_ptr(), table._version, self.point_counter._version, self.cnl_mlp.module.encoder.embeddings._version)
@@ -448,6 +457,7 @@
                 cond = f32(dst_posevec).reshape(-1) if iter_val >= nr.kick_in_iter else \
                     torch.zeros(dst_posevec.numel(), device=dev)
                 center = None
+                self.last_shared_rows = torch.zeros(1, device=dev, dtype=torch.int32)
                 if cfg.get('knn_center_cache', True) and cfg.get('knn_culling', True):
                     center = self._knn_center(cond, hann.tolist(), wc['table'], pack)
                 Rs, Ts = ops.pose_motion_bases(self.pose_decoder, f32(dst_posevec).reshape(-1), refine, f32(dst_Rs[0]),
diff --git a/occnerf_amd/ops.py b/occnerf_amd/ops.py
--- a/occnerf_amd/ops.py
+++ b/occnerf_amd/ops.py
@@ -434,7 +434,8 @@
     return center, idx
 
 
-def msknn_clustered(xyz, n_rays, S, cl, seed_from_coarser, mask=None, rows=None, count=None, out=None, center=None):
+def msknn_clustered(xyz, n_rays, S, cl, seed_from_coarser, mask=None, rows=None, count=None, out=None, center=None,
+                    skip_center_rows=False):
     nscale = int(cl['ranges'].shape[0]) + 1
     if out is None:
         out = torch.empty(n_rays * S, nscale, 10, device=xyz.device, dtype=torch.int32)
@@ -444,7 +445,7 @@
     _kc, pc = _host_i32(cl['coarse_rows'])
     _ks, ps = _host_i32(seed_from_coarser)
     with _guard(xyz):
-        rc = _lib.lib().occnerf_msknn_clustered_centered(
+        rc = _lib.lib().occnerf_msknn_clustered_shared(
             _chk(xyz, torch.float32, 'xyz'), _opt(mask, torch.float32, 'mask'), int(n_rays), int(S),
             _chk(cl['points'], torch.float32, 'points'), _chk(cl['centers'], torch.float32, 'centers'), _chk(cl['ranges'], torch.int32, 'cluster_ranges'),
             _chk(cl['radius'], torch.float32, 'cluster_radius'), int(cl['ncl']),
@@ -453,7 +454,8 @@
             _opt(rows, torch.int32, 'rows'), _opt(count, torch.int32, 'count'),
             None if ray_start is None else ray_start.data_ptr(),
             None if center is None else _chk(center[0], torch.float32, 'center'),
-            None if center is None else _chk(center[1], torch.int32, 'center_idx'), out.data_ptr(), _stream(xyz))
+            None if center is None else _chk(center[1], torch.int32, 'center_idx'), int(bool(skip_center_rows)),
+            out.data_ptr(), _stream(xyz))
     _lib.check(rc, 'msknn_clustered')
     return out
 
@@ -525,9 +527,14 @@
     return torch.cat([mlp_in_row[:36], enc_in_row[:4], mlp_in_row[36:68]]).contiguous()
 
 
+def shared_row(center_agg):
+    return torch.cat([center_agg[:36], center_agg[40:72]])
+
+
 def sample_features(xyz, knn_idxs, point_base, normals, unit, counter, table, bound32, two_bound32,
                     embeddings, offsets, S, H, raw=None, want_enc_in=False, geo_idxs=None,
-                    att_in=None, rows=None, count=None, pack=None, center=None, center_agg=None):
+                    att_in=None, rows=None, count=None, pack=None, center=None, center_agg=None, center_idx=None,
+                    want_row_of=False, shared_count=None):
     N = xyz.shape[0] if rows is None else rows.shape[0]
     dev = xyz.device
     if (pack is None and N > 0 and knn_idxs.shape[1] == 4 and geo_idxs is None and att_in is None
@@ -536,11 +543,12 @@
     geo, tail = pack if pack is not None else (None, None)
     if table.dim() != 2 or table.shape[1] != table_stride():
         raise RuntimeError(f'sample_features: table must be [P,{table_stride()}] (ops.point_table), got {tuple(table.shape)}')
-    mlp_in = torch.empty(N, 68, device=dev, dtype=torch.float32)
+    mlp_in = torch.empty(N + 1 if want_row_of else N, 68, device=dev, dtype=torch.float32)
+    row_of = torch.empty(N, device=dev, dtype=torch.int32) if want_row_of else None
     raw = torch.empty(N, 5, device=dev, dtype=torch.float32) if raw is None else raw
     enc_in = torch.empty(N, 4, device=dev, dtype=torch.float32) if want_enc_in else None
     with _guard_dev(dev):
-        rc = _lib.lib().occnerf_sample_features_centered(
+        rc = _lib.lib().occnerf_sample_features_shared(
             _chk(xyz, torch.float32, 'xyz'), N, _chk(knn_idxs, torch.int32, 'knn_idxs'),
             int(knn_idxs.shape[1]), _chk(point_base, torch.float32, 'point_base'),
             _chk(normals, torch.float64, 'normals'), _chk(unit, torch.float64, 'unit_normals'),
@@ -552,9 +560,13 @@
             _opt(geo, torch.float32, 'point_geo'), _opt(tail, torch.float32, 'point_tail'),
             0 if geo is None else int(geo.shape[0]),
             _opt(center, torch.float32, 'center'), _opt(center_agg, torch.float32, 'center_agg'),
+            _opt(center_idx, torch.int32, 'center_idx'), None if row_of is None else row_of.data_ptr(), int(N),
+            _opt(shared_count, torch.int32, 'shared_count'),
             mlp_in.data_ptr(), _chk(raw, torch.float32, 'raw'),
             None if enc_in is None else enc_in.data_ptr(), _stream(xyz))
     _lib.check(rc, 'sample_features')
+    if want_row_of:
+        return mlp_in, raw, enc_in, row_of
     return mlp_in, raw, enc_in
 
 
```
